# wkh923/m3pc

Hardware: AMD Instinct MI355X
Metric: MPC plan-steps/sec (N=1024, H=16, hopper-medium-v2); independent plan steps, 3 in flight (higher is better)
Workload: dtype bf16; 1 GPU; hopper-medium-v2 shapes (S=11,A=3) rtg_guiding N=1024 H=16 T=32 bf16 candidate pass + fp32 policy pass + fp32 re-score (arg-max and multinomial draw certified under the calibrated bound delta, 8.4 candidates re-scored on average); 3 independent plan steps in flight (policy pass / candidate pass / re-score of neighbouring steps on different streams); window resident in HBM; candidates_per_gpu=1024, global_candidates=1024, horizon=16, traj_length=32, steps_in_flight=3, settle_steps=24, parallelism=1 GPU

## Files before the change

include/m3pc_hip_debug.h:

```cpp
#ifndef M3PC_HIP_DEBUG_H
#define M3PC_HIP_DEBUG_H

#ifdef __cplusplus
extern "C" {
#endif

int m3pc_debug_gemm(int dtype, const void* A, const void* Wt, const float* bias, const float* res, void* C, int M, int N,
                    int K, int gelu, int f32out, int variant, void* stream);
typedef struct m3pc_debug_gemm_args {
    int dtype;
    const void* A;
    int lda;
    int amap[3];
    const void* W;
    int ldw;
    int M, N, K;
    const float* bias;
    const float* rowtab;
    int rt_mod, rt_ld;
    int gelu;
    const float* res;
    int ldr;
    void* C;
    int f32out;
    int ldc;
    int cmap[3];
    float* ws;
    long long ws_bytes;
    int a_padded;
    const float* ln_g;
    const float* ln_b;
    float* ln_out;
    const float* a_ln_g;
    const float* a_ln_b;
    int variant;
    void* stream;
    int* picked;
} m3pc_debug_gemm_args;
int m3pc_debug_gemm_ex(const m3pc_debug_gemm_args* a);
int m3pc_debug_gemm_plan(const m3pc_debug_gemm_args* a);
int m3pc_debug_gemm_group(const m3pc_debug_gemm_args* a, int n);
int m3pc_debug_clock(long long* out2);
int m3pc_debug_clock_big(long long* out4);
int m3pc_debug_topk(const float* v, int n, int k, int* idx_out, void* stream);
int m3pc_debug_calibrate_stats(const float* scores_low, const float* f32, int n, float factor, float* stats, float* delta_out,
                               void* stream);
long long m3pc_debug_block_stream_bytes(void);
int m3pc_debug_block_fused(const void* O, int M, const float* res, const float* rowtab, int rt_mod, const void* Wo, const void* W1,
                           const void* W2, void* stream_buf, int pack, const float* bo, const float* b1, const float* b2,
                           const float* ln2_g, const float* ln2_b, const float* lnA_g, const float* lnA_b, const float* lnB_g0,
                           const float* lnB_b0, const float* lnB_g1, const float* lnB_b1, int out_mod, int out_grp, float* Xout,
                           void* Hout, int variant, void* stream, long long* stamps);
int m3pc_debug_block_fused_qkv(const void* O, int M, const float* res, const void* Wo, const void* W1, const void* W2, const void* Wqkv,
                               void* stream_buf, const float* bo, const float* b1, const float* b2, const float* ln2_g,
                               const float* ln2_b, const float* lnA_g, const float* lnA_b, const float* bqkv, float* Xout, void* QKV,
                               void* stream, long long* stamps, int x_bf16);
int m3pc_debug_block_fused_heads(const void* O, int M, const float* rowtab, int rt_mod, const void* Wo, const void* W1, const void* W2,
                                 const void* Wh, void* stream_buf, const float* bo, const float* b1, const float* b2, const float* ln2_g,
                                 const float* ln2_b, const float* lnA_g, const float* lnA_b, const float* lnB_g0, const float* lnB_b0,
                                 const float* lnB_g1, const float* lnB_b1, int out_mod, int out_grp, const float* hb1, const float* hw2,
                                 const float* hb2, const float* hmean, const float* hstd, float* out0, float* out1, void* stream,
                                 long long* stamps);
long long m3pc_debug_kv_stream_bytes(void);
int m3pc_debug_kv_fused(const void* Z, int n, int Le, int kept0, int off0, int kept1, int off1, const void* We0, const void* We1,
                        const void* Wkv, void* stream_buf, const float* rowtab0, const float* rowtab1, const float* ln_g,
                        const float* ln_b, const float* bkv, void* KV, void* stream, long long* stamps);
int m3pc_debug_attention_bf16(const void* QKV, const void* QKVs, void* O, int batch, int n_own, int n_sh, int kernel, void* stream,
                              long long* stamps);
int m3pc_debug_attention_dec_bf16(const void* Qtab, const void* QKVm, const void* KV, void* O, float* pre, int n, int nq, int Lm, int kernel,
                                  void* stream);
int m3pc_debug_attention_dec_le_bf16(const void* Qtab, const void* QKVm, const void* KV, void* O, float* pre, int n, int nq, int Lm, int Le,
                                     int kernel, void* stream);
int m3pc_debug_attention_mix_bf16(const void* Qown, const void* Qsh, const void* KV, const void* QKVm, void* O, int n, int Lq, int Lq2, int kernel,
                                  void* stream);
int m3pc_debug_attention(int dtype, const void* Q, long long q_bstride, int ldq, int Lq, int orow1, const void* Q2, int ldq2, int Lq2,
                         int orow2, const void* K1, const void* V1, long long kv1_bstride, int ldkv1, int L1, const void* K2,
                         const void* V2, int ldkv2, int L2, const void* Kp, const void* Vp, int ldp, int Lp, float* pre, void* O,
                         long long o_bstride, int ldo, int batch, int n_head, int hd, float scale, int kernel, int* picked,
                         void* stream);
int m3pc_debug_stamp_log(m3pc_handle* h, int cap, long long* out, int* n_logged);
int m3pc_debug_step_streams_created(m3pc_handle* h);
int m3pc_debug_xcc_probe(int* out, int n_blocks, void* stream);

#ifdef __cplusplus
}
#endif
#endif
```

m3pc_amd/capi.py:

```python
from __future__ import annotations

import ctypes as C
import os
from typing import Dict, Optional, Sequence

import torch

_HERE = os.path.dirname(os.path.abspath(__file__))
LIB_PATH = os.environ.get("M3PC_LIB") or os.path.join(_HERE, "libm3pc_hip.so")

STATES, ACTIONS, REWARDS, RETURNS = 0, 1, 2, 3
KEYS = ("states", "actions", "rewards", "returns")
MODE_RTG, MODE_CRITIC, MODE_NOISE = 0, 1, 2
PREC_FP32, PREC_BF16, PREC_BF16X3 = 0, 1, 2
PRECISIONS = {"fp32": PREC_FP32, "bf16": PREC_BF16, "bf16x3": PREC_BF16X3}
LOW_PRECISION = (PREC_BF16, PREC_BF16X3)
PROF_LAYER_TAIL = 16
ABI_VERSION = 7
GOAL_PIID, GOAL_ID = 0, 1
SLOTS = 4


def precision_code(name: str) -> int:
    if name not in PRECISIONS:
# ... 249 lines not shown
        x = x.contiguous()
        out = torch.empty(x.shape, dtype=torch.float32, device=x.device)
        rows = x.numel() // x.shape[-1]
        check(self.lib.m3pc_tokenize(self._h, key, _ptr(x), int(x.dtype == torch.float64), _ptr(out), rows,
                                     _stream(self.device)))
        return out

    def detokenize(self, key: int, y: torch.Tensor) -> torch.Tensor:
        y = y.contiguous()
        out = torch.empty_like(y)
        check(self.lib.m3pc_detokenize(self._h, key, _ptr(y), _ptr(out), y.numel() // y.shape[-1],
                                       _stream(self.device)))
        return out

    def forward(self, tokens: Sequence[Optional[torch.Tensor]], masks: Sequence, want=KEYS, precision=PREC_FP32):
        B = next(t.shape[0] for t in tokens if t is not None)
        toks = [None if t is None else t.to(torch.float32).contiguous() for t in tokens]
        tp = (C.c_void_p * 4)(*[None if t is None else t.data_ptr() for t in toks])
        mb = [bytes(bytearray(int(v != 0) for v in m)) for m in masks]
        mbuf = [C.create_string_buffer(b, len(b)) for b in mb]
        mp = (C.c_void_p * 4)(*[C.addressof(b) for b in mbuf])
        dev = self.device
        feat = (self.S, self.A, 1, 1)
        out = {}
        for k, name in enumerate(KEYS):
            if name in want and k != ACTIONS:
                out[name] = torch.empty((B, self.T, feat[k]), dtype=torch.float32, device=dev)
        mu = sd = None
        if "actions" in want:
            mu = torch.empty((B, self.T, self.A), dtype=torch.float32, device=dev)
            sd = torch.empty_like(mu)
            out["actions"] = (mu, sd)
        check(self.lib.m3pc_forward(self._h, B, tp, mp, _ptr(out.get("states")), _ptr(out.get("rewards")),
                                    _ptr(out.get("returns")), _ptr(mu), _ptr(sd), precision, _stream(dev)))
        return out

    @staticmethod
    def _mask_ptrs(masks):
        mb = [bytes(bytearray(int(v != 0) for v in m)) for m in masks]
        mbuf = [C.create_string_buffer(b, len(b)) for b in mb]
        return (C.c_void_p * 4)(*[C.addressof(b) for b in mbuf]), mbuf

    def goal_step(self, states, actions, rewards, rtg, masks_pi, masks_fid, idx: int):
        E = states.shape[0]
        f32 = dict(dtype=torch.float32, device=self.device)
        ins = [self._f32(t) for t in (states, actions, rewards)]
        inferred = torch.empty((E, self.T, self.S), **f32)
        window = torch.empty((E, self.T, self.S), **f32)
        mu = torch.empty((E, self.T, self.A), **f32)
        sd = torch.empty_like(mu)
        rt = (C.c_double * E)(*[float(v) for v in rtg])
        pi, keep1 = self._mask_ptrs(masks_pi)
        fid, keep2 = self._mask_ptrs(masks_fid)
        check(self.lib.m3pc_goal_step(self._h, E, _ptr(ins[0]), _ptr(ins[1]), _ptr(ins[2]), rt, pi, fid, int(idx), _ptr(inferred),
                                      _ptr(window), _ptr(mu), _ptr(sd), _stream(self.device)))
        return mu, sd, inferred, window

    def goal_step_batch(self, states, actions, idx: int, goal_mode: int = GOAL_PIID, precision: int = PREC_BF16,
                        want_window: bool = False, out=None):
        E = states.shape[0]
        f32 = dict(dtype=torch.float32, device=self.device)
        s, a = self._f32(states), self._f32(actions)
        assert s.shape == (E, self.T, self.S) and a.shape == (E, self.T, self.A)
        mu, sd = out if out is not None else (torch.empty((E, self.A), **f32), torch.empty((E, self.A), **f32))
        window = torch.empty((E, self.T, self.S), **f32) if want_window else None
        check(self.lib.m3pc_goal_step_batch(self._h, E, _ptr(s), _ptr(a), int(idx), int(goal_mode), int(precision), _ptr(window),
                                            _ptr(mu), _ptr(sd), _stream(self.device)))
        return (mu, sd, window) if want_window else (mu, sd)

    @staticmethod
    def _f32(t):
        return t if (t.dtype == torch.float32 and t.is_contiguous()) else t.to(torch.float32).contiguous()

    def _args(self, mode, precision, horizon, n_total, n_begin, n_count, lmbda, discount, rtg, slot=0, returns=None):
        a = PlanArgs(mode, precision, horizon, n_total, n_begin, n_count, lmbda, discount, rtg, slot, 0, None, 0, 0)
        if returns is not None:
            assert returns.is_cuda and returns.is_contiguous() and returns.numel() == self.T
            assert returns.dtype in (torch.float32, torch.float64)
            a.returns_f64 = int(returns.dtype == torch.float64)
            a.returns = returns.data_ptr()
        return a

    def policy_pass(self, mode: int, states, actions, rewards, horizon: int, rtg: float, slot: int = 0, returns=None,
                    loc=None, std=None, pruned: bool = False):
        args = self._args(mode, PREC_FP32, horizon, 1, 0, 1, 0.0, 0.0, rtg, slot, returns)
        if pruned and loc is None and std is None:
            args.flags = PLAN_PRUNED_POLICY
        check(self.lib.m3pc_policy_pass(self._h, C.byref(args), _ptr(self._f32(states)), _ptr(self._f32(actions)),
                                        _ptr(self._f32(rewards)), _ptr(loc), _ptr(std), _stream(self.device)))

    def candidate_pass(self, mode: int, states, actions, rewards, eps, horizon: int, lmbda: float, discount: float,
                       n_total: int, n_begin: int = 0, n_count: Optional[int] = None, precision: int = PREC_FP32, slot: int = 0,
                       want_debug: bool = False, out=None, defer_join: bool = False, window: int = 0):
        n_count = n_total - n_begin if n_count is None else n_count
        dev = self.device
        f32 = dict(dtype=torch.float32, device=dev)
        out = out or {}
        loc = out.get("loc")
        std = out.get("std")
        if loc is None:
            loc = torch.empty((self.T, self.A), **f32)
            std = torch.empty((self.T, self.A), **f32)
        acts = out.get("sample_actions")
        if acts is None:
            acts = torch.empty((n_count, horizon, self.A), **f32)
        er = out.get("expect_return")
        if er is None:
            er = torch.empty((n_count,), **f32)
        pr = torch.empty((n_count, horizon), **f32) if want_debug else None
        pb = torch.empty((n_count, horizon), **f32) if want_debug else None
        args = self._args(mode, precision, horizon, n_total, n_begin, n_count, lmbda, discount, 0.0, slot)
        args.flags = PLAN_DEFER_JOIN if defer_join else 0
        args.window = int(window)
        ins = [self._f32(t) for t in (states, actions, rewards, eps)]
        check(self.lib.m3pc_candidate_pass(self._h, C.byref(args), _ptr(ins[0]), _ptr(ins[1]), _ptr(ins[2]), _ptr(ins[3]),
                                           _ptr(loc), _ptr(std), _ptr(acts), _ptr(er), _ptr(pr), _ptr(pb), _stream(dev)))
        res = dict(loc=loc, std=std, sample_actions=acts, expect_return=er)
        if want_debug:
            res["pred_rewards"], res["pred_boot"] = pr, pb
        return res

    def policy_pass_batch(self, mode: int, states, actions, rewards, horizon: int, rtg, slot: int = 0, loc=None, std=None):
        E = states.shape[0]
        args = self._args(mode, PREC_FP32, horizon, 1, 0, 1, 0.0, 0.0, 0.0, slot)
        rt = (C.c_double * E)(*[float(v) for v in rtg])
        check(self.lib.m3pc_policy_pass_batch(self._h, C.byref(args), E, _ptr(self._f32(states)), _ptr(self._f32(actions)),
                                              _ptr(self._f32(rewards)), rt, _ptr(loc), _ptr(std), _stream(self.device)))

    def candidate_join(self, slot: int):
        check(self.lib.m3pc_candidate_join(self._h, int(slot), _stream(self.device)))

    def plan_step(self, mode: int, states, actions, rewards, eps, horizon: int, rtg: float, lmbda: float,
                  discount: float, n_total: int, n_begin: int = 0, n_count: Optional[int] = None,
                  precision: int = PREC_FP32, want_debug: bool = False, slot: int = 0, returns=None):
        n_count = n_total - n_begin if n_count is None else n_count
        dev = self.device
        f32 = dict(dtype=torch.float32, device=dev)
        loc = torch.empty((self.T, self.A), **f32)
        std = torch.empty((self.T, self.A), **f32)
        acts = torch.empty((n_count, horizon, self.A), **f32)
        er = torch.empty((n_count,), **f32)
        pr = torch.empty((n_count, horizon), **f32) if want_debug else None
        pb = torch.empty((n_count, horizon), **f32) if want_debug else None
        args = self._args(mode, precision, horizon, n_total, n_begin, n_count, lmbda, discount, rtg, slot, returns)
        ins = [self._f32(t) for t in (states, actions, rewards, eps)]
        check(self.lib.m3pc_plan_step(self._h, C.byref(args), _ptr(ins[0]), _ptr(ins[1]), _ptr(ins[2]), _ptr(ins[3]),
                                      _ptr(loc), _ptr(std), _ptr(acts), _ptr(er), _ptr(pr), _ptr(pb), _stream(dev)))
        res = dict(loc=loc, std=std, sample_actions=acts, expect_return=er)
        if want_debug:
            res["pred_rewards"], res["pred_boot"] = pr, pb
        return res

    def plan_step_certified(self, mode: int, states, actions, rewards, eps, expo, horizon: int, rtg: float, lmbda: float,
                            discount: float, n_total: int, temperature: float, delta: float = 0.0, grow_delta: bool = False,
                            kmin: int = 8, kmax: int = 128, rfirst: int = 2, rmax: int = 32, precision: int = PREC_BF16,
                            slot: int = 0, returns=None, pruned: bool = False):
        dev = self.device
        f32 = dict(dtype=torch.float32, device=dev)
        loc = torch.empty((self.T, self.A), **f32)
        std = torch.empty((self.T, self.A), **f32)
        acts = torch.empty((n_total, horizon, self.A), **f32)
        low = torch.empty((n_total,), **f32)
        merged = torch.empty((n_total,), **f32)
        lst = torch.empty((int(rmax) + 1024,), dtype=torch.int32, device=dev)
        sel = self.select_buffers(n_total)
        args = self._args(mode, precision, horizon, n_total, 0, n_total, lmbda, discount, rtg, slot, returns)
        args.flags = PLAN_PRUNED_POLICY if pruned else 0
        cert = CertArgs(float(temperature), float(delta), int(bool(grow_delta)), int(kmin), int(kmax), int(rfirst), int(rmax))
# ... 316 lines not shown
```

m3pc_amd/csrc/elementwise.hip:

```cpp
#include "kernels.h"

namespace m3pc {

__device__ __forceinline__ int map_row(const RowMap& m, int r) {
    if (m.rpg == 0) return r;
    return (r / m.rpg) * m.gstride + (r % m.rpg) + m.off;
}

__device__ __forceinline__ float wave_sum(float v) {
#pragma unroll
    for (int o = 32; o > 0; o >>= 1) v += __shfl_xor(v, o);
    return v;
}
__device__ __forceinline__ float wave_max(float v) {
#pragma unroll
    for (int o = 32; o > 0; o >>= 1) v = fmaxf(v, __shfl_xor(v, o));
    return v;
}

__global__ __launch_bounds__(256) void embed_kernel(EmbedP p) {
    const long long row = blockIdx.x;
    const int b = (int)(row / p.L), j = (int)(row % p.L);
    const int2 kt = p.tokmap[j];
    const int key = kt.x, t = kt.y;
    const int D = p.feat[key];
    const float* x = p.tok[key] + (long long)b * p.bstride[key] + (p.widx ? (long long)p.widx[b] * p.wstride[key] : 0) + (long long)t * D;
    __shared__ float xs[32];
    if (threadIdx.x < D) {
        float v = x[threadIdx.x];
        if (p.normalize[key]) v = (v - p.mean[key][threadIdx.x]) / p.stdv[key][threadIdx.x];
        xs[threadIdx.x] = v;
    }
    __syncthreads();
    const float* WT = p.WT[key];
    const float* E = p.E[key] + (long long)t * p.d;
    float* out = p.X + row * p.d;
    float vals[4];
    float s = 0.f;
#pragma unroll
    for (int i = 0; i < 4; ++i) {
        const int c = threadIdx.x + i * blockDim.x;
        vals[i] = 0.f;
        if (c < p.d) {
            float acc = 0.f;
            for (int f = 0; f < D; ++f) acc = fmaf(xs[f], WT[f * p.d + c], acc);
            acc += E[c];
            out[c] = acc;
            vals[i] = acc;
            s += acc;
        }
    }
    if (!p.ln_g) return;
    __shared__ float red[8];
    const int lane = threadIdx.x & 63, wid = threadIdx.x >> 6, nwv = blockDim.x >> 6;
    s = wave_sum(s);
    if (lane == 0) red[wid] = s;
    __syncthreads();
    float tot = 0.f;
    for (int w = 0; w < nwv; ++w) tot += red[w];
    const float mean = tot / (float)p.d;
    float q = 0.f;
#pragma unroll
    for (int i = 0; i < 4; ++i)
        if (threadIdx.x + i * blockDim.x < p.d) {
            const float c = vals[i] - mean;
            q += c * c;
        }
    q = wave_sum(q);
    __syncthreads();
    if (lane == 0) red[wid] = q;
    __syncthreads();
    tot = 0.f;
    for (int w = 0; w < nwv; ++w) tot += red[w];
    const float rstd = rsqrtf(tot / (float)p.d + 1e-5f);
#pragma unroll
    for (int i = 0; i < 4; ++i) {
        const int c = threadIdx.x + i * blockDim.x;
        if (c < p.d) {
            const float y = (vals[i] - mean) * rstd * p.ln_g[c] + p.ln_b[c];
            if (p.Hf) p.Hf[row * p.d + c] = y;
            if (p.Hb) p.Hb[row * p.d + c] = (bf16_t)y;
        }
    }
}
template <int NV>
__global__ __launch_bounds__(256) void embed_rows_kernel(EmbedP p, int CB, int nchunk) {
    const int lane = threadIdx.x & 63;
    const int w = blockIdx.x * 4 + (threadIdx.x >> 6);
    if (w >= p.L * nchunk) return;
    const int j = w / nchunk, ch = w % nchunk;
    const int2 kt = p.tokmap[j];
    const int key = kt.x, t = kt.y;
    const int D = p.feat[key], d = p.d;
    const float* WT = p.WT[key];
    const float* E = p.E[key] + (long long)t * d;
    const bool indep = j < p.n_indep;
    const int b0 = ch * CB, b1 = b0 + CB < p.batch ? b0 + CB : p.batch;
    if (indep && p.x_first_only && b0 > 0 && p.Hb && !p.Hf && j < p.n_sh) return;
    const int n_own = p.L - p.n_sh;
    float4 ev[NV], gv[NV], bv[NV];
#pragma unroll
    for (int i = 0; i < NV; ++i) {
        const int c = (i * 64 + lane) * 4;
        ev[i] = *(const float4*)(E + c);
        if (p.ln_g) {
            gv[i] = *(const float4*)(p.ln_g + c);
            bv[i] = *(const float4*)(p.ln_b + c);
        }
    }
    float4 x[NV], y[NV];
    for (int b = b0; b < b1; ++b) {
        if (b == b0 || !indep) {
            const float* xin = p.tok[key] + (long long)b * p.bstride[key] + (p.widx ? (long long)p.widx[b] * p.wstride[key] : 0) + (long long)t * D;
#pragma unroll
            for (int i = 0; i < NV; ++i) x[i] = make_float4(0.f, 0.f, 0.f, 0.f);
            for (int f = 0; f < D; ++f) {
                float xf = xin[f];
                if (p.normalize[key]) xf = (xf - p.mean[key][f]) / p.stdv[key][f];
#pragma unroll
                for (int i = 0; i < NV; ++i) {
                    const float4 wv = *(const float4*)(WT + (long long)f * d + (i * 64 + lane) * 4);
                    x[i].x = fmaf(xf, wv.x, x[i].x);
                    x[i].y = fmaf(xf, wv.y, x[i].y);
                    x[i].z = fmaf(xf, wv.z, x[i].z);
                    x[i].w = fmaf(xf, wv.w, x[i].w);
                }
            }
            float s = 0.f;
#pragma unroll
            for (int i = 0; i < NV; ++i) {
                x[i].x += ev[i].x;
                x[i].y += ev[i].y;
                x[i].z += ev[i].z;
                x[i].w += ev[i].w;
                s += (x[i].x + x[i].y) + (x[i].z + x[i].w);
            }
            if (p.ln_g) {
                const float mean = wave_sum(s) / (float)d;
                float q = 0.f;
#pragma unroll
                for (int i = 0; i < NV; ++i) {
                    const float c0 = x[i].x - mean, c1 = x[i].y - mean, c2 = x[i].z - mean, c3 = x[i].w - mean;
                    q += (c0 * c0 + c1 * c1) + (c2 * c2 + c3 * c3);
                }
                const float rstd = rsqrtf(wave_sum(q) / (float)d + 1e-5f);
#pragma unroll
                for (int i = 0; i < NV; ++i) {
                    y[i].x = (x[i].x - mean) * rstd * gv[i].x + bv[i].x;
                    y[i].y = (x[i].y - mean) * rstd * gv[i].y + bv[i].y;
                    y[i].z = (x[i].z - mean) * rstd * gv[i].z + bv[i].z;
                    y[i].w = (x[i].w - mean) * rstd * gv[i].w + bv[i].w;
                }
            }
        }
        const long long row = (long long)b * p.L + j;
        if (!(indep && p.x_first_only && b > 0)) {
            if (p.Xb) {
#pragma unroll
                for (int i = 0; i < NV; ++i) {
                    typedef bf16_t bf16x4_t __attribute__((ext_vector_type(4)));
                    bf16x4_t o;
                    o[0] = (bf16_t)x[i].x;
                    o[1] = (bf16_t)x[i].y;
                    o[2] = (bf16_t)x[i].z;
                    o[3] = (bf16_t)x[i].w;
                    stream_store(o, (bf16x4_t*)(p.Xb + row * d + (i * 64 + lane) * 4));
                }
            } else {
#pragma unroll
                for (int i = 0; i < NV; ++i) *(float4*)(p.X + row * d + (i * 64 + lane) * 4) = x[i];
            }
        }
        if (!p.ln_g) continue;
        if (p.Hf) {
#pragma unroll
            for (int i = 0; i < NV; ++i) *(float4*)(p.Hf + row * d + (i * 64 + lane) * 4) = y[i];
        }
        if (p.Hb) {
            bf16_t* dst;
            if (p.n_sh == 0)
                dst = p.Hb + row * d;
            else if (j >= p.n_sh)
                dst = p.Hb + ((long long)b * n_own + (j - p.n_sh)) * d;
            else if (b == 0)
                dst = p.Hb_sh + (long long)j * d;
            else
                continue;
#pragma unroll
            for (int i = 0; i < NV; ++i) {
                typedef bf16_t bf16x4_t __attribute__((ext_vector_type(4)));
                bf16x4_t o;
                o[0] = (bf16_t)y[i].x;
                o[1] = (bf16_t)y[i].y;
                o[2] = (bf16_t)y[i].z;
                o[3] = (bf16_t)y[i].w;
                stream_store(o, (bf16x4_t*)(dst + (i * 64 + lane) * 4));
            }
        }
    }
}

void launch_embed(const EmbedP& p, hipStream_t st) {
    const long long rows = (long long)p.batch * p.L;
    if (rows <= 0) return;
    if (p.d % 256 == 0 && p.d <= 1024) {
        int CB = p.batch / 64;
        CB = CB < 1 ? 1 : (CB > 16 ? 16 : CB);
        if (p.n_indep == 0 && CB > 4) CB = 4;
        const int nchunk = (p.batch + CB - 1) / CB;
        const int waves = p.L * nchunk;
        const dim3 grid((waves + 3) / 4), block(256);
        switch (p.d / 256) {
            case 1: hipLaunchKernelGGL(embed_rows_kernel<1>, grid, block, 0, st, p, CB, nchunk); break;
            case 2: hipLaunchKernelGGL(embed_rows_kernel<2>, grid, block, 0, st, p, CB, nchunk); break;
            case 3: hipLaunchKernelGGL(embed_rows_kernel<3>, grid, block, 0, st, p, CB, nchunk); break;
            default: hipLaunchKernelGGL(embed_rows_kernel<4>, grid, block, 0, st, p, CB, nchunk); break;
        }
        return;
    }
    hipLaunchKernelGGL(embed_kernel, dim3((unsigned)rows), dim3(p.d < 256 ? p.d : 256), 0, st, p);
}

__global__ __launch_bounds__(256) void gather_rows_kernel(GatherP p) {
    const long long row = blockIdx.x;
    const int b = (int)(row / p.rows_per_batch), i = (int)(row % p.rows_per_batch);
    const int s = p.rowsrc[i];
    const float* src = s >= 0 ? p.Xe + (long long)b * p.xe_bstride + (long long)s * p.d : p.table + (long long)(-s - 1) * p.d;
    for (int c = threadIdx.x * 4; c < p.d; c += blockDim.x * 4) {
        const float4 v = *(const float4*)(src + c);
        if (p.out) *(float4*)(p.out + row * p.d + c) = v;
        if (p.outb) {
            bf16_t* ob = p.outb + row * p.d + c;
            ob[0] = (bf16_t)v.x;
            ob[1] = (bf16_t)v.y;
            ob[2] = (bf16_t)v.z;
            ob[3] = (bf16_t)v.w;
        }
    }
}
void launch_gather_rows(const GatherP& p, hipStream_t st) {
    const long long rows = (long long)p.batch * p.rows_per_batch;
    if (rows <= 0) return;
    hipLaunchKernelGGL(gather_rows_kernel, dim3((unsigned)rows), dim3(p.d / 4 < 256 ? p.d / 4 : 256), 0, st, p);
}

__global__ __launch_bounds__(256) void layernorm_kernel(LnP p) {
    const int lane = threadIdx.x & 63;
    const int r = blockIdx.x * 4 + (threadIdx.x >> 6);
    if (r >= p.rows) return;
    const float* x = p.X + (long long)map_row(p.xmap, r) * p.ldx;
    const int n = p.d >> 6;
    float v[16];
    float s = 0.f;
#pragma unroll
    for (int i = 0; i < 16; ++i)
        if (i < n) {
            v[i] = x[i * 64 + lane];
            s += v[i];
        }
    const float inv_d = 1.0f / (float)p.d;
    float mean = wave_sum(s) * inv_d;
    float q = 0.f;
#pragma unroll
    for (int i = 0; i < 16; ++i)
        if (i < n) {
            const float c = v[i] - mean;
            q += c * c;
        }
    float rstd = rsqrtf(wave_sum(q) * inv_d + 1e-5f);
#pragma unroll
    for (int i = 0; i < 16; ++i)
        if (i < n) v[i] = (v[i] - mean) * rstd * p.g1[i * 64 + lane] + p.b1[i * 64 + lane];
    if (p.g2) {
        s = 0.f;
#pragma unroll
        for (int i = 0; i < 16; ++i)
            if (i < n) s += v[i];
        mean = wave_sum(s) * inv_d;
        q = 0.f;
#pragma unroll
        for (int i = 0; i < 16; ++i)
            if (i < n) {
                const float c = v[i] - mean;
                q += c * c;
            }
        rstd = rsqrtf(wave_sum(q) * inv_d + 1e-5f);
#pragma unroll
        for (int i = 0; i < 16; ++i)
            if (i < n) v[i] = (v[i] - mean) * rstd * p.g2[i * 64 + lane] + p.b2[i * 64 + lane];
    }
#pragma unroll
    for (int i = 0; i < 16; ++i)
        if (i < n) {
            if (p.Yf) p.Yf[(long long)r * p.d + i * 64 + lane] = v[i];
            if (p.Yb) p.Yb[(long long)r * p.d + i * 64 + lane] = (bf16_t)v[i];
        }
}
typedef float f32x4v __attribute__((ext_vector_type(4)));
typedef __bf16 bf16x4v __attribute__((ext_vector_type(4)));
__global__ __launch_bounds__(256) void layernorm_vec_kernel(LnP p) {
// ... 310 lines not shown
#pragma unroll
    for (int f = 0; f < AMAX; ++f) {
        s1[f] = 0.f;
        s2[f] = 0.f;
        const int ff = f < p.A ? f : p.A - 1;
#pragma unroll
        for (int i = 0; i < 4; ++i)
            if (i < n) {
                const f32x4v wm = *(const f32x4v*)(p.Wmu + (long long)ff * p.d + i * 256 + lane * 4);
                const f32x4v wl = *(const f32x4v*)(p.Wls + (long long)ff * p.d + i * 256 + lane * 4);
#pragma unroll
                for (int e = 0; e < 4; ++e) {
                    s1[f] = fmaf(v[i][e], wm[e], s1[f]);
                    s2[f] = fmaf(v[i][e], wl[e], s2[f]);
                }
            }
    }
#pragma unroll
    for (int f = 0; f < AMAX; ++f) {
        s1[f] = wave_sum(s1[f]);
        s2[f] = wave_sum(s2[f]);
    }
#pragma unroll
    for (int f = 0; f < AMAX; ++f)
        if (f < p.A && lane == f) {
            p.mu[(long long)r * p.A + f] = s1[f] + p.bmu[f];
            float ls = tanhf(s2[f] + p.bls[f]);
            ls = -5.0f + 0.5f * (2.0f - (-5.0f)) * (ls + 1.0f);
            p.sd[(long long)r * p.A + f] = expf(ls);
        }
}
__global__ __launch_bounds__(256) void actor_head_small_kernel(ActorP p) {
    const int lane = threadIdx.x & 63;
    const int r = blockIdx.x * 4 + (threadIdx.x >> 6);
    if (r >= p.rows) return;
    const float* x = p.X + (long long)map_row(p.xmap, r) * p.ldx;
    const int n = p.d >> 6;
    float v[16];
#pragma unroll
    for (int i = 0; i < 16; ++i)
        if (i < n) v[i] = x[i * 64 + lane];
    for (int f = 0; f < p.A; ++f) {
        float s1 = 0.f, s2 = 0.f;
#pragma unroll
        for (int i = 0; i < 16; ++i)
            if (i < n) {
                s1 = fmaf(v[i], p.Wmu[(long long)f * p.d + i * 64 + lane], s1);
                s2 = fmaf(v[i], p.Wls[(long long)f * p.d + i * 64 + lane], s2);
            }
        s1 = wave_sum(s1);
        s2 = wave_sum(s2);
        if (lane == 0) {
            p.mu[(long long)r * p.A + f] = s1 + p.bmu[f];
            float ls = tanhf(s2 + p.bls[f]);
            ls = -5.0f + 0.5f * (2.0f - (-5.0f)) * (ls + 1.0f);
            p.sd[(long long)r * p.A + f] = expf(ls);
        }
    }
}
bool actor_head_fuses_ln(int d, int A) { return d % 256 == 0 && d <= 1024 && A <= 8; }
void launch_actor_head(const ActorP& p, hipStream_t st) {
    if (p.rows <= 0) return;
    const dim3 grid((p.rows + 3) / 4), block(256);
    if (actor_head_fuses_ln(p.d, p.A)) {
        if (p.A <= 4) hipLaunchKernelGGL((actor_head_kernel<4>), grid, block, 0, st, p);
        else hipLaunchKernelGGL((actor_head_kernel<8>), grid, block, 0, st, p);
    } else {
        hipLaunchKernelGGL(actor_head_small_kernel, grid, block, 0, st, p);
    }
}

__global__ __launch_bounds__(256) void sample_kernel(SampleP p) {
    const long long tot = (long long)p.n_count * p.T * p.A;
    if (blockIdx.x == 0) {
        for (int x = threadIdx.x; x < p.T * p.A; x += blockDim.x) {
            if (p.loc_out && p.loc) p.loc_out[x] = p.loc[x];
            if (p.sd_out && p.sd) p.sd_out[x] = p.sd[x];
        }
    }
    for (long long x = blockIdx.x * (long long)blockDim.x + threadIdx.x; x < tot; x += (long long)gridDim.x * blockDim.x) {
        const int a = (int)(x % p.A);
        const int t = (int)((x / p.A) % p.T);
        const long long n = x / ((long long)p.A * p.T);
        float v;
        if (t < p.idx) {
            v = p.hist_actions[(p.widx ? (long long)p.widx[n] * p.T * p.A : 0) + t * p.A + a];
        } else {
            const int ta = t * p.A + a;
            const long long src = p.index ? (long long)p.index[n] : p.n_begin + n;
            if (p.mode == 2) {
                v = p.eps[(src * p.h + (t - p.idx)) * p.A + a];
            } else if (p.mode == 0) {
                const float e = p.eps[(src * p.T + t) * p.A + a];
                v = tanhf(__fadd_rn(__fmul_rn(e, p.sd[ta]), p.loc[ta]));
            } else {
                const float e = p.eps[(src * p.h + (t - p.idx)) * p.A + a];
                v = __fadd_rn(tanhf(p.loc[ta]), __fmul_rn(e, 0.09f));
                v = fminf(fmaxf(v, -0.99999f), 0.99999f);
            }
            if (p.sample_actions) p.sample_actions[(n * p.h + (t - p.idx)) * p.A + a] = v;
        }
        p.cand[x] = v;
    }
}
void launch_sample(const SampleP& p, hipStream_t st) {
    const long long tot = (long long)p.n_count * p.T * p.A;
    if (tot <= 0) return;
    const int grid = (int)((tot + 255) / 256 < 2048 ? (tot + 255) / 256 : 2048);
    hipLaunchKernelGGL(sample_kernel, dim3(grid), dim3(256), 0, st, p);
}

#define CR_ROWS 16
__global__ __launch_bounds__(256) void critic_kernel(CriticP p) {
    __shared__ float sa[CR_ROWS][32];
    __shared__ float h1[CR_ROWS][256];
    __shared__ float red[CR_ROWS][4];
    const int tid = threadIdx.x;
    const int r0 = blockIdx.x * CR_ROWS;
    const int SA = p.S + p.A, Hd = p.hidden;
    const bool on = tid < Hd;
    for (int x = tid; x < CR_ROWS * SA; x += 256) {
        const int rr = x / SA, f = x % SA, r = r0 + rr;
        float v = 0.f;
        if (r < p.rows) v = f < p.S ? (p.states[(long long)r * p.S + f] - p.om[f]) / p.os[f] : p.actions[(long long)r * p.A + (f - p.S)];
        sa[rr][f] = v;
    }
    float qmin = 0.f;
    for (int net = 0; net < 2; ++net) {
        __syncthreads();
        {
            float acc[CR_ROWS];
#pragma unroll
            for (int rr = 0; rr < CR_ROWS; ++rr) acc[rr] = 0.f;
            if (on) {
                for (int f = 0; f < SA; ++f) {
                    const float w = p.W1T[net][f * Hd + tid];
#pragma unroll
                    for (int rr = 0; rr < CR_ROWS; ++rr) acc[rr] = fmaf(sa[rr][f], w, acc[rr]);
                }
                const float bb = p.b1[net][tid];
#pragma unroll
                for (int rr = 0; rr < CR_ROWS; ++rr) h1[rr][tid] = fmaxf(acc[rr] + bb, 0.f);
            }
        }
        __syncthreads();
        float acc[CR_ROWS];
#pragma unroll
        for (int rr = 0; rr < CR_ROWS; ++rr) acc[rr] = 0.f;
        float bb = 0.f, w3 = 0.f;
        if (on) {
            for (int k = 0; k < Hd; ++k) {
                const float w = p.W2T[net][k * Hd + tid];
#pragma unroll
                for (int rr = 0; rr < CR_ROWS; ++rr) acc[rr] = fmaf(h1[rr][k], w, acc[rr]);
            }
            bb = p.b2[net][tid];
            w3 = p.W3[net][tid];
        }
#pragma unroll
        for (int rr = 0; rr < CR_ROWS; ++rr) {
            float v = on ? fmaxf(acc[rr] + bb, 0.f) * w3 : 0.f;
            v = wave_sum(v);
            if ((tid & 63) == 0) red[rr][tid >> 6] = v;
        }
        __syncthreads();
        if (tid < CR_ROWS) {
            const float q = red[tid][0] + red[tid][1] + red[tid][2] + red[tid][3] + p.b3[net][0];
            qmin = net == 0 ? q : fminf(qmin, q);
            if (net == 1 && r0 + tid < p.rows) p.q[r0 + tid] = qmin;
        }
    }
}
template <int NT>
__global__ __launch_bounds__(256, 2) void critic_mfma_kernel(CriticP p) {
#if defined(__HIP_DEVICE_COMPILE__)
    typedef float f32x16v __attribute__((ext_vector_type(16)));
    const int lane = threadIdx.x & 63, wave = threadIdx.x >> 6;
    const int l31 = lane & 31, lh = lane >> 5;
    const int r = (blockIdx.x * 4 + wave) * 32 + l31;
    if ((blockIdx.x * 4 + wave) * 32 >= p.rows) return;
    const long long rl = r < p.rows ? r : p.rows - 1;
    const int SA = p.S + p.A;
    float x[16];
#pragma unroll
// ... 244 lines not shown
```

m3pc_amd/csrc/kernels.h:

```cpp
#pragma once
#include <hip/hip_runtime.h>
#include <stdint.h>

#ifdef M3PC_LAB
#define M3PC_ENV(name) getenv(name)
#else
#define M3PC_ENV(name) ((const char*)nullptr)
#endif

namespace m3pc {

typedef __bf16 bf16_t;

enum DType { DT_F32 = 0, DT_BF16 = 1, DT_X3 = 2 };

static inline size_t dtype_size(int dt) { return dt == DT_F32 ? 4 : 2; }

#ifndef M3PC_STREAM_AUX
#define M3PC_STREAM_AUX 0
#endif
template <typename V>
__device__ __forceinline__ V stream_load(const V* p) { return M3PC_STREAM_AUX ? __builtin_nontemporal_load(p) : *p; }
template <typename V>
__device__ __forceinline__ void stream_store(V v, V* p) {
// ... 164 lines not shown
    const float* g2;
    const float* b2;
    float* Yf;
    bf16_t* Yb;
};
void launch_layernorm(const LnP& p, hipStream_t st);

struct AttnP {
    const void* Q;
    long long q_bstride;
    int ldq;
    const void* K1;
    const void* V1;
    long long kv1_bstride;
    int ldkv1;
    int L1;
    const void* K2;
    const void* V2;
    int ldkv2;
    int L2;
    void* O;
    long long o_bstride;
    int ldo;
    int batch, n_head, hd, Lq;
    float scale;
    const void* Q2;
    int ldq2, Lq2;
    int orow1, orow2;
    const float* pre_m;
    const float* pre_l;
    const float* pre_O;
    long long* stamps;
    int no_pipe;
};
void launch_attention_prestats(const AttnP& p, float* pre_m, float* pre_l, float* pre_O, hipStream_t st);
void launch_attention(const AttnP& p, int dtype, hipStream_t st);
#ifdef M3PC_LAB
extern thread_local int g_attn_picked;
#define M3PC_ATTN_PICK(id) (::m3pc::g_attn_picked = (id))
#else
#define M3PC_ATTN_PICK(id) ((void)0)
#endif
void launch_attention_bf16(const AttnP& p, hipStream_t st);
#ifdef M3PC_LAB
extern thread_local int g_gemm_picked[4];
extern thread_local int g_gemm_dry;
#define M3PC_GEMM_PICK(id, S, peel, flags)                                                          \
    (::m3pc::g_gemm_picked[0] = (id), ::m3pc::g_gemm_picked[1] = (S), ::m3pc::g_gemm_picked[2] = (peel), \
     ::m3pc::g_gemm_picked[3] = (flags))
#define M3PC_GEMM_PICK_FLAG(f) (::m3pc::g_gemm_picked[3] |= (f))
#define M3PC_GEMM_LAUNCH(...)                                     \
    do {                                                          \
        if (!::m3pc::g_gemm_dry) hipLaunchKernelGGL(__VA_ARGS__); \
    } while (0)
#else
#define M3PC_GEMM_PICK(id, S, peel, flags) ((void)0)
#define M3PC_GEMM_PICK_FLAG(f) ((void)0)
#define M3PC_GEMM_LAUNCH(...) hipLaunchKernelGGL(__VA_ARGS__)
#endif

struct EmbedP {
    const float* tok[4];
    long long bstride[4];
    const int* widx;
    long long wstride[4];
    int normalize[4];
    const float* mean[4];
    const float* stdv[4];
    const float* WT[4];
    const float* E[4];
    int feat[4];
    const int2* tokmap;
    int batch, L, d, T;
    float* X;
    bf16_t* Xb;
    const float* ln_g;
    const float* ln_b;
    float* Hf;
    bf16_t* Hb;
    int n_indep;
    int x_first_only;
    int n_sh;
    bf16_t* Hb_sh;
};
void launch_embed(const EmbedP& p, hipStream_t st);

struct GatherP {
    const float* Xe;
    long long xe_bstride;
    const float* table;
    const int* rowsrc;
    int rows_per_batch, batch, d;
    float* out;
    bf16_t* outb;
};
void launch_gather_rows(const GatherP& p, hipStream_t st);

struct HeadOutP {
    const float* X;
    const bf16_t* Xb;
    int ldx;
    int rows, d, D;
    const float* W;
    const float* b;
    const float* mean;
    const float* stdv;
    float* Y;
    RowMap ymap;
    int ldy;
};
void launch_head_out(const HeadOutP& p, hipStream_t st);
bool head_out_mfma_covers(int rows, int d, int D);

struct ActorP {
    const float* X;
    int ldx;
    RowMap xmap;
    int rows, d, A;
    const float* Wmu;
    const float* bmu;
    const float* Wls;
    const float* bls;
    float* mu;
    float* sd;
    const float* ln_g;
    const float* ln_b;
};
void launch_actor_head(const ActorP& p, hipStream_t st);
bool actor_head_fuses_ln(int d, int A);

struct SampleP {
    const float* hist_actions;
    const float* loc;
    const float* sd;
    const float* eps;
    int mode, T, A, idx, h, n_begin, n_count;
    const int* widx;
    const int* index;
    float* cand;
    float* sample_actions;
    float* loc_out;
    float* sd_out;
};
void launch_sample(const SampleP& p, hipStream_t st);

struct CriticP {
    const float* states;
    const float* actions;
    int rows, S, A, hidden;
    const float* om;
    const float* os;
    const float* W1T[2];
    const float* b1[2];
    const float* W2T[2];
    const float* b2[2];
    const float* W3[2];
    const float* b3[2];
    const float* W1F[2];
    const float* W2F[2];
    float* q;
};
void launch_critic(const CriticP& p, hipStream_t st);
bool critic_mfma_covers(int S, int A, int hidden);
size_t critic_w1f_floats(int hidden);
size_t critic_w2f_floats(int hidden);
void critic_pack(const float* W1, const float* W2, int SA, int hidden, float* w1f, float* w2f);

struct ScoreP {
// ... 82 lines not shown
```

m3pc_amd/csrc/m3pc.hip:

```cpp
#include <atomic>
#include <chrono>

#include "m3pc_internal.h"

namespace m3pc {
thread_local char g_err[512] = "";
int fail(int code, const char* fmt, ...) {
    va_list ap;
    va_start(ap, fmt);
    vsnprintf(g_err, sizeof(g_err), fmt, ap);
    va_end(ap);
    return code;
}
}

namespace {

int find_tensor(const m3pc_named_tensor* list, int n, const std::string& name) {
    for (int i = 0; i < n; ++i)
        if (list[i].name && name == list[i].name) return i;
    return -1;
}


}


static int fill_rtok(m3pc_handle* h, const double* rtg, int n_windows, hipStream_t st);

#pragma GCC visibility push(default)
extern "C" {

const char* m3pc_last_error(void) { return g_err; }
int m3pc_abi_version(void) { return M3PC_ABI_VERSION; }

int m3pc_create(const m3pc_dims* dims, int device, m3pc_handle** out) {
    if (!dims || !out) return fail(M3PC_EINVAL, "null argument");
    const m3pc_dims& D = *dims;
    if (D.n_embd % 64 || D.n_embd > 1024 || D.n_head <= 0 || D.n_embd % D.n_head)
        return fail(M3PC_EINVAL, "n_embd must be a multiple of 64 (<=1024) and divisible by n_head");
    const int hd = D.n_embd / D.n_head;
    if (hd != 32 && hd != 64 && hd != 128) return fail(M3PC_EINVAL, "head_dim %d unsupported (32, 64, 128)", hd);
    if (D.state_dim < 1 || D.state_dim > 32 || D.action_dim < 1 || D.action_dim > 32)
        return fail(M3PC_EINVAL, "state_dim/action_dim must be in [1,32]");
    if (D.traj_length < 1 || D.traj_length > 64) return fail(M3PC_EINVAL, "traj_length must be in [1,64]");
    if (D.n_dec_layer != 1) return fail(M3PC_EINVAL, "n_dec_layer must be 1 (every shipped m3pc config)");
    if (D.n_enc_layer < 1 || D.max_candidates < 1 || D.max_batch < 1) return fail(M3PC_EINVAL, "bad sizes");
    if (D.critic_hidden < 0 || D.critic_hidden > 256) return fail(M3PC_EINVAL, "critic_hidden must be <= 256");
    if (D.max_goal_batch < 0) return fail(M3PC_EINVAL, "max_goal_batch must be >= 0");
    HIPCHK(hipSetDevice(device));
    std::unique_ptr<m3pc_handle> h(new m3pc_handle());
    h->dm = D;
    h->device = device;
    h->d = D.n_embd;
    h->nh = D.n_head;
    h->hd = hd;
    h->T = D.traj_length;
    h->S = D.state_dim;
    h->A = D.action_dim;
    h->ff = 4 * D.n_embd;
    h->feat[0] = D.state_dim;
    h->feat[1] = D.action_dim;
    h->feat[2] = 1;
    h->feat[3] = 1;
    declare_weights(h.get());
    for (auto& kv : h->w) {
        CHK(dmalloc(&kv.second.f, (size_t)kv.second.numel));
        if (kv.second.gemm) {
            CHK(dmalloc(&kv.second.b, 2 * (size_t)kv.second.numel));
            h->gemm_w.push_back({kv.second.f, &kv.second});
        }
    }
    std::sort(h->gemm_w.begin(), h->gemm_w.end());
    const int d = h->d, T = h->T;
    for (int k = 0; k < 4; ++k) {
        CHK(dmalloc(&h->WT[k], (size_t)h->feat[k] * d));
        CHK(dmalloc(&h->Eenc[k], (size_t)T * d));
        CHK(dmalloc(&h->Edec[k], (size_t)T * d));
        CHK(dmalloc(&h->tok_mean[k], 32));
        CHK(dmalloc(&h->tok_std[k], 32));
    }
    CHK(dmalloc(&h->mask_tokens, (size_t)4 * d));
    {
        const long long r1 = (long long)D.max_candidates * 2 * T, r2 = (long long)D.max_batch * 4 * T;
        const long long r3 = (long long)D.max_goal_batch * 2 * T;
        long long R = r1 > r2 ? r1 : r2;
        if (r3 > R) R = r3;
        if (R < 4 * T) R = 4 * T;
        CHK(alloc_ws(h.get(), h->base, R, D.max_candidates > D.max_goal_batch ? D.max_candidates : D.max_goal_batch, 64LL << 20));
        if (D.max_goal_batch > 0) CHK(dmalloc(&h->goal_ws, (size_t)D.max_goal_batch * T * h->S));
    }
    {
        const int mr = D.max_rescore > 0 ? D.max_rescore : 64;
        long long R = (long long)mr * 2 * T;
        if (R < 4 * T) R = 4 * T;
        for (int par = 0; par < 2; ++par) {
            CHK(alloc_ws(h.get(), h->chain[par], R, mr, 32LL << 20));
            CHK(alloc_ws(h.get(), h->pchain[par], (long long)D.max_batch * 4 * T, 1, 32LL << 20));
        }
    }
    for (int s = 0; s < M3PC_SLOTS; ++s) {
        CHK(dmalloc(&h->slot[s].loc, (size_t)D.max_batch * T * h->A + 64));
        CHK(dmalloc(&h->slot[s].sd, (size_t)D.max_batch * T * h->A + 64));
        CHK(dmalloc(&h->slot[s].rtok, (size_t)D.max_batch * T));
    }
    CHK(dmalloc(&h->sel_scratch, 64));
    CHK(dmalloc(&h->d_topk, 1024));
    CHK(dmalloc(&h->er_top, 1024));
    CHK(dmalloc(&h->sa_buf, (size_t)(D.max_candidates > h->chain[0].max_cand ? D.max_candidates : h->chain[0].max_cand) * T * h->A));
    CHK(dmalloc(&h->sa_chain[0], (size_t)h->chain[0].max_cand * T * h->A));
    CHK(dmalloc(&h->sa_chain[1], (size_t)h->chain[0].max_cand * T * h->A));
    CHK(dmalloc(&h->refine_noise, (size_t)D.max_candidates * T * h->A));
    CHK(dmalloc(&h->refine_scores, (size_t)D.max_candidates));
    CHK(dmalloc(&h->refine_elites, (size_t)D.max_candidates));
    for (int s = 0; s < M3PC_SLOTS; ++s) {
        CHK(dmalloc(&h->cert_list[s], 64 + 1024));
        CHK(dmalloc(&h->cert_b[s], 64 + 1024));
        CHK(dmalloc(&h->cert_f[s], 64 + 1024));
        CHK(dmalloc(&h->cert_stats[s], 32));
        CHK(dmalloc(&h->cert_f32[s], (size_t)D.max_candidates));
        CHK(dmalloc(&h->cert_top1[s], 4));
    }
    HIPCHK(hipHostMalloc((void**)&h->cert_host, (size_t)M3PC_SLOTS * 8 * sizeof(float), hipHostMallocMapped | hipHostMallocCoherent));
    memset(h->cert_host, 0, (size_t)M3PC_SLOTS * 8 * sizeof(float));
    HIPCHK(hipHostGetDevicePointer((void**)&h->cert_host_dev, h->cert_host, 0));
    bind_ws(h.get(), &h->base);
    bind_slot(h.get(), 0);
    {
        static std::map<int, hipStream_t> shared_aux;
        static std::mutex shared_aux_mutex;
        std::lock_guard<std::mutex> lock(shared_aux_mutex);
        hipStream_t& sa = shared_aux[device];
#ifdef M3PC_LAB
        if (!sa)
            if (const char* e = M3PC_ENV("M3PC_AUX_CU_MASK")) {
                std::vector<uint32_t> words;
                for (const char* q = e; *q;) {
                    words.push_back((uint32_t)strtoul(q, nullptr, 16));
                    while (*q && *q != ',') ++q;
                    if (*q == ',') ++q;
                }
                HIPCHK(hipExtStreamCreateWithCUMask(&sa, (uint32_t)words.size(), words.data()));
            }
#endif
        if (!sa) HIPCHK(hipStreamCreateWithFlags(&sa, hipStreamNonBlocking));
        h->aux = sa;
    }
    HIPCHK(hipEventCreateWithFlags(&h->ev_fork, hipEventDisableTiming));
    HIPCHK(hipEventCreateWithFlags(&h->ev_join, hipEventDisableTiming));
    for (int s = 0; s < M3PC_SLOTS; ++s)
        for (int i = 0; i < 3; ++i) HIPCHK(hipEventCreateWithFlags(&h->slot_join[s][i], hipEventDisableTiming));
    for (int i = 0; i < 3; ++i) HIPCHK(hipEventCreateWithFlags(&h->aux_tail[i], hipEventDisableTiming));
    if (const char* e = M3PC_ENV("M3PC_TWO_STREAM")) h->two_stream = atoi(e) != 0;
    h->auxs.push_back(h->aux);
    h->ev_joins.push_back(h->ev_join);
    if (const char* e = M3PC_ENV("M3PC_STREAM_SPLIT")) {
        for (const char* q = e; *q;) {
            h->stream_split.push_back(atoi(q));
            while (*q && *q != ',') ++q;
            if (*q == ',') ++q;
        }
        for (size_t i = 1; i < h->stream_split.size() && i < 3; ++i) {
            hipStream_t s2;
            hipEvent_t e2;
            HIPCHK(hipStreamCreateWithFlags(&s2, hipStreamNonBlocking));
            HIPCHK(hipEventCreateWithFlags(&e2, hipEventDisableTiming));
            h->auxs.push_back(s2);
            h->ev_joins.push_back(e2);
        }
    }
    if (D.critic_hidden > 0) {
        const int Hd = D.critic_hidden, SA = h->S + h->A;
        for (int i = 0; i < 2; ++i) {
            CHK(dmalloc(&h->cW1T[i], (size_t)SA * Hd));
            CHK(dmalloc(&h->cb1[i], Hd));
            CHK(dmalloc(&h->cW2T[i], (size_t)Hd * Hd));
            CHK(dmalloc(&h->cb2[i], Hd));
            CHK(dmalloc(&h->cW3[i], Hd));
            CHK(dmalloc(&h->cb3[i], 4));
            if (critic_mfma_covers(h->S, h->A, Hd)) {
                CHK(dmalloc(&h->cW1F[i], critic_w1f_floats(Hd)));
                CHK(dmalloc(&h->cW2F[i], critic_w2f_floats(Hd)));
            }
        }
        CHK(dmalloc(&h->c_om, 32));
        CHK(dmalloc(&h->c_os, 32));
    }
    *out = h.release();
    return 0;
}

int m3pc_destroy(m3pc_handle* h) {
    if (!h) return 0;
    hipSetDevice(h->device);
    hipDeviceSynchronize();
    for (auto& kv : h->w) {
        hipFree(kv.second.f);
        if (kv.second.b) hipFree(kv.second.b);
    }
    for (int k = 0; k < 4; ++k) {
        hipFree(h->WT[k]);
        hipFree(h->Eenc[k]);
        hipFree(h->Edec[k]);
        hipFree(h->tok_mean[k]);
        hipFree(h->tok_std[k]);
    }
    hipFree(h->mask_tokens);
    free_ws(h->base);
    for (int par = 0; par < 2; ++par) {
        free_ws(h->chain[par]);
        free_ws(h->pchain[par]);
    }
    for (int s = 0; s < M3PC_SLOTS; ++s) {
        hipFree(h->slot[s].loc);
        hipFree(h->slot[s].sd);
        hipFree(h->slot[s].rtok);
    }
    void* bufs[] = {h->sel_scratch, h->d_topk, h->er_top, h->sa_buf, h->sa_chain[0], h->sa_chain[1], h->c_om, h->c_os, h->goal_ws,
                    h->refine_noise, h->refine_scores, h->refine_elites};
    for (int s = 0; s < M3PC_SLOTS; ++s) {
        void* cb[] = {h->cert_list[s], h->cert_b[s], h->cert_f[s], h->cert_stats[s], h->cert_f32[s], h->cert_top1[s]};
        for (void* b : cb)
            if (b) hipFree(b);
        for (int i = 0; i < 4; ++i)
            if (h->step_ev[s][i]) hipEventDestroy(h->step_ev[s][i]);
    }
    if (h->ev_excl) hipEventDestroy(h->ev_excl);
    if (h->step_chain_own)
        for (int i = 0; i < 2; ++i)
            if (h->step_chain[i]) hipStreamDestroy(h->step_chain[i]);
    if (h->cert_host) hipHostFree(h->cert_host);
    for (size_t i = 1; i < h->auxs.size(); ++i) {
        hipStreamDestroy(h->auxs[i]);
        hipEventDestroy(h->ev_joins[i]);
    }
    for (int s = 0; s < M3PC_SLOTS; ++s)
        for (int i = 0; i < 3; ++i)
            if (h->slot_join[s][i]) hipEventDestroy(h->slot_join[s][i]);
    for (int i = 0; i < 3; ++i)
        if (h->aux_tail[i]) hipEventDestroy(h->aux_tail[i]);
    if (h->aux) hipStreamSynchronize(h->aux);
    if (h->ev_fork) hipEventDestroy(h->ev_fork);
    if (h->ev_join) hipEventDestroy(h->ev_join);
    for (void* b : bufs)
        if (b) hipFree(b);
    for (int i = 0; i < 2; ++i) {
        void* cb[] = {h->cW1T[i], h->cb1[i], h->cW2T[i], h->cb2[i], h->cW3[i], h->cb3[i], h->cW1F[i], h->cW2F[i]};
        for (void* b : cb)
            if (b) hipFree(b);
    }
    for (auto& kv : h->plans) {
        Plan* pl = kv.second.get();
        hipFree(pl->d_tokmap);
        hipFree(pl->d_dec_rowsrc);
        hipFree(pl->d_masked_rowsrc);
        for (int k = 0; k < 4; ++k)
            if (pl->edec_own[k]) hipFree(pl->edec_own[k]);
        for (int q = 0; q < N_QUERY; ++q) {
            if (pl->query[q].d_q_rowsrc_tab) hipFree(pl->query[q].d_q_rowsrc_tab);
            if (pl->query[q].d_q_rowsrc_mix) hipFree(pl->query[q].d_q_rowsrc_mix);
            for (int pr = 0; pr < 2; ++pr) free_tables(pl->query[q].tab[pr]);
        }
    }
    for (auto& e : h->ev) {
        hipEventDestroy(e.a);
        hipEventDestroy(e.b);
    }
    for (int k = 0; k < 4; ++k)
        if (h->kvstream[k]) hipFree(h->kvstream[k]);
    for (auto& kv : h->wstream)
        if (kv.second) hipFree(kv.second);
    delete h;
    return 0;
}

int m3pc_load_weights(m3pc_handle* h, const m3pc_named_tensor* tensors, int n, void* stream) {
    if (!h || !tensors) return fail(M3PC_EINVAL, "null argument");
    hipStream_t st = (hipStream_t)stream;
    HIPCHK(hipSetDevice(h->device));
    CHK(ws_sync(h, st));
    const bool first = !h->weights_loaded;
    std::vector<std::string> dirty;
    for (auto& kv : h->w) {
        const int i = find_tensor(tensors, n, kv.first);
        if (i < 0) {
            if (first) return fail(M3PC_EINVAL, "state_dict is missing '%s'", kv.first.c_str());
            continue;
        }
        if (tensors[i].numel != kv.second.numel)
            return fail(M3PC_EINVAL, "'%s' has %lld elements, expected %lld", kv.first.c_str(), tensors[i].numel, kv.second.numel);
        HIPCHK(hipMemcpyAsync(kv.second.f, tensors[i].data, (size_t)kv.second.numel * sizeof(float),
                              tensors[i].on_device ? hipMemcpyDeviceToDevice : hipMemcpyHostToDevice, st));
        if (kv.second.gemm) launch_f32_split_bf16(kv.second.f, kv.second.b, kv.second.b + kv.second.numel, kv.second.numel, st);
        kv.second.loaded = true;
        dirty.push_back(kv.first);
    }
    auto is_dirty = [&](const std::string& name) {
        for (const std::string& d : dirty)
            if (d == name) return true;
        return false;
    };
    long long* ls = h->load_stats;
    ls[0] = (long long)dirty.size();
    ls[1] = ls[2] = ls[3] = 0;
    if (block_fused_supported(h->d, h->ff)) {
        auto pack = [&](const std::string& pfx, const std::string& nxt) -> int {
            const bool own = is_dirty(pfx + ".self_attn.out_proj.weight") || is_dirty(pfx + ".linear1.weight") || is_dirty(pfx + ".linear2.weight");
            const bool qkv = !nxt.empty() && is_dirty(nxt + ".self_attn.in_proj_weight");
            if (!own && !qkv) return 0;
            bf16_t*& ws = h->wstream[pfx];
            if (!ws) CHK(dmalloc((char**)&ws, block_stream_bytes()));
            if (own)
                launch_pack_block_stream(W(h, pfx + ".self_attn.out_proj.weight").b, W(h, pfx + ".linear1.weight").b,
                                         W(h, pfx + ".linear2.weight").b, ws, st);
            if (qkv) launch_pack_block_qkv(W(h, nxt + ".self_attn.in_proj_weight").b, ws, st);
            ++ls[1];
            return 0;
        };
        for (int i = 0; i < h->dm.n_enc_layer; ++i)
            CHK(pack("encoder.layers." + std::to_string(i), i + 1 < h->dm.n_enc_layer ? "encoder.layers." + std::to_string(i + 1) : ""));
        for (int i = 0; i < h->dm.n_dec_layer; ++i) CHK(pack("decoder.layers." + std::to_string(i), ""));
        if (h->dm.n_dec_layer >= 1 && h->wstream.count("decoder.layers.0")) {
            const std::string w0 = std::string("output_head_dict.") + KEYN[M3PC_REWARDS] + ".1.weight";
            const std::string w1 = std::string("output_head_dict.") + KEYN[M3PC_RETURNS] + ".1.weight";
            if (is_dirty(w0) || is_dirty(w1)) {
                launch_pack_block_heads(W(h, w0).b, W(h, w1).b, h->wstream["decoder.layers.0"], st);
                ++ls[1];
            }
        }
        if (h->dm.n_dec_layer >= 1)
            for (int k = 0; k < 4; ++k) {
                const std::string we = std::string("decoder_embed_dict.") + KEYN[k] + ".weight";
                if (!(is_dirty(we) || is_dirty("decoder.layers.0.self_attn.in_proj_weight"))) continue;
                if (!h->kvstream[k]) CHK(dmalloc((char**)&h->kvstream[k], kv_stream_bytes()));
                launch_pack_kv_stream(W(h, we).b, W(h, "decoder.layers.0.self_attn.in_proj_weight").b + (size_t)h->d * h->d,
                                      h->kvstream[k], st);
                ++ls[2];
            }
    }
    const int d = h->d, T = h->T;
    const bool pos_dirty = is_dirty("pos_embed");
    for (int k = 0; k < 4; ++k) {
        const std::string kn = KEYN[k];
        if (is_dirty("encoder_embed_dict." + kn + ".weight"))
            launch_transpose_f32(W(h, "encoder_embed_dict." + kn + ".weight").f, h->WT[k], d, h->feat[k], st);
        for (int pass = 0; pass < 2; ++pass) {
            const std::string side = pass == 0 ? "encoder" : "decoder";
            if (pos_dirty || is_dirty(side + "_embed_dict." + kn + ".bias") || is_dirty(side + "_per_dim_encoding." + kn))
                launch_embed_table(W(h, side + "_embed_dict." + kn + ".bias").f, W(h, side + "_per_dim_encoding." + kn).f,
                                   W(h, "pos_embed").f, pass == 0 ? h->Eenc[k] : h->Edec[k], T, d, st);
        }
        if (is_dirty("mask_token_dict." + kn))
            HIPCHK(hipMemcpyAsync(h->mask_tokens + (size_t)k * d, W(h, "mask_token_dict." + kn).f, d * sizeof(float),
                                  hipMemcpyDeviceToDevice, st));
    }
    bool dec_dirty = pos_dirty;
    for (const std::string& nme : dirty)
        if (nme.rfind("decoder", 0) == 0 || nme.rfind("mask_token_dict", 0) == 0) dec_dirty = true;
    if (dec_dirty) {
        invalidate_tables(h);
        ls[3] = 1;
    }
    for (int sl = 0; sl < M3PC_SLOTS; ++sl) {
        h->slot[sl].policy_valid = false;
        h->slot[sl].n_windows = 0;
    }
    HIPCHK(hipStreamSynchronize(st));
    h->weights_loaded = true;
    return check_launch("load_weights");
}

int m3pc_load_stats(m3pc_handle* h, long long* out4) {
    if (!h || !out4) return fail(M3PC_EINVAL, "null argument");
    for (int i = 0; i < 4; ++i) out4[i] = h->load_stats[i];
    return 0;
}

int m3pc_set_tokenizer(m3pc_handle* h, int key, const float* mean, const float* std_, int dim, int normalize) {
    if (!h || key < 0 || key > 3 || !mean || !std_) return fail(M3PC_EINVAL, "bad argument");
    if (dim != h->feat[key]) return fail(M3PC_EINVAL, "tokenizer '%s' has dim %d, expected %d", KEYN[key], dim, h->feat[key]);
    HIPCHK(hipSetDevice(h->device));
    HIPCHK(hipMemcpy(h->tok_mean[key], mean, dim * sizeof(float), hipMemcpyHostToDevice));
    HIPCHK(hipMemcpy(h->tok_std[key], std_, dim * sizeof(float), hipMemcpyHostToDevice));
    h->h_mean[key].assign(mean, mean + dim);
    h->h_std[key].assign(std_, std_ + dim);
    h->tok_norm[key] = normalize ? 1 : 0;
    h->tok_set[key] = true;
    return 0;
}

int m3pc_set_critic(m3pc_handle* h, const m3pc_named_tensor* tensors, int n, const float* obs_mean, const float* obs_std,
                    void* stream) {
    if (!h || !tensors || !obs_mean || !obs_std) return fail(M3PC_EINVAL, "null argument");
    if (h->dm.critic_hidden <= 0) return fail(M3PC_EINVAL, "handle was created without a critic");
    hipStream_t st = (hipStream_t)stream;
    HIPCHK(hipSetDevice(h->device));
    HIPCHK(hipStreamSynchronize(st));
    const int Hd = h->dm.critic_hidden, SA = h->S + h->A;
    auto fetch = [&](const std::string& name, long long numel, std::vector<float>& out) -> int {
        const int i = find_tensor(tensors, n, name);
        if (i < 0) return fail(M3PC_EINVAL, "critic state_dict is missing '%s'", name.c_str());
        if (tensors[i].numel != numel) return fail(M3PC_EINVAL, "'%s' has %lld elements, expected %lld", name.c_str(), tensors[i].numel, numel);
        out.resize((size_t)numel);
        HIPCHK(hipMemcpy(out.data(), tensors[i].data, (size_t)numel * sizeof(float),
                         tensors[i].on_device ? hipMemcpyDeviceToHost : hipMemcpyHostToHost));
        return 0;
    };
    for (int qn = 0; qn < 2; ++qn) {
        const std::string q = qn == 0 ? "q1" : "q2";
        std::vector<float> w1, b1, w2, b2, w3, b3;
        CHK(fetch(q + ".net.0.weight", (long long)Hd * SA, w1));
        CHK(fetch(q + ".net.0.bias", Hd, b1));
        CHK(fetch(q + ".net.2.weight", (long long)Hd * Hd, w2));
        CHK(fetch(q + ".net.2.bias", Hd, b2));
        CHK(fetch(q + ".net.4.weight", Hd, w3));
        CHK(fetch(q + ".net.4.bias", 1, b3));
        std::vector<float> w1t((size_t)SA * Hd), w2t((size_t)Hd * Hd);
        for (int c = 0; c < Hd; ++c)
            for (int f = 0; f < SA; ++f) w1t[(size_t)f * Hd + c] = w1[(size_t)c * SA + f];
        for (int c = 0; c < Hd; ++c)
            for (int k = 0; k < Hd; ++k) w2t[(size_t)k * Hd + c] = w2[(size_t)c * Hd + k];
        HIPCHK(hipMemcpy(h->cW1T[qn], w1t.data(), w1t.size() * sizeof(float), hipMemcpyHostToDevice));
        HIPCHK(hipMemcpy(h->cb1[qn], b1.data(), b1.size() * sizeof(float), hipMemcpyHostToDevice));
        HIPCHK(hipMemcpy(h->cW2T[qn], w2t.data(), w2t.size() * sizeof(float), hipMemcpyHostToDevice));
        HIPCHK(hipMemcpy(h->cb2[qn], b2.data(), b2.size() * sizeof(float), hipMemcpyHostToDevice));
        HIPCHK(hipMemcpy(h->cW3[qn], w3.data(), w3.size() * sizeof(float), hipMemcpyHostToDevice));
        HIPCHK(hipMemcpy(h->cb3[qn], b3.data(), sizeof(float), hipMemcpyHostToDevice));
        if (h->cW1F[qn]) {
            std::vector<float> w1f(critic_w1f_floats(Hd)), w2f(critic_w2f_floats(Hd));
            critic_pack(w1.data(), w2.data(), SA, Hd, w1f.data(), w2f.data());
            HIPCHK(hipMemcpy(h->cW1F[qn], w1f.data(), w1f.size() * sizeof(float), hipMemcpyHostToDevice));
            HIPCHK(hipMemcpy(h->cW2F[qn], w2f.data(), w2f.size() * sizeof(float), hipMemcpyHostToDevice));
        }
    }
    HIPCHK(hipMemcpy(h->c_om, obs_mean, h->S * sizeof(float), hipMemcpyHostToDevice));
    HIPCHK(hipMemcpy(h->c_os, obs_std, h->S * sizeof(float), hipMemcpyHostToDevice));
    h->critic_set = true;
    return 0;
}

int m3pc_tokenize(m3pc_handle* h, int key, const void* in, int in_f64, float* out, long long rows, void* stream) {
    if (!h || key < 0 || key > 3 || !in || !out) return fail(M3PC_EINVAL, "bad argument");
    if (!h->tok_set[key]) return fail(M3PC_ESTATE, "tokenizer '%s' not set", KEYN[key]);
    HIPCHK(hipSetDevice(h->device));
    launch_tokenize(in, in_f64, out, rows, h->feat[key], h->tok_mean[key], h->tok_std[key], h->tok_norm[key], (hipStream_t)stream);
    return check_launch("tokenize");
}

int m3pc_detokenize(m3pc_handle* h, int key, const float* in, float* out, long long rows, void* stream) {
    if (!h || key < 0 || key > 3 || !in || !out) return fail(M3PC_EINVAL, "bad argument");
    if (!h->tok_set[key]) return fail(M3PC_ESTATE, "tokenizer '%s' not set", KEYN[key]);
    HIPCHK(hipSetDevice(h->device));
    launch_detokenize(in, out, rows, h->feat[key], h->tok_mean[key], h->tok_std[key], h->tok_norm[key], (hipStream_t)stream);
    return check_launch("detokenize");
}

int m3pc_forward(m3pc_handle* h, int batch, const float* const tokens[4], const unsigned char* const masks[4],
                 float* out_states, float* out_rewards, float* out_returns, float* out_mu, float* out_std, int precision,
                 void* stream) {
    if (!h || !tokens || !masks) return fail(M3PC_EINVAL, "null argument");
    if (!h->weights_loaded) return fail(M3PC_ESTATE, "weights not loaded");
    if (batch < 1 || batch > h->dm.max_batch) return fail(M3PC_EINVAL, "batch %d outside [1, max_batch=%d]", batch, h->dm.max_batch);
    if (!precision_ok(precision)) return fail(M3PC_EINVAL, "bad precision %d", precision);
    if ((out_mu == nullptr) != (out_std == nullptr)) return fail(M3PC_EINVAL, "out_mu and out_std go together");
    HIPCHK(hipSetDevice(h->device));
    Plan* pl = nullptr;
    CHK(get_plan(h, masks, &pl));
    TokIn in;
    memset(&in, 0, sizeof(in));
    for (int k = 0; k < 4; ++k) {
        if (pl->kept[k] && !tokens[k]) return fail(M3PC_EINVAL, "tokens[%s] is null but its mask keeps tokens", KEYN[k]);
        in.ptr[k] = tokens[k];
        in.bstride[k] = (long long)h->T * h->feat[k];
    }
    h->allow_splitk = true;
    CHK(ws_sync(h, (hipStream_t)stream));
    X3Scope x3(h, precision == M3PC_PREC_BF16X3);
    return forward_impl(h, pl, in, batch, out_states, out_rewards, out_returns, out_mu, out_std, pass_dt(precision),
                        (hipStream_t)stream);
}

int m3pc_goal_step(m3pc_handle* h, int batch, const float* states, const float* actions, const float* rewards, const double* rtg,
                   const unsigned char* const masks_pi[4], const unsigned char* const masks_fid[4], int idx, float* inferred,
                   float* window_states, float* out_mu, float* out_std, void* stream) {
    if (!h || !states || !actions || !rewards || !rtg || !masks_pi || !masks_fid || !inferred || !window_states || !out_mu || !out_std)
        return fail(M3PC_EINVAL, "null argument");
    if (!h->weights_loaded) return fail(M3PC_ESTATE, "weights not loaded");
    for (int k = 0; k < 4; ++k)
        if (!h->tok_set[k]) return fail(M3PC_ESTATE, "tokenizer '%s' not set", KEYN[k]);
    if (batch < 1 || batch > h->dm.max_batch) return fail(M3PC_EINVAL, "batch %d outside [1, max_batch=%d]", batch, h->dm.max_batch);
    const int T = h->T;
    if (idx < 0 || idx >= T) return fail(M3PC_EINVAL, "idx %d outside [0, T=%d)", idx, T);
    hipStream_t st = (hipStream_t)stream;
    HIPCHK(hipSetDevice(h->device));
    Plan *pi = nullptr, *fid = nullptr;
    CHK(get_plan(h, masks_pi, &pi));
    CHK(get_plan(h, masks_fid, &fid));
    bind_slot(h, 0);
    h->slot[0].policy_valid = false;
    h->slot[0].n_windows = 0;
    CHK(fill_rtok(h, rtg, batch, st));
    TokIn in;
    memset(&in, 0, sizeof(in));
    const float* src[4] = {states, actions, rewards, h->rtok};
    for (int k = 0; k < 4; ++k) {
        in.ptr[k] = src[k];
        in.bstride[k] = (long long)T * h->feat[k];
        in.normalize[k] = k == M3PC_RETURNS ? 0 : h->tok_norm[k];
    }
    h->allow_splitk = true;
    WsScope ws(h, true, true);
    CHK(forward_impl(h, pi, in, batch, inferred, nullptr, nullptr, nullptr, nullptr, DT_F32, st));
    launch_goal_overlay(inferred, states, window_states, (long long)batch * T, T, h->S, idx, h->tok_mean[M3PC_STATES],
                        h->tok_std[M3PC_STATES], h->tok_norm[M3PC_STATES], st);
    in.ptr[M3PC_STATES] = window_states;
    CHK(forward_impl(h, fid, in, batch, nullptr, nullptr, nullptr, out_mu, out_std, DT_F32, st));
    return check_launch("goal_step");
}

static int goal_prepare(m3pc_handle* h, int kind, int qi, int idx, int dt, hipStream_t st, Plan** pl_out, Plan::Query** q_out) {
    const int T = h->T;
    Plan* pl = nullptr;
    CHK(get_mask_plan(h, kind, idx, &pl));
    std::vector<int> toks;
    if (qi == 2) {
        for (int t = 0; t < T; ++t)
            if (t <= idx || (t >= idx + 2 && t < T - 1)) toks.push_back(M3PC_STATES * T + t);
    } else {
        toks.push_back(M3PC_ACTIONS * T + idx);
    }
    CHK(build_query_list(h, pl, qi, T - idx, toks, 1, qi == 2 ? M3PC_STATES : M3PC_ACTIONS, 0));
    CHK(build_tables(h, pl, qi, dt, st));
    CHK(ensure_edec(h, pl, st));
    if (pl_out) *pl_out = pl;
    if (q_out) *q_out = &pl->query[qi];
    return 0;
}

static int goal_forward(m3pc_handle* h, int kind, int qi, int idx, const float* states, const float* actions, int n, int dt,
                        hipStream_t st, int tail, float** xrows) {
    const int T = h->T;
    Plan* pl = nullptr;
    Plan::Query* qp = nullptr;
    CHK(goal_prepare(h, kind, qi, idx, dt, st, &pl, &qp));
    Plan::Query& q = *qp;
    if ((long long)n * pl->Le > h->R || (long long)n * q.nq > h->R) return fail(M3PC_ENOMEM, "batch %d exceeds workspace", n);
    TokIn in;
    memset(&in, 0, sizeof(in));
    in.ptr[M3PC_STATES] = states;
    in.bstride[M3PC_STATES] = (long long)T * h->S;
    in.normalize[M3PC_STATES] = h->tok_norm[M3PC_STATES];
    in.ptr[M3PC_ACTIONS] = actions;
    in.bstride[M3PC_ACTIONS] = (long long)T * h->A;
    in.normalize[M3PC_ACTIONS] = h->tok_norm[M3PC_ACTIONS];
    CHK(run_encoder(h, pl, in, n, dt, st, dt == DT_BF16, 0));
    return pruned_decoder(h, pl, q, q.tab[dt], n, dt, st, tail, xrows);
}

int m3pc_goal_step_batch(m3pc_handle* h, int batch, const float* states, const float* actions, int idx, int goal_mode,
                         int precision, float* window_states, float* out_mu, float* out_std, void* stream) {
    if (!h || !states || !actions || !out_mu || !out_std) return fail(M3PC_EINVAL, "null argument");
    if (!h->weights_loaded) return fail(M3PC_ESTATE, "weights not loaded");
    for (int k = 0; k < 2; ++k)
        if (!h->tok_set[k]) return fail(M3PC_ESTATE, "tokenizer '%s' not set", KEYN[k]);
    if (batch < 1 || batch > h->dm.max_goal_batch) return fail(M3PC_EINVAL, "batch %d outside [1, max_goal_batch=%d]", batch, h->dm.max_goal_batch);
    if (!precision_ok(precision)) return fail(M3PC_EINVAL, "bad precision %d", precision);
    if (goal_mode != M3PC_GOAL_PIID && goal_mode != M3PC_GOAL_ID) return fail(M3PC_EINVAL, "bad goal_mode %d", goal_mode);
    const int T = h->T, d = h->d;
    if (idx < 0 || idx >= T) return fail(M3PC_EINVAL, "idx %d outside [0, T=%d)", idx, T);
    hipStream_t st = (hipStream_t)stream;
    HIPCHK(hipSetDevice(h->device));
    const int dt = pass_dt(precision);
    X3Scope x3(h, precision == M3PC_PREC_BF16X3);
    bind_ws(h, &h->base);
    CHK(ws_sync(h, st));
    h->allow_splitk = false;
    h->pass_scale = 1.0;
    int nq_a = 0;
    for (int t = 0; t < T; ++t) nq_a += (t <= idx || (t >= idx + 2 && t < T - 1)) ? 1 : 0;
    float* const ws_all = window_states ? window_states : h->goal_ws;
    auto run_part = [&](int c0, int cnt, hipStream_t s) -> int {
        set_view(h, c0, cnt);
        const float* st_p = states + (size_t)c0 * T * h->S;
// ... 7 lines not shown
        } else if (window_states) {
            HIPCHK(hipMemcpyAsync(window_states + (size_t)c0 * T * h->S, st_p, (size_t)cnt * T * h->S * sizeof(float), hipMemcpyDeviceToDevice, s));
        }
        float* xr = nullptr;
        CHK(goal_forward(h, goal_mode == M3PC_GOAL_PIID ? 3 : 2, 3, idx, second, ac_p, cnt, dt, s, TAIL_X, &xr));
        const bool fuse_ln = actor_head_fuses_ln(d, h->A);
        if (!fuse_ln) {
            LnP ln;
            memset(&ln, 0, sizeof(ln));
            ln.X = xr;
            ln.ldx = d;
            ln.rows = cnt;
            ln.d = d;
            ln.g1 = W(h, "decoder.norm.weight").f;
            ln.b1 = W(h, "decoder.norm.bias").f;
            ln.Yf = h->G;
            launch_layernorm(ln, s);
        }
        ActorP ac;
        memset(&ac, 0, sizeof(ac));
        ac.X = fuse_ln ? xr : h->G;
        if (fuse_ln) {
            ac.ln_g = W(h, "decoder.norm.weight").f;
            ac.ln_b = W(h, "decoder.norm.bias").f;
        }
        ac.ldx = d;
        ac.rows = cnt;
        ac.d = d;
        ac.A = h->A;
        ac.Wmu = W(h, "output_head_dict.actions.mu.weight").f;
        ac.bmu = W(h, "output_head_dict.actions.mu.bias").f;
        ac.Wls = W(h, "output_head_dict.actions.log_std.weight").f;
        ac.bls = W(h, "output_head_dict.actions.log_std.bias").f;
        ac.mu = out_mu + (size_t)c0 * h->A;
        ac.sd = out_std + (size_t)c0 * h->A;
        launch_actor_head(ac, s);
        return 0;
    };
    int rc = 0;
    if (h->two_stream && dt == DT_BF16 && batch >= 2048 && !h->prof_serial) {
        const int n0 = ((batch / 2 + 63) / 64) * 64;
        if (goal_mode == M3PC_GOAL_PIID) CHK(goal_prepare(h, 2, 2, idx, dt, st, nullptr, nullptr));
        CHK(goal_prepare(h, goal_mode == M3PC_GOAL_PIID ? 3 : 2, 3, idx, dt, st, nullptr, nullptr));
        HIPCHK(hipEventRecord(h->ev_fork, st));
        HIPCHK(hipStreamWaitEvent(h->aux, h->ev_fork, 0));
        h->pass_scale = (double)batch / (double)n0;
        rc = run_part(0, n0, st);
        h->pass_scale = (double)batch / (double)(batch - n0);
        if (rc == 0) rc = run_part(n0, batch - n0, h->aux);
        HIPCHK(hipEventRecord(h->ev_join, h->aux));
        HIPCHK(hipStreamWaitEvent(st, h->ev_join, 0));
    } else {
        rc = run_part(0, batch, st);
    }
    h->pass_scale = 1.0;
    set_view(h, 0, h->base.max_cand);
    if (rc) return rc;
    return check_launch("goal_step_batch");
}

static int plan_check(m3pc_handle* h, const m3pc_plan_args* a, bool need_critic) {
    if (!h->weights_loaded) return fail(M3PC_ESTATE, "weights not loaded");
    for (int k = 0; k < 4; ++k)
        if (!h->tok_set[k]) return fail(M3PC_ESTATE, "tokenizer '%s' not set", KEYN[k]);
    const int T = h->T;
    if (a->horizon < 1 || a->horizon > T) return fail(M3PC_EINVAL, "horizon %d outside [1, T=%d]", a->horizon, T);
    if (a->mode < 0 || a->mode > 2) return fail(M3PC_EINVAL, "bad mode %d", a->mode);
    if (!precision_ok(a->precision)) return fail(M3PC_EINVAL, "bad precision %d", a->precision);
    if (a->slot < 0 || a->slot >= M3PC_SLOTS) return fail(M3PC_EINVAL, "slot %d outside [0, %d)", a->slot, M3PC_SLOTS);
    if (a->flags & ~(M3PC_PLAN_DEFER_JOIN | M3PC_PLAN_PRUNED_POLICY))
        return fail(M3PC_EINVAL, "unknown m3pc_plan_args::flags 0x%x (is the caller's structure the ABI v%d one?)", a->flags, M3PC_ABI_VERSION);
    if (need_critic && a->mode != M3PC_MODE_RTG && !h->critic_set) return fail(M3PC_ESTATE, "critic weights not set");
    HIPCHK(hipSetDevice(h->device));
    bind_slot(h, a->slot);
    return 0;
}

int m3pc_policy_pass(m3pc_handle* h, const m3pc_plan_args* a, const float* states, const float* actions, const float* rewards,
                     float* loc, float* std_, void* stream) {
    if (!h || !a || !states || !actions || !rewards) return fail(M3PC_EINVAL, "null argument");
    CHK(plan_check(h, a, false));
    hipStream_t st = (hipStream_t)stream;
    const int T = h->T, hh = a->horizon, idx = T - hh;
    if (a->returns) {
        launch_tokenize(a->returns, a->returns_f64, h->rtok, T, 1, h->tok_mean[M3PC_RETURNS], h->tok_std[M3PC_RETURNS],
                        h->tok_norm[M3PC_RETURNS], st);
    } else {
        double rt = a->rtg;
        if (h->tok_norm[M3PC_RETURNS]) rt = (rt - (double)h->h_mean[M3PC_RETURNS][0]) / (double)h->h_std[M3PC_RETURNS][0];
        launch_fill(h->rtok, (float)rt, T, st);
    }
    Plan* pl = nullptr;
    CHK(get_mask_plan(h, 0, idx, &pl));
    TokIn in;
    memset(&in, 0, sizeof(in));
    in.ptr[M3PC_STATES] = states;
    in.normalize[M3PC_STATES] = h->tok_norm[M3PC_STATES];
    in.ptr[M3PC_ACTIONS] = actions;
    in.normalize[M3PC_ACTIONS] = h->tok_norm[M3PC_ACTIONS];
    in.ptr[M3PC_REWARDS] = rewards;
    in.normalize[M3PC_REWARDS] = h->tok_norm[M3PC_REWARDS];
    in.ptr[M3PC_RETURNS] = h->rtok;
    h->allow_splitk = true;
    int rc;
    if ((a->flags & M3PC_PLAN_PRUNED_POLICY) && !loc && !std_ && idx > 0) {
        WsScope ws(h, true, true, a->slot);
        std::vector<int> toks;
        for (int t = idx; t < T; ++t) toks.push_back(M3PC_ACTIONS * T + t);
        rc = build_query_list(h, pl, 4, hh, toks, 1, M3PC_ACTIONS, 0);
        if (!rc) rc = build_tables(h, pl, 4, DT_F32, st);
        if (!rc && !pl->query[4].all_masked) rc = fail(M3PC_EINVAL, "policy pass: an action token at t >= idx is not masked");
        if (!rc) rc = run_encoder(h, pl, in, 1, DT_F32, st, false, 0);
        float* xr = nullptr;
        if (!rc) rc = pruned_decoder(h, pl, pl->query[4], pl->query[4].tab[DT_F32], 1, DT_F32, st, TAIL_X, &xr);
        if (!rc) {
            const int d = h->d;
            const bool fuse_ln = actor_head_fuses_ln(d, h->A);
            if (!fuse_ln) {
                LnP ln;
                memset(&ln, 0, sizeof(ln));
                ln.X = xr;
                ln.ldx = d;
                ln.rows = hh;
                ln.d = d;
                ln.g1 = W(h, "decoder.norm.weight").f;
                ln.b1 = W(h, "decoder.norm.bias").f;
                ln.Yf = h->G;
                launch_layernorm(ln, st);
            }
            ActorP ac;
            memset(&ac, 0, sizeof(ac));
            ac.X = fuse_ln ? xr : h->G;
            if (fuse_ln) {
                ac.ln_g = W(h, "decoder.norm.weight").f;
                ac.ln_b = W(h, "decoder.norm.bias").f;
            }
            ac.ldx = d;
            ac.rows = hh;
            ac.d = d;
            ac.A = h->A;
            ac.Wmu = W(h, "output_head_dict.actions.mu.weight").f;
            ac.bmu = W(h, "output_head_dict.actions.mu.bias").f;
            ac.Wls = W(h, "output_head_dict.actions.log_std.weight").f;
            ac.bls = W(h, "output_head_dict.actions.log_std.bias").f;
            ac.mu = h->loc + (size_t)idx * h->A;
            ac.sd = h->sd + (size_t)idx * h->A;
            launch_actor_head(ac, st);
            if (hipMemsetAsync(h->loc, 0, (size_t)idx * h->A * sizeof(float), st) != hipSuccess ||
                hipMemsetAsync(h->sd, 0, (size_t)idx * h->A * sizeof(float), st) != hipSuccess)
                rc = fail(M3PC_EHIP, "hipMemsetAsync failed in the pruned policy pass");
        }
    } else {
        WsScope ws(h, true, true, a->slot);
        rc = forward_impl(h, pl, in, 1, nullptr, nullptr, nullptr, h->loc, h->sd, DT_F32, st);
    }
    h->allow_splitk = false;
    if (rc) return rc;
    h->slot[a->slot].policy_valid = true;
    h->slot[a->slot].n_windows = 1;
    if (loc) HIPCHK(hipMemcpyAsync(loc, h->loc, (size_t)T * h->A * sizeof(float), hipMemcpyDeviceToDevice, st));
    if (std_) HIPCHK(hipMemcpyAsync(std_, h->sd, (size_t)T * h->A * sizeof(float), hipMemcpyDeviceToDevice, st));
    return check_launch("policy_pass");
}

int m3pc_candidate_pass(m3pc_handle* h, const m3pc_plan_args* a, const float* states, const float* actions, const float* rewards,
                        const float* eps, float* loc, float* std_, float* sample_actions, float* expect_return,
                        float* pred_rewards, float* pred_boot, void* stream) {
    if (!h || !a || !states || !actions || !rewards || !eps || !sample_actions || !expect_return)
        return fail(M3PC_EINVAL, "null argument");
    CHK(plan_check(h, a, true));
    if (a->window < 0 || a->window >= h->slot[a->slot].n_windows)
        return fail(M3PC_ESTATE, "m3pc_candidate_pass: slot %d holds %d policy pass(es), window %d asked for (m3pc_policy_pass[_batch] first)",
                    a->slot, h->slot[a->slot].n_windows, a->window);
    const int T = h->T;
    if (a->n_count < 1 || a->n_begin < 0 || a->n_begin + a->n_count > a->n_total)
        return fail(M3PC_EINVAL, "candidate range [%d,+%d) outside n_total=%d", a->n_begin, a->n_count, a->n_total);
    if (a->n_count > h->dm.max_candidates) return fail(M3PC_ENOMEM, "n_count %d > max_candidates %d", a->n_count, h->dm.max_candidates);
    hipStream_t st = (hipStream_t)stream;
    const int hh = a->horizon, idx = T - hh;
    bind_ws(h, &h->base);
    h->allow_splitk = false;

    auto sample = [&](int c0, int cnt, hipStream_t s) {
        SampleP sp;
        memset(&sp, 0, sizeof(sp));
        sp.hist_actions = actions;
        sp.loc = h->loc + (size_t)a->window * T * h->A;
        sp.sd = h->sd + (size_t)a->window * T * h->A;
        sp.eps = eps;
        sp.mode = a->mode == M3PC_MODE_NOISE ? 1 : 0;
        sp.T = T;
        sp.A = h->A;
        sp.idx = idx;
        sp.h = hh;
        sp.n_begin = a->n_begin + c0;
        sp.n_count = cnt;
        sp.cand = h->base.cand + (size_t)c0 * T * h->A;
        sp.sample_actions = sample_actions + (size_t)c0 * hh * h->A;
        if (c0 == 0) {
            sp.loc_out = loc;
            sp.sd_out = std_;
        }
        launch_sample(sp, s);
    };

    const int dt = pass_dt(a->precision);
    X3Scope x3(h, a->precision == M3PC_PREC_BF16X3);
    const int n = a->n_count;
    h->slot_join_n[a->slot] = 0;
    if (h->two_stream && dt == DT_BF16 && n >= 512 && (long long)n * (2 * T - hh + 1) > 256 * 128) {
        std::vector<int> parts;
        if (!h->stream_split.empty()) {
            int left = n;
            for (int v : h->stream_split)
                if (v > 0 && v < left && parts.size() + 1 < h->auxs.size() + 1) {
                    parts.push_back(v);
                    left -= v;
                }
            parts.push_back(left);
        } else {
            int n0 = ((n / 2 + 127) / 128) * 128;
            parts = {n0, n - n0};
        }
        const bool defer = (a->flags & M3PC_PLAN_DEFER_JOIN) != 0 && !h->prof_serial && parts.size() <= 4;
        if (!(defer && parts == h->defer_parts)) CHK(ws_sync(h, st));
        HIPCHK(hipEventRecord(h->ev_fork, st));
        int rc = 0;
        const int n_stage = h->dm.n_enc_layer + 1;
        PieceState lnst[4];
        for (int stg = 0; stg < (h->prof_serial ? 1 : n_stage) && rc == 0; ++stg) {
            int c0 = 0;
            for (size_t i = 0; i < parts.size() && rc == 0; ++i) {
                hipStream_t s = i == 0 || h->prof_serial ? st : h->auxs[i - 1];
                if (stg == 0) {
                    if (s != st) HIPCHK(hipStreamWaitEvent(s, h->ev_fork, 0));
                    sample(c0, parts[i], s);
                }
                set_view(h, c0, parts[i]);
                rc = candidate_pass(h, a, states, rewards, parts[i], sample_actions + (size_t)c0 * hh * h->A, expect_return + c0,
                                    pred_rewards ? pred_rewards + (size_t)c0 * hh : nullptr,
                                    pred_boot ? pred_boot + (size_t)c0 * hh : nullptr, dt, s, nullptr,
                                    h->prof_serial ? 0 : stg, h->prof_serial ? 1 << 30 : stg + 1, &lnst[i]);
                if (s != st && stg == n_stage - 1 && rc == 0) {
                    if (defer) {
                        HIPCHK(hipEventRecord(h->slot_join[a->slot][i - 1], s));
                        HIPCHK(hipEventRecord(h->aux_tail[i - 1], s));
                        h->aux_unjoined[i - 1] = true;
                        h->slot_join_n[a->slot] = (int)i;
                    } else {
                        HIPCHK(hipEventRecord(h->ev_joins[i - 1], s));
                        HIPCHK(hipStreamWaitEvent(st, h->ev_joins[i - 1], 0));
                    }
                }
                c0 += parts[i];
            }
        }
        if (defer && rc == 0) h->defer_parts = parts;
        set_view(h, 0, h->dm.max_candidates);
        return rc;
    }
    CHK(ws_sync(h, st));
    sample(0, n, st);
    return candidate_pass(h, a, states, rewards, n, sample_actions, expect_return, pred_rewards, pred_boot, dt, st);
}

int m3pc_candidate_join(m3pc_handle* h, int slot, void* stream) {
    if (!h) return fail(M3PC_EINVAL, "null handle");
    if (slot < 0 || slot >= M3PC_SLOTS) return fail(M3PC_EINVAL, "slot %d outside [0, %d)", slot, M3PC_SLOTS);
    for (int i = 0; i < h->slot_join_n[slot]; ++i) HIPCHK(hipStreamWaitEvent((hipStream_t)stream, h->slot_join[slot][i], 0));
    h->slot_join_n[slot] = 0;
    return 0;
}

int m3pc_plan_step(m3pc_handle* h, const m3pc_plan_args* a, const float* states, const float* actions, const float* rewards,
                   const float* eps, float* loc, float* std_, float* sample_actions, float* expect_return,
                   float* pred_rewards, float* pred_boot, void* stream) {
    if (!h || !a || !states || !actions || !rewards || !eps || !sample_actions || !expect_return)
        return fail(M3PC_EINVAL, "null argument");
    if (a->mode >= 0 && a->mode <= 2 && a->mode != M3PC_MODE_RTG && !h->critic_set) return fail(M3PC_ESTATE, "critic weights not set");
    if (a->n_count < 1 || a->n_begin < 0 || a->n_begin + a->n_count > a->n_total)
        return fail(M3PC_EINVAL, "candidate range [%d,+%d) outside n_total=%d", a->n_begin, a->n_count, a->n_total);
    if (a->n_count > h->dm.max_candidates) return fail(M3PC_ENOMEM, "n_count %d > max_candidates %d", a->n_count, h->dm.max_candidates);
    CHK(m3pc_policy_pass(h, a, states, actions, rewards, nullptr, nullptr, stream));
    return m3pc_candidate_pass(h, a, states, actions, rewards, eps, loc, std_, sample_actions, expect_return, pred_rewards,
                               pred_boot, stream);
}

static int fill_rtok(m3pc_handle* h, const double* rtg, int n_windows, hipStream_t st) {
    for (int w = 0; w < n_windows; ++w) {
        double rt = rtg[w];
        if (h->tok_norm[M3PC_RETURNS]) rt = (rt - (double)h->h_mean[M3PC_RETURNS][0]) / (double)h->h_std[M3PC_RETURNS][0];
        launch_fill(h->rtok + (size_t)w * h->T, (float)rt, h->T, st);
    }
    return 0;
}

int m3pc_score_actions(m3pc_handle* h, const m3pc_plan_args* a, int n_windows, const float* states, const float* actions,
                       const float* rewards, const float* cand, const int* window_index, float* expect_return,
                       float* pred_rewards, float* pred_boot, void* stream) {
    if (!h || !a || !states || !actions || !rewards || !cand || !expect_return) return fail(M3PC_EINVAL, "null argument");
    if (!h->weights_loaded) return fail(M3PC_ESTATE, "weights not loaded");
    for (int k = 0; k < 4; ++k)
        if (!h->tok_set[k]) return fail(M3PC_ESTATE, "tokenizer '%s' not set", KEYN[k]);
    const int T = h->T, n = a->n_count;
    if (a->horizon < 1 || a->horizon > T) return fail(M3PC_EINVAL, "horizon %d outside [1, T=%d]", a->horizon, T);
    if (a->mode != M3PC_MODE_RTG && a->mode != M3PC_MODE_CRITIC) return fail(M3PC_EINVAL, "mode must be RTG or CRITIC scoring");
    if (!precision_ok(a->precision)) return fail(M3PC_EINVAL, "bad precision %d", a->precision);
    if (n < 1 || (n > h->dm.max_candidates && !(a->precision == M3PC_PREC_FP32 && n <= h->chain[0].max_cand)))
        return fail(M3PC_ENOMEM, "n_count %d outside [1, max_candidates=%d]", n, h->dm.max_candidates);
    if (n_windows < 1 || (n_windows > 1 && !window_index)) return fail(M3PC_EINVAL, "n_windows > 1 needs window_index");
    if (a->mode == M3PC_MODE_CRITIC && !h->critic_set) return fail(M3PC_ESTATE, "critic weights not set");
    hipStream_t st = (hipStream_t)stream;
    HIPCHK(hipSetDevice(h->device));
    const int dt = pass_dt(a->precision);
    const bool fp32 = a->precision == M3PC_PREC_FP32;
    X3Scope x3(h, a->precision == M3PC_PREC_BF16X3);
    WsScope ws(h, fp32 && n <= h->chain[0].max_cand, false, a->slot);
    if (h->cur == &h->base) CHK(ws_sync(h, st));
    SampleP sp;
    memset(&sp, 0, sizeof(sp));
    sp.hist_actions = actions;
    sp.eps = cand;
    sp.mode = 2;
    sp.T = T;
    sp.A = h->A;
    sp.idx = T - a->horizon;
    sp.h = a->horizon;
    sp.n_count = n;
    sp.widx = window_index;
    sp.cand = h->cand;
    launch_sample(sp, st);
    h->allow_splitk = fp32;
    const int rc = candidate_pass(h, a, states, rewards, n, cand, expect_return, pred_rewards, pred_boot, dt, st, window_index);
    h->allow_splitk = false;
    return rc;
}

int m3pc_policy_pass_batch(m3pc_handle* h, const m3pc_plan_args* a, int n_windows, const float* states, const float* actions,
                           const float* rewards, const double* rtg, float* loc, float* std_, void* stream) {
    if (!h || !a || !states || !actions || !rewards || !rtg) return fail(M3PC_EINVAL, "null argument");
    if (!h->weights_loaded) return fail(M3PC_ESTATE, "weights not loaded");
    for (int k = 0; k < 4; ++k)
        if (!h->tok_set[k]) return fail(M3PC_ESTATE, "tokenizer '%s' not set", KEYN[k]);
    const int T = h->T, E = n_windows;
    if (E < 1 || E > h->dm.max_batch) return fail(M3PC_ENOMEM, "n_windows %d outside [1, max_batch=%d]", E, h->dm.max_batch);
    if (a->horizon < 1 || a->horizon > T) return fail(M3PC_EINVAL, "horizon %d outside [1, T=%d]", a->horizon, T);
    if (a->mode < 0 || a->mode > 2) return fail(M3PC_EINVAL, "bad mode %d", a->mode);
    if (a->slot < 0 || a->slot >= M3PC_SLOTS) return fail(M3PC_EINVAL, "slot %d outside [0, %d)", a->slot, M3PC_SLOTS);
    hipStream_t st = (hipStream_t)stream;
    HIPCHK(hipSetDevice(h->device));
    const int idx = T - a->horizon, A = h->A;
    bind_slot(h, a->slot);
    CHK(fill_rtok(h, rtg, E, st));
    Plan* pl = nullptr;
    CHK(get_mask_plan(h, 0, idx, &pl));
    TokIn in;
    memset(&in, 0, sizeof(in));
    in.ptr[M3PC_STATES] = states;
    in.bstride[M3PC_STATES] = (long long)T * h->S;
    in.normalize[M3PC_STATES] = h->tok_norm[M3PC_STATES];
    in.ptr[M3PC_ACTIONS] = actions;
    in.bstride[M3PC_ACTIONS] = (long long)T * A;
    in.normalize[M3PC_ACTIONS] = h->tok_norm[M3PC_ACTIONS];
    in.ptr[M3PC_REWARDS] = rewards;
    in.bstride[M3PC_REWARDS] = T;
    in.normalize[M3PC_REWARDS] = h->tok_norm[M3PC_REWARDS];
    in.ptr[M3PC_RETURNS] = h->rtok;
    in.bstride[M3PC_RETURNS] = T;
    h->allow_splitk = true;
    {
        WsScope ws(h, true, true, a->slot);
        const int rc = forward_impl(h, pl, in, E, nullptr, nullptr, nullptr, h->loc, h->sd, DT_F32, st);
        h->allow_splitk = false;
        if (rc) return rc;
    }
    h->slot[a->slot].policy_valid = E == 1;
    h->slot[a->slot].n_windows = E;
    if (loc) HIPCHK(hipMemcpyAsync(loc, h->loc, (size_t)E * T * A * sizeof(float), hipMemcpyDeviceToDevice, st));
    if (std_) HIPCHK(hipMemcpyAsync(std_, h->sd, (size_t)E * T * A * sizeof(float), hipMemcpyDeviceToDevice, st));
    return check_launch("policy_pass_batch");
}

int m3pc_plan_step_batch(m3pc_handle* h, const m3pc_plan_args* a, int n_windows, const float* states, const float* actions,
                         const float* rewards, const double* rtg, const float* eps, const int* window_index, float* loc,
                         float* std_, float* sample_actions, float* expect_return, void* stream) {
    if (!h || !a || !states || !actions || !rewards || !rtg || !eps || !window_index || !sample_actions || !expect_return)
        return fail(M3PC_EINVAL, "null argument");
    const int T = h->T, E = n_windows, N = a->n_total;
    if (!precision_ok(a->precision)) return fail(M3PC_EINVAL, "bad precision %d", a->precision);
    if (E >= 1 && (N < 1 || (long long)E * N > h->dm.max_candidates))
        return fail(M3PC_ENOMEM, "n_windows * n_total = %lld > max_candidates %d", (long long)E * N, h->dm.max_candidates);
    if (a->mode >= 0 && a->mode <= 2 && a->mode != M3PC_MODE_RTG && !h->critic_set) return fail(M3PC_ESTATE, "critic weights not set");
    CHK(m3pc_policy_pass_batch(h, a, n_windows, states, actions, rewards, rtg, nullptr, nullptr, stream));
    hipStream_t st = (hipStream_t)stream;
    const int hh = a->horizon, idx = T - hh, A = h->A;
    h->slot[a->slot].policy_valid = false;
    CHK(ws_sync(h, st));
    for (int w = 0; w < E; ++w) {
        SampleP sp;
        memset(&sp, 0, sizeof(sp));
        sp.hist_actions = actions + (size_t)w * T * A;
        sp.loc = h->loc + (size_t)w * T * A;
        sp.sd = h->sd + (size_t)w * T * A;
        const size_t per = a->mode == M3PC_MODE_NOISE ? (size_t)hh * A : (size_t)T * A;
        sp.eps = eps + (size_t)w * N * per;
        sp.mode = a->mode == M3PC_MODE_NOISE ? 1 : 0;
        sp.T = T;
        sp.A = A;
        sp.idx = idx;
        sp.h = hh;
        sp.n_count = N;
        sp.cand = h->cand + (size_t)w * N * T * A;
        sp.sample_actions = sample_actions + (size_t)w * N * hh * A;
        sp.loc_out = loc ? loc + (size_t)w * T * A : nullptr;
        sp.sd_out = std_ ? std_ + (size_t)w * T * A : nullptr;
        launch_sample(sp, st);
    }
    const int dt = pass_dt(a->precision);
    X3Scope x3(h, a->precision == M3PC_PREC_BF16X3);
    return candidate_pass(h, a, states, rewards, E * N, sample_actions, expect_return, nullptr, nullptr, dt, st, window_index);
}

int m3pc_rescore(m3pc_handle* h, const m3pc_plan_args* a, const float* states, const float* actions, const float* rewards,
                 const float* eps, const int* index, int n, float* sample_actions, float* expect_return, void* stream) {
    if (!h || !a || !states || !actions || !rewards || !eps || !index || !expect_return) return fail(M3PC_EINVAL, "null argument");
    if (!h->weights_loaded) return fail(M3PC_ESTATE, "weights not loaded");
    if (a->slot < 0 || a->slot >= M3PC_SLOTS) return fail(M3PC_EINVAL, "slot %d outside [0, %d)", a->slot, M3PC_SLOTS);
    if (!h->slot[a->slot].policy_valid) return fail(M3PC_ESTATE, "m3pc_rescore needs a preceding m3pc_plan_step / m3pc_policy_pass on slot %d", a->slot);
    const int T = h->T;
    if (a->horizon < 1 || a->horizon > T || a->mode < 0 || a->mode > 2) return fail(M3PC_EINVAL, "bad horizon/mode");
    const bool in_chain = n <= h->chain[0].max_cand;
    if (n < 1 || (!in_chain && n > h->dm.max_candidates))
        return fail(M3PC_ENOMEM, "n %d outside [1, max(max_rescore=%d, max_candidates=%d)]", n, h->chain[0].max_cand, h->dm.max_candidates);
    if (a->mode != M3PC_MODE_RTG && !h->critic_set) return fail(M3PC_ESTATE, "critic weights not set");
    hipStream_t st = (hipStream_t)stream;
    HIPCHK(hipSetDevice(h->device));
    bind_slot(h, a->slot);
    WsScope ws(h, in_chain, false, a->slot);
    if (!in_chain) CHK(ws_sync(h, st));
    float* sa = sample_actions ? sample_actions : (in_chain ? h->sa_chain[a->slot & 1] : h->sa_buf);
    SampleP sp;
    memset(&sp, 0, sizeof(sp));
    sp.hist_actions = actions;
    sp.loc = h->loc;
    sp.sd = h->sd;
    sp.eps = eps;
    sp.mode = a->mode == M3PC_MODE_NOISE ? 1 : 0;
    sp.T = T;
    sp.A = h->A;
    sp.idx = T - a->horizon;
    sp.h = a->horizon;
    sp.n_count = n;
    sp.index = index;
    sp.cand = h->cand;
    sp.sample_actions = sa;
    launch_sample(sp, st);
    h->allow_splitk = true;
    const int rc = candidate_pass(h, a, states, rewards, n, sa, expect_return, nullptr, nullptr, DT_F32, st);
    h->allow_splitk = false;
    return rc;
// ... 605 lines not shown
int m3pc_refine_plan(m3pc_handle* h, const m3pc_plan_args* a, const m3pc_refine_args* r, const float* states, const float* actions,
                     const float* rewards, const float* init_mean, const float* noise, float* mean, float* std_, float* candidates,
                     float* scores, int* elites, float* sample_action, float* eval_action, void* stream) {
    if (!h || !a || !r || !states || !actions || !rewards || !mean || !std_ || !candidates) return fail(M3PC_EINVAL, "null argument");
    CHK(cert_check_args(a, "m3pc_refine_plan"));
    if (a->mode != M3PC_MODE_RTG && a->mode != M3PC_MODE_CRITIC) return fail(M3PC_EINVAL, "m3pc_refine_plan: mode must be RTG or CRITIC scoring");
    if (a->horizon < 1) return fail(M3PC_EINVAL, "m3pc_refine_plan: horizon %d < 1", a->horizon);
    if (a->flags & ~M3PC_PLAN_PRUNED_POLICY)
        return fail(M3PC_EINVAL, "m3pc_refine_plan: m3pc_plan_args::flags 0x%x holds more than M3PC_PLAN_PRUNED_POLICY", a->flags);
    if (r->iterations < 1 || r->iterations > M3PC_REFINE_MAX_ITER)
        return fail(M3PC_EINVAL, "m3pc_refine_plan: iterations %d outside [1, %d]", r->iterations, M3PC_REFINE_MAX_ITER);
    if (r->top_k < 1 || r->top_k > a->n_total) return fail(M3PC_EINVAL, "m3pc_refine_plan: top_k %d outside [1, n_total=%d]", r->top_k, a->n_total);
    CHK(refine_check_refit(r->weighting, r->temperature, r->min_std, "m3pc_refine_plan"));
    if (!finite_nonneg(r->init_std)) return fail(M3PC_EINVAL, "m3pc_refine_plan: init_std must be finite and >= 0");
    if (cert_any_begun(h)) return fail(M3PC_ESTATE, "m3pc_refine_plan with a pipelined step begun (m3pc_plan_step_certified_end first)");
    if (a->mode == M3PC_MODE_CRITIC && !h->critic_set) return fail(M3PC_ESTATE, "critic weights not set");
    const int N = a->n_total, k = r->top_k, T = h->T, hh = a->horizon;
    if (N > h->dm.max_candidates) return fail(M3PC_ENOMEM, "n_total %d > max_candidates %d", N, h->dm.max_candidates);
    if (hh > T) return fail(M3PC_EINVAL, "horizon %d outside [1, T=%d]", hh, T);
    hipStream_t st = (hipStream_t)stream;
    const int C = hh * h->A;
    const long long total = (long long)N * C;

    m3pc_plan_args pa = *a;
    pa.window = 0;
    CHK(m3pc_policy_pass(h, &pa, states, actions, rewards, nullptr, nullptr, stream));
    pa.flags = 0;

    const unsigned long long seed = ((unsigned long long)r->seed_hi << 32) | r->seed_lo, step = ((unsigned long long)r->step_hi << 32) | r->step_lo;
    auto noise_of = [&](int it) -> const float* {
        if (noise) return noise + (size_t)it * total;
        launch_variates(seed, step, 0, (long long)it * total, (long long)(it + 1) * total, h->refine_noise, st);
        return h->refine_noise;
    };
    ResampleP sp;
    memset(&sp, 0, sizeof(sp));
    sp.out = candidates;
    sp.total = (int)total;
    sp.C = C;
    sp.A = h->A;
    sp.mean = init_mean;
    sp.loc = h->loc + (size_t)(T - hh) * h->A;
    sp.std_const = r->init_std;
    sp.noise = noise_of(0);
    sp.mean_out = mean;
    sp.std_out = std_;
    launch_resample(sp, st);
    CHK(check_launch("refine_plan"));
    sp.mean_out = sp.std_out = nullptr;
    for (int it = 0; it < r->iterations; ++it) {
        float* er = scores ? scores + (size_t)it * N : h->refine_scores;
        int* top = elites ? elites + (size_t)it * k : h->refine_elites;
        CHK(m3pc_score_actions(h, &pa, 1, states, actions, rewards, candidates, nullptr, er, nullptr, nullptr, stream));
        launch_topk(er, N, k, top, st);
        RefitP rp;
        memset(&rp, 0, sizeof(rp));
        rp.cand = candidates;
        rp.elite = top;
        rp.scores = er;
        rp.n = N;
        rp.k = k;
        rp.C = C;
        rp.weighting = r->weighting;
        rp.tau = r->temperature;
        rp.min_std = r->min_std;
        rp.mean = mean + (size_t)(it + 1) * C;
        rp.std = std_ + (size_t)(it + 1) * C;
        launch_refit(rp, st);
        sp.mean = rp.mean;
        sp.std = rp.std;
        sp.noise = noise_of(it + 1);
        if (it == r->iterations - 1) {
            sp.sample_action = sample_action;
            sp.eval_action = eval_action;
        }
        launch_resample(sp, st);
        CHK(check_launch("refine_plan"));
    }
    return 0;
}

#ifdef M3PC_LAB
int m3pc_debug_step_streams_created(m3pc_handle* h) { return h ? h->step_streams_created : -1; }
int m3pc_debug_gemm(int dtype, const void* A, const void* Wt, const float* bias, const float* res, void* C, int M, int N,
                    int K, int gelu, int f32out, int variant, void* stream) {
    static const int ldpad = M3PC_ENV("M3PC_DEBUG_LDPAD") ? atoi(M3PC_ENV("M3PC_DEBUG_LDPAD")) : 0;
    GemmP p = gemm_basic(A, K + ldpad, Wt, K + ldpad, M, N, K, bias);
    p.a_padded = 0;
    p.gelu = gelu;
    p.res = res;
    p.ldr = N;
    p.variant = variant;
    if (dtype == DT_BF16 && !f32out)
        p.Cb = (bf16_t*)C;
    else
        p.Cf = (float*)C;
    p.ldc = N;
    if (dtype != DT_BF16 && variant != 1) {
        static float* ws = nullptr;
        if (!ws) HIPCHK(hipMalloc((void**)&ws, 64 << 20));
        p.ws = ws;
        p.ws_bytes = 64 << 20;
    }
    if (dtype == DT_X3) {
        static bf16_t* wsplit = nullptr;
        static size_t cap = 0;
        const size_t n = (size_t)N * (K + ldpad);
        if (n > cap) {
            if (wsplit) HIPCHK(hipFree(wsplit));
            wsplit = nullptr;
            cap = 0;
            HIPCHK(hipMalloc((void**)&wsplit, 2 * n * sizeof(bf16_t)));
            cap = n;
        }
        launch_f32_split_bf16((const float*)Wt, wsplit, wsplit + n, (long long)n, (hipStream_t)stream);
        p.W = wsplit;
        p.w_lo_off = (long long)n;
        if (launch_gemm_x3(p, (hipStream_t)stream) < 0) return fail(M3PC_EINVAL, "debug_gemm: shape not covered by the x3 kernel");
        return check_launch("debug_gemm");
    }
    launch_gemm(p, dtype, (hipStream_t)stream);
    return check_launch("debug_gemm");
}

static int debug_gemm_fill(const m3pc_debug_gemm_args* a, GemmP& p) {
    if (!a) return fail(M3PC_EINVAL, "debug_gemm_ex: null argument");
    const int dt = a->dtype;
    if (dt != DT_F32 && dt != DT_BF16 && dt != DT_X3) return fail(M3PC_EINVAL, "debug_gemm_ex: dtype %d", dt);
    if (!a->A || !a->W || !a->C) return fail(M3PC_EINVAL, "debug_gemm_ex: null operand");
    if (a->M < 1 || a->M > (1 << 20) || a->N < 32 || a->N > (1 << 16) || a->K < 1 || a->K > (1 << 16)) return fail(M3PC_EINVAL, "debug_gemm_ex: M / N / K out of range");
    const int es = dt == DT_BF16 ? 2 : 4;
    if (a->N % 32) return fail(M3PC_EINVAL, "debug_gemm_ex: N %d is not a multiple of 32 (columns would be dropped)", a->N);
    if (((long long)a->K * es) % 128) return fail(M3PC_EINVAL, "debug_gemm_ex: K %d is not a whole number of 128-byte k-tiles (k terms would be dropped)", a->K);
    if (dt == DT_F32 && !a->f32out) return fail(M3PC_EINVAL, "debug_gemm_ex: fp32 operands have fp32 output only");
    const int f32out = dt == DT_F32 || a->f32out;
    const int os = f32out ? 4 : 2;
    const uintptr_t ptrs = (uintptr_t)a->A | (uintptr_t)a->W | (uintptr_t)a->C | (uintptr_t)a->bias | (uintptr_t)a->rowtab | (uintptr_t)a->res |
                           (uintptr_t)a->ws | (uintptr_t)a->ln_g | (uintptr_t)a->ln_b | (uintptr_t)a->ln_out | (uintptr_t)a->a_ln_g |
                           (uintptr_t)a->a_ln_b;
    if (ptrs & 15) return fail(M3PC_EINVAL, "debug_gemm_ex: pointers must be 16-byte aligned");
    if (a->lda < a->K || a->ldw < a->K || a->ldc < a->N || (a->res && a->ldr < a->N) || (a->rowtab && a->rt_ld < a->N))
        return fail(M3PC_EINVAL, "debug_gemm_ex: a leading dimension is below its row length");
    if (((long long)a->lda * es) % 16 || ((long long)a->ldw * (dt == DT_F32 ? 4 : 2)) % 16 || (dt == DT_X3 && a->ldw % 4) || ((long long)a->ldc * os) % 16 ||
        (a->res && a->ldr % 4) || (a->rowtab && a->rt_ld % 4))
        return fail(M3PC_EINVAL, "debug_gemm_ex: rows of a leading dimension leave 16-byte alignment");
    if (a->rowtab && a->rt_mod < 1) return fail(M3PC_EINVAL, "debug_gemm_ex: rowtab with rt_mod %d", a->rt_mod);
    for (const int* m : {a->amap, a->cmap})
        if (m[0] < 0 || m[2] < 0 || (m[0] >= 1 && m[1] < m[0])) return fail(M3PC_EINVAL, "debug_gemm_ex: row map {%d, %d, %d}", m[0], m[1], m[2]);
    if (a->ws && a->ws_bytes < 0) return fail(M3PC_EINVAL, "debug_gemm_ex: negative ws_bytes");
    if (a->ln_out && (!f32out || !a->ln_g || !a->ln_b)) return fail(M3PC_EINVAL, "debug_gemm_ex: ln_out needs fp32 C, ln_g and ln_b");
    if ((a->a_ln_g != nullptr) != (a->a_ln_b != nullptr)) return fail(M3PC_EINVAL, "debug_gemm_ex: a_ln_g and a_ln_b go together");
    const int v = a->variant;
    if (!(v == 0 || (dt == DT_BF16 && (v == 2 || v == 26 || v == 37 || v == 43 || v == 44)) || (dt == DT_F32 && v == 2)))
        return fail(M3PC_EINVAL, "debug_gemm_ex: variant %d of dtype %d is not one this hook drives", v, dt);
    if (v == 44 && a->a_padded && a->M % 256 && 256 - a->M % 256 > 127)
        return fail(M3PC_EINVAL, "debug_gemm_ex: variant 44 with a_padded would read %d rows behind A", 256 - a->M % 256);
    p = gemm_basic(a->A, a->lda, a->W, a->ldw, a->M, a->N, a->K, a->bias);
    p.amap = RowMap{a->amap[0], a->amap[1], a->amap[2]};
    p.cmap = RowMap{a->cmap[0], a->cmap[1], a->cmap[2]};
    p.rowtab = a->rowtab;
    if (a->rowtab) {
        p.rt_mod = a->rt_mod;
        p.rt_ld = a->rt_ld;
    }
    p.gelu = a->gelu ? 1 : 0;
    p.res = a->res;
// ... 542 lines not shown
```

m3pc_amd/csrc/m3pc_internal.h:

```cpp
#pragma once
#include <math.h>
#include <stdarg.h>
#include <stdio.h>
#include <stdlib.h>
#include <string.h>

#include <algorithm>
#include <map>
#include <mutex>
#include <memory>
#include <string>
#include <vector>

#include "../../include/m3pc_hip.h"
#ifdef M3PC_LAB
#include "../../include/m3pc_hip_debug.h"
#endif
#include "kernels.h"

using namespace m3pc;

namespace m3pc {
extern thread_local char g_err[512];
int fail(int code, const char* fmt, ...);
// ... 58 lines not shown
    } query[N_QUERY];
};

struct EventPair {
    hipEvent_t a, b;
    double flops;
    int dt;
    int kind;
};

}


struct m3pc_handle {
    m3pc_dims dm;
    int device = 0;
    int d = 0, nh = 0, hd = 0, T = 0, S = 0, A = 0, ff = 0, feat[4] = {0, 0, 0, 0};
    std::map<std::string, Tensor> w;
    bool weights_loaded = false;
    long long load_stats[4] = {0, 0, 0, 0};
    float* WT[4] = {nullptr, nullptr, nullptr, nullptr};
    float* Eenc[4] = {nullptr, nullptr, nullptr, nullptr};
    float* Edec[4] = {nullptr, nullptr, nullptr, nullptr};
    float* mask_tokens = nullptr;
    bool tok_set[4] = {false, false, false, false};
    int tok_norm[4] = {0, 0, 0, 0};
    float* tok_mean[4] = {nullptr, nullptr, nullptr, nullptr};
    float* tok_std[4] = {nullptr, nullptr, nullptr, nullptr};
    std::vector<float> h_mean[4], h_std[4];
    bool critic_set = false;
    float *cW1T[2] = {nullptr, nullptr}, *cb1[2] = {nullptr, nullptr}, *cW2T[2] = {nullptr, nullptr},
          *cb2[2] = {nullptr, nullptr}, *cW3[2] = {nullptr, nullptr}, *cb3[2] = {nullptr, nullptr};
    float *cW1F[2] = {nullptr, nullptr}, *cW2F[2] = {nullptr, nullptr};
    float *c_om = nullptr, *c_os = nullptr;
    long long R = 0;
    float *X = nullptr, *Y = nullptr, *EncOut = nullptr, *G = nullptr;
    void *Hn = nullptr, *QKV = nullptr, *O = nullptr, *F = nullptr, *Z = nullptr;
    float *cand = nullptr, *loc = nullptr, *sd = nullptr, *rtok = nullptr, *pred[2] = {nullptr, nullptr}, *qv = nullptr;
    float* sel_scratch = nullptr;
    float* goal_ws = nullptr;
    int* d_topk = nullptr;
    float* er_top = nullptr;
    float* sa_buf = nullptr;
    float* sa_chain[2] = {nullptr, nullptr};
    float* refine_noise = nullptr;
    float* refine_scores = nullptr;
    int* refine_elites = nullptr;
    float* splitk_ws = nullptr;
    long long splitk_ws_bytes = 0;
    int* cert_list[M3PC_SLOTS] = {};
    float *cert_b[M3PC_SLOTS] = {}, *cert_f[M3PC_SLOTS] = {}, *cert_stats[M3PC_SLOTS] = {}, *cert_f32[M3PC_SLOTS] = {};
    int* cert_top1[M3PC_SLOTS] = {};
    float* cert_host = nullptr;
    float* cert_host_dev = nullptr;
    int cert_seq[M3PC_SLOTS] = {};
    struct CertStep {
        bool begun = false;
        bool tail_pending = false;
        bool async = false;
        unsigned long long order = 0;
        m3pc_plan_args a;
        m3pc_cert_args c;
        const float *states = nullptr, *actions = nullptr, *rewards = nullptr, *eps = nullptr, *expo = nullptr;
        float *sample_actions = nullptr, *scores_low = nullptr, *merged = nullptr, *p = nullptr, *eval_action = nullptr,
              *sample_action = nullptr;
        int *list = nullptr, *argmax = nullptr, *sample_idx = nullptr;
        hipStream_t tail = nullptr;
        double delta = 0.0;
        int rounds = 0, n_done = 0, r_done = 0;
        float seq = 0.f;
    } cstep[M3PC_SLOTS];
    hipStream_t step_chain[2] = {nullptr, nullptr};
    bool step_chain_own = false;
    int step_streams_created = 0;
    hipEvent_t step_ev[M3PC_SLOTS][4] = {};
    hipEvent_t ev_excl = nullptr;
    bool excl_valid = false;
    int cand_last_slot = -1;
    unsigned long long step_order = 0;
    struct Slot {
        float *loc = nullptr, *sd = nullptr, *rtok = nullptr;
        bool policy_valid = false;
        int n_windows = 0;
    } slot[M3PC_SLOTS];
    int cur_slot = 0;
    struct Base {
        float *X = nullptr, *Y = nullptr, *EncOut = nullptr, *G = nullptr, *cand = nullptr, *pred[2] = {nullptr, nullptr},
              *qv = nullptr, *splitk_ws = nullptr;
        char *Hn = nullptr, *QKV = nullptr, *O = nullptr, *F = nullptr, *Z = nullptr;
        long long splitk_ws_bytes = 0;
        float* head_part = nullptr;
        int* head_ticket = nullptr;
        int head_rows = 0;
        long long R = 0;
        int max_cand = 0;
    } base, chain[2], pchain[2];
    Base* cur = nullptr;
    bool two_stream = true;
    bool allow_splitk = true;
    bool x3 = false;
    std::vector<std::pair<const float*, Tensor*>> gemm_w;
    double pass_scale = 1.0;
    hipStream_t aux = nullptr;
    hipEvent_t ev_fork = nullptr, ev_join = nullptr;
    const int* score_scatter_index = nullptr;
    float* score_scatter_out = nullptr;
    std::vector<hipStream_t> auxs;
    std::vector<hipEvent_t> ev_joins;
    std::vector<int> stream_split;
    hipEvent_t slot_join[M3PC_SLOTS][3] = {};
    int slot_join_n[M3PC_SLOTS] = {};
    hipEvent_t aux_tail[3] = {};
    bool aux_unjoined[3] = {false, false, false};
    std::vector<int> defer_parts;
    std::map<std::string, std::unique_ptr<Plan>> plans;
    Plan* mask_plan[4][65] = {};
    std::map<std::string, bf16_t*> wstream;
    bf16_t* kvstream[4] = {nullptr, nullptr, nullptr, nullptr};
    long long* stamp_log = nullptr;
    int stamp_cap = 0, stamp_i = 0;
    bool prof = false;
    bool prof_serial = false;
    std::vector<EventPair> ev;
    size_t ev_used = 0;
};

namespace m3pc {


template <typename T>
inline int dmalloc(T** p, size_t n) {
    hipError_t e = hipMalloc((void**)p, n * sizeof(T) > 0 ? n * sizeof(T) : 16);
    if (e != hipSuccess) return fail(M3PC_EHIP, "hipMalloc(%zu bytes) failed: %s", n * sizeof(T), hipGetErrorString(e));
    return 0;
}

inline int check_launch(const char* what) {
    hipError_t e = hipGetLastError();
    if (e != hipSuccess) return fail(M3PC_EHIP, "kernel launch failed in %s: %s", what, hipGetErrorString(e));
    return 0;
}

inline void set_view(m3pc_handle* h, int c0, int ) {
    const size_t rows = (size_t)c0 * 2 * h->T, d = (size_t)h->d;
    const m3pc_handle::Base& b = *h->cur;
    h->X = b.X + rows * d;
    h->Y = b.Y + rows * d;
    h->EncOut = b.EncOut + rows * d;
    h->G = b.G + rows * d;
    h->Hn = b.Hn + rows * d * 4;
    h->QKV = b.QKV + rows * 3 * d * 4;
    h->O = b.O + rows * d * 4;
    h->F = b.F + rows * 4 * d * 4;
    h->Z = b.Z + rows * d * 4;
    h->cand = b.cand + (size_t)c0 * h->T * h->A;
    h->pred[0] = b.pred[0] + (size_t)c0 * h->T * 32;
    h->pred[1] = b.pred[1] + (size_t)c0 * h->T * 32;
    h->qv = b.qv + (size_t)c0 * h->T;
    const long long half = b.splitk_ws_bytes / 2;
    h->splitk_ws = c0 == 0 ? b.splitk_ws : b.splitk_ws + half / 4;
    h->splitk_ws_bytes = half;
}

inline void bind_ws(m3pc_handle* h, m3pc_handle::Base* b) {
    h->cur = b;
    h->R = b->R;
    set_view(h, 0, b->max_cand);
}
struct WsScope {
    m3pc_handle* h;
    WsScope(m3pc_handle* h_, bool chain, bool policy = false, int slot = 0) : h(h_) {
        if (chain) bind_ws(h, policy ? &h->pchain[slot & 1] : &h->chain[slot & 1]);
    }
    ~WsScope() { bind_ws(h, &h->base); }
};
struct X3Scope {
    m3pc_handle* h;
    bool prev;
    X3Scope(m3pc_handle* h_, bool on) : h(h_), prev(h_->x3) { h->x3 = on; }
    ~X3Scope() { h->x3 = prev; }
};
// ... 131 lines not shown
        }
        e = &h->ev[h->ev_used++];
        e->flops = flops;
        e->dt = dt;
        e->kind = kind;
        hipEventRecord(e->a, st);
    }
    ~GemmTimer() {
        if (e) hipEventRecord(e->b, st);
    }
};

inline Tensor* x3_weight(m3pc_handle* h, const void* w) {
    const float* f = (const float*)w;
    auto it = std::upper_bound(h->gemm_w.begin(), h->gemm_w.end(), f,
                               [](const float* a, const std::pair<const float*, Tensor*>& e) { return a < e.first; });
    if (it == h->gemm_w.begin()) return nullptr;
    --it;
    return f < it->first + it->second->numel ? it->second : nullptr;
}

inline int gemm(m3pc_handle* h, const GemmP& p_in, int dt, hipStream_t st) {
    GemmP p = p_in;
    p.ws = h->allow_splitk ? h->splitk_ws : nullptr;
    p.ws_bytes = h->splitk_ws_bytes;
    if (h->x3 && dt == DT_F32 && p.K >= 32) {
        if (Tensor* t = x3_weight(h, p.W)) {
            p.W = t->b + ((const float*)p.W - t->f);
            p.w_lo_off = t->numel;
            GemmTimer t3(h, st, 2.0 * p.M * (double)p.N * p.K, DT_X3);
            const int rc = launch_gemm_x3(p, st);
            if (rc >= 0) return rc;
            p = p_in;
            p.ws = h->allow_splitk ? h->splitk_ws : nullptr;
            p.ws_bytes = h->splitk_ws_bytes;
        }
    }
#ifdef M3PC_LAB
    static const int env_variant = M3PC_ENV("M3PC_GEMM_VARIANT") ? atoi(M3PC_ENV("M3PC_GEMM_VARIANT")) : 0;
    if (env_variant) p.variant = env_variant;
#endif
    GemmTimer t(h, st, 2.0 * p.M * (double)p.N * p.K, dt);
    return launch_gemm(p, dt, st);
}

inline bool can_fold_ln(m3pc_handle* h, const GemmP& p, int dt) {
    static const bool on = M3PC_ENV("M3PC_LN_FOLD") != nullptr && M3PC_ENV("M3PC_NO_F32_DIRECT") == nullptr &&
                           M3PC_ENV("M3PC_GEMM_VARIANT") == nullptr;
    return dt == DT_F32 && on && h->allow_splitk && h->splitk_ws && gemm_f32_direct_covers(p);
}

inline GemmP gemm_basic(const void* A, int lda, const void* Wp, int ldw, int M, int N, int K, const float* bias) {
    GemmP p;
    memset(&p, 0, sizeof(p));
    p.A = A;
    p.lda = lda;
    p.W = Wp;
    p.ldw = ldw;
    p.M = M;
    p.N = N;
    p.K = K;
    p.bias = bias;
    p.rt_mod = 1;
    p.a_padded = 1;
    return p;
}
inline void gemm_out(GemmP& p, int dt_out, void* C, int ldc) {
    if (dt_out == DT_BF16)
        p.Cb = (bf16_t*)C;
    else
        p.Cf = (float*)C;
    p.ldc = ldc;
}

constexpr long long FUSED_MIN_ROWS = 96 * 128;
constexpr long long SPLIT_MIN_ROWS = 16 * 128;

struct TokIn {
    const float* ptr[4];
    long long bstride[4];
    int normalize[4];
    const int* widx = nullptr;
    long long wstride[4] = {0, 0, 0, 0};
};

struct PieceState {
    bool ln = true, qkv = false;
};

enum { TAIL_HEADS = 0, TAIL_X = 1 };

int get_plan(m3pc_handle* h, const unsigned char* const masks[4], Plan** out);
int get_mask_plan(m3pc_handle* h, int kind, int idx, Plan** out);
int ensure_edec(m3pc_handle* h, Plan* pl, hipStream_t st);
void free_tables(SharedTables& t);
void invalidate_tables(m3pc_handle* h);
int build_query_list(m3pc_handle* h, Plan* pl, int qi, int hh, const std::vector<int>& toks, int n_groups, int key0, int key1);
int build_query(m3pc_handle* h, Plan* pl, int qi, int hh);
int build_tables(m3pc_handle* h, Plan* pl, int qi, int dt, hipStream_t st);
int run_block(m3pc_handle* h, const std::string& pfx, float* X, int batch, int L, int dt, hipStream_t st, bool ln1_done = false,
              int n_sh = 0, const LnP* next_ln = nullptr, bool* next_ln_done = nullptr, bool x_dead = false,
              float* Xnext = nullptr, int res_nshared = 0, bool qkv_done = false, const std::string* next_qkv = nullptr,
              bool* next_qkv_done = nullptr, bool x_bf16 = false);
int run_encoder(m3pc_handle* h, Plan* pl, const TokIn& in, int batch, int dt, hipStream_t st, bool bf16_out_only = false,
                int n_indep = 0, int layer_from = 0, int layer_to = 1 << 30, PieceState* ln_state = nullptr);
void dec_embed(m3pc_handle* h, int k, const void* Zop, RowMap amap, float* Yout, RowMap cmap, int M, int mod, int dt,
               hipStream_t st, const float* table = nullptr);
int run_decoder_full(m3pc_handle* h, const void* Zop, int batch, int dt, hipStream_t st);
int run_head(m3pc_handle* h, int k, const float* Ysrc, RowMap xmap, int rows, float* out, int ldy, bool detok, int dt,
             hipStream_t st);
int run_head_tail(m3pc_handle* h, int k, const void* ln_rows, int rows, float* out, int ldy, bool detok, int dt, hipStream_t st);
int forward_impl(m3pc_handle* h, Plan* pl, const TokIn& in, int batch, float* out_states, float* out_rewards,
                 float* out_returns, float* out_mu, float* out_std, int dt, hipStream_t st);
int pruned_decoder(m3pc_handle* h, Plan* pl, Plan::Query& q, SharedTables& tb, int n, int dt, hipStream_t st, int tail,
                   float** xrows);
int candidate_pass(m3pc_handle* h, const m3pc_plan_args* a, const float* states, const float* rewards, int n,
                   const float* sample_actions, float* expect_return, float* pred_rewards, float* pred_boot, int dt,
                   hipStream_t st, const int* widx = nullptr, int stage_from = 0, int stage_to = 1 << 30, PieceState* ln_state = nullptr);

}
```

m3pc_amd/csrc/m3pc_passes.hip:

```cpp
#include "m3pc_internal.h"

namespace m3pc {


int run_block(m3pc_handle* h, const std::string& pfx, float* X, int batch, int L, int dt, hipStream_t st, bool ln1_done,
              int n_sh, const LnP* next_ln, bool* next_ln_done, bool x_dead,
              float* Xnext, int res_nshared, bool qkv_done, const std::string* next_qkv,
              bool* next_qkv_done, bool x_bf16) {
    const int d = h->d, ff = h->ff;
    const int rows = batch * L;
    const int es = (int)dtype_size(dt);
    (void)es;
    LnP ln;
    memset(&ln, 0, sizeof(ln));
    ln.X = X;
    ln.ldx = d;
    ln.rows = rows;
    ln.d = d;
    ln.g1 = W(h, pfx + ".norm1.weight").f;
    ln.b1 = W(h, pfx + ".norm1.bias").f;
    if (dt == DT_BF16)
        ln.Yb = (bf16_t*)h->Hn;
    else
        ln.Yf = (float*)h->Hn;
    GemmP pqkv = gemm_basic(h->Hn, d, Wop(h, pfx + ".self_attn.in_proj_weight", dt), d, rows, 3 * d, d,
                            W(h, pfx + ".self_attn.in_proj_bias").f);
    gemm_out(pqkv, dt, h->QKV, 3 * d);
    if (!ln1_done && n_sh == 0) {
        GemmP t = pqkv;
        t.A = X;
        t.a_ln_g = ln.g1;
        t.a_ln_b = ln.b1;
        if (can_fold_ln(h, t, dt)) {
            pqkv = t;
            ln1_done = true;
        }
    }
    if (!ln1_done && !qkv_done) launch_layernorm(ln, st);
    if (n_sh > 0) {
        const int n_own = L - n_sh;
        const size_t es2 = dtype_size(dt);
        char* hn_sh = (char*)h->Hn + (size_t)batch * n_own * d * es2;
        char* qkv_sh = (char*)h->QKV + (size_t)batch * n_own * 3 * d * es2;
        {
            GemmP p = gemm_basic(h->Hn, d, Wop(h, pfx + ".self_attn.in_proj_weight", dt), d, batch * n_own, 3 * d, d,
                                 W(h, pfx + ".self_attn.in_proj_bias").f);
            gemm_out(p, dt, h->QKV, 3 * d);
            gemm(h, p, dt, st);
        }
        {
            GemmP p = gemm_basic(hn_sh, d, Wop(h, pfx + ".self_attn.in_proj_weight", dt), d, n_sh, 3 * d, d,
                                 W(h, pfx + ".self_attn.in_proj_bias").f);
            gemm_out(p, dt, qkv_sh, 3 * d);
            gemm(h, p, dt, st);
        }
        AttnP a;
        memset(&a, 0, sizeof(a));
        const char* q = (const char*)h->QKV;
        a.Q = q;
        a.q_bstride = (long long)n_own * 3 * d;
        a.ldq = 3 * d;
        a.Lq = n_own;
        a.orow1 = n_sh;
        a.Q2 = qkv_sh;
        a.ldq2 = 3 * d;
        a.Lq2 = n_sh;
        a.orow2 = 0;
        a.K1 = q + (size_t)d * es2;
        a.V1 = q + (size_t)2 * d * es2;
        a.kv1_bstride = (long long)n_own * 3 * d;
        a.ldkv1 = 3 * d;
        a.L1 = n_own;
        a.K2 = qkv_sh + (size_t)d * es2;
        a.V2 = qkv_sh + (size_t)2 * d * es2;
        a.ldkv2 = 3 * d;
        a.L2 = n_sh;
        a.O = h->O;
        a.o_bstride = (long long)L * d;
        a.ldo = d;
        a.batch = batch;
        a.n_head = h->nh;
        a.hd = h->hd;
        a.scale = 1.0f / sqrtf((float)h->hd);
        launch_attention(a, dt, st);
    } else {
    if (!qkv_done) gemm(h, pqkv, dt, st);
    {
        AttnP a;
        memset(&a, 0, sizeof(a));
        const char* q = (const char*)h->QKV;
        a.Q = q;
        a.q_bstride = (long long)L * 3 * d;
        a.ldq = 3 * d;
        a.K1 = q + (size_t)d * dtype_size(dt);
        a.V1 = q + (size_t)2 * d * dtype_size(dt);
        a.kv1_bstride = (long long)L * 3 * d;
        a.ldkv1 = 3 * d;
        a.L1 = L;
        a.O = h->O;
        a.o_bstride = (long long)L * d;
        a.ldo = d;
        a.batch = batch;
        a.n_head = h->nh;
        a.hd = h->hd;
        a.Lq = L;
        a.scale = 1.0f / sqrtf((float)h->hd);
        launch_attention(a, dt, st);
    }
    }
    static const bool no_fused = M3PC_ENV("M3PC_NO_BLOCK_FUSED") != nullptr;
    static const bool no_split = M3PC_ENV("M3PC_NO_BLOCK_SPLIT") != nullptr;
    const double step_rows = (double)rows * h->pass_scale;
    if (x_bf16 && (ln1_done == false && !qkv_done)) return fail(M3PC_EINVAL, "%s: norm1 of a bf16 residual stream has no kernel", pfx.c_str());
    if (dt == DT_BF16 && !no_fused && !no_split && step_rows < (double)FUSED_MIN_ROWS && step_rows >= (double)SPLIT_MIN_ROWS && !x_bf16 &&
        h->wstream.count(pfx) && !Xnext && !res_nshared && (long long)rows * block_split_n() * d <= h->R * 4LL * d) {
        BlockP b;
        memset(&b, 0, sizeof(b));
        b.O = (const bf16_t*)h->O;
        b.ldo = d;
        b.M = rows;
        b.res = X;
        b.ldr = d;
        b.wstream = h->wstream[pfx];
        b.bo = W(h, pfx + ".self_attn.out_proj.bias").f;
        b.b1 = W(h, pfx + ".linear1.bias").f;
        b.b2 = W(h, pfx + ".linear2.bias").f;
        b.ln2_g = W(h, pfx + ".norm2.weight").f;
        b.ln2_b = W(h, pfx + ".norm2.bias").f;
        b.split = 1;
        b.Xout = (float*)h->F;
        b.ldx = d;
        const bool fuse_ln = next_ln && next_ln->Yb && !next_ln->Yf && !next_ln->g2 && next_ln->X == X && next_ln->xmap.rpg == 0 &&
                             next_ln->rows == rows;
// ... 45 lines not shown
        static const bool no_qkv_fused = M3PC_ENV("M3PC_NO_QKV_FUSED") != nullptr;
        const bool fuse_qkv = fuse_ln && next_qkv && !no_qkv_fused && next_ln->Yb == (bf16_t*)h->Hn &&
                              (size_t)rows * 3 * d * 2 < 0x7fffffffull;
        if (fuse_qkv) {
            b.lnA_g = next_ln->g1;
            b.lnA_b = next_ln->b1;
            b.QKVout = (bf16_t*)h->QKV;
            b.ldq = 3 * d;
            b.qkv_bytes = (unsigned)((size_t)rows * 3 * d * 2);
            b.bqkv = W(h, *next_qkv + ".self_attn.in_proj_bias").f;
        } else if (fuse_ln) {
            b.lnA_g = next_ln->g1;
            b.lnA_b = next_ln->b1;
            b.Hout = next_ln->Yb;
            b.ldh = d;
        }
        if (next_qkv_done) *next_qkv_done = fuse_qkv;
        if (!(fuse_ln && x_dead)) {
            b.Xout = Xnext ? Xnext : X;
            b.ldx = d;
        }
        if (h->stamp_log) {
            b.stamps = h->stamp_log + 64 * (h->stamp_i++ % h->stamp_cap);
            b.stamp_block = 37;
        }
        GemmTimer t(h, st, 2.0 * rows * ((double)d * d + 2.0 * d * ff + (fuse_qkv ? 3.0 * d * d : 0.0)), dt, 1);
        if (x_bf16 && !(fuse_ln && (fuse_qkv || x_dead)))
            return fail(M3PC_EINVAL, "%s: a bf16 residual stream needs the consumer of the block output inside the tail", pfx.c_str());
        if (launch_block_fused(b, st)) {
            if (next_ln_done) *next_ln_done = fuse_ln;
            return check_launch(pfx.c_str());
        }
        if (next_qkv_done) *next_qkv_done = false;
    }
    if (Xnext || res_nshared || x_bf16) return fail(M3PC_EINVAL, "%s: the fused layer tail did not take a pass set up for it", pfx.c_str());
    {
        GemmP p = gemm_basic(h->O, d, Wop(h, pfx + ".self_attn.out_proj.weight", dt), d, rows, d, d,
                             W(h, pfx + ".self_attn.out_proj.bias").f);
        p.res = X;
        p.ldr = d;
        gemm_out(p, DT_F32, X, d);
        ln.g1 = W(h, pfx + ".norm2.weight").f;
        ln.b1 = W(h, pfx + ".norm2.bias").f;
        GemmP p1 = gemm_basic(h->Hn, d, Wop(h, pfx + ".linear1.weight", dt), d, rows, ff, d, W(h, pfx + ".linear1.bias").f);
        p1.gelu = 1;
        gemm_out(p1, dt, h->F, ff);
        GemmP t = p1;
        t.A = X;
        t.a_ln_g = ln.g1;
        t.a_ln_b = ln.b1;
        if (can_fold_ln(h, t, dt)) {
            gemm(h, p, dt, st);
            gemm(h, t, dt, st);
        } else {
            if (dt == DT_F32) {
                p.ln_g = ln.g1;
                p.ln_b = ln.b1;
                p.ln_out = ln.Yf;
            }
            if (!gemm(h, p, dt, st)) launch_layernorm(ln, st);
            gemm(h, p1, dt, st);
        }
    }
    {
        GemmP p = gemm_basic(h->F, ff, Wop(h, pfx + ".linear2.weight", dt), ff, rows, d, ff, W(h, pfx + ".linear2.bias").f);
        p.res = X;
        p.ldr = d;
        gemm_out(p, DT_F32, X, d);
        if (dt == DT_F32 && next_ln && next_ln->Yf && !next_ln->Yb && !next_ln->g2 && next_ln->X == X && next_ln->xmap.rpg == 0 &&
            next_ln->rows == rows) {
            p.ln_g = next_ln->g1;
            p.ln_b = next_ln->b1;
            p.ln_out = next_ln->Yf;
        }
        const int done = gemm(h, p, dt, st);
        if (next_ln_done) *next_ln_done = done != 0;
    }
    return check_launch(pfx.c_str());
}


int run_encoder(m3pc_handle* h, Plan* pl, const TokIn& in, int batch, int dt, hipStream_t st, bool bf16_out_only,
                int n_indep, int layer_from, int layer_to, PieceState* ln_state) {
    int n_sh = 0;
    static const bool no_prune1 = M3PC_ENV("M3PC_NO_PRUNE1") != nullptr;
    if (dt == DT_BF16 && batch >= 64 && h->d % 256 == 0 && h->d <= 1024 && n_indep >= 32 && !no_prune1)
        n_sh = (n_indep / 32) * 32;
    EmbedP e;
    memset(&e, 0, sizeof(e));
    e.n_indep = n_indep;
    e.n_sh = n_sh;
    e.Hb_sh = n_sh ? (bf16_t*)((char*)h->Hn + (size_t)batch * (pl->Le - n_sh) * h->d * 2) : nullptr;
    for (int k = 0; k < 4; ++k) {
        e.tok[k] = in.ptr[k];
        e.bstride[k] = in.bstride[k];
        e.wstride[k] = in.wstride[k];
        e.normalize[k] = in.normalize[k];
        e.mean[k] = h->tok_mean[k];
        e.stdv[k] = h->tok_std[k];
        e.WT[k] = h->WT[k];
        e.E[k] = h->Eenc[k];
        e.feat[k] = h->feat[k];
    }
    static const bool shared_res_on = M3PC_ENV("M3PC_SHARED_RES") != nullptr && M3PC_ENV("M3PC_NO_BLOCK_FUSED") == nullptr;
    const bool shared_res = n_sh > 0 && shared_res_on && (long long)batch * pl->Le >= 512 && h->wstream.count("encoder.layers.0") &&
                            bf16_out_only;
    static const bool no_xb16 = M3PC_ENV("M3PC_NO_BF16_RESIDUAL") != nullptr;
    static const bool no_fused_env = M3PC_ENV("M3PC_NO_BLOCK_FUSED") != nullptr || M3PC_ENV("M3PC_NO_QKV_FUSED") != nullptr;
    bool xb16 = dt == DT_BF16 && bf16_out_only && !shared_res && !no_xb16 && !no_fused_env && block_fused_supported(h->d, h->ff) &&
                (double)batch * pl->Le * h->pass_scale >= (double)FUSED_MIN_ROWS && (size_t)batch * pl->Le * 3 * h->d * 2 < 0x7fffffffull &&
                (unsigned long long)batch * pl->Le * h->d * 2 < 0x80000000ull;
    for (int i = 0; i < h->dm.n_enc_layer && xb16; ++i) xb16 = h->wstream.count("encoder.layers." + std::to_string(i)) != 0;
    e.x_first_only = shared_res ? 1 : 0;
    if (xb16) e.Xb = (bf16_t*)h->X;
    e.widx = in.widx;
    e.tokmap = pl->d_tokmap;
    e.batch = batch;
    e.L = pl->Le;
    e.d = h->d;
    e.T = h->T;
    e.X = h->X;
    e.ln_g = W(h, "encoder.layers.0.norm1.weight").f;
    e.ln_b = W(h, "encoder.layers.0.norm1.bias").f;
    if (dt == DT_BF16)
        e.Hb = (bf16_t*)h->Hn;
    else
        e.Hf = (float*)h->Hn;
    if (layer_from <= 0) launch_embed(e, st);
    LnP ln;
    memset(&ln, 0, sizeof(ln));
    ln.X = h->X;
    ln.ldx = h->d;
    ln.rows = batch * pl->Le;
    ln.d = h->d;
    ln.g1 = W(h, "encoder.norm.weight").f;
    ln.b1 = W(h, "encoder.norm.bias").f;
    if (bf16_out_only)
        ln.Yb = (bf16_t*)h->Z;
    else
        ln.Yf = h->EncOut;
    bool ln_done = layer_from <= 0 || !ln_state ? true : ln_state->ln;
    bool qkv_done = layer_from <= 0 || !ln_state ? false : ln_state->qkv;
    const int nl = h->dm.n_enc_layer;
    float* Xs = shared_res && layer_from > 0 ? h->Y : h->X;
    for (int i = layer_from > 0 ? layer_from : 0; i < nl && i < layer_to; ++i) {
        float* Xn = shared_res && i == 0 ? h->Y : nullptr;
        LnP nxt = ln;
        nxt.X = ln.X = Xn ? Xn : Xs;
        if (i + 1 < nl) {
            nxt.g1 = W(h, "encoder.layers." + std::to_string(i + 1) + ".norm1.weight").f;
            nxt.b1 = W(h, "encoder.layers." + std::to_string(i + 1) + ".norm1.bias").f;
            nxt.Yb = dt == DT_BF16 ? (bf16_t*)h->Hn : nullptr;
            nxt.Yf = dt == DT_F32 ? (float*)h->Hn : nullptr;
        }
        const bool l1 = ln_done;
        ln_done = false;
        const std::string nq = "encoder.layers." + std::to_string(i + 1);
        const bool q1 = qkv_done;
        qkv_done = false;
        CHK(run_block(h, "encoder.layers." + std::to_string(i), Xs, batch, pl->Le, dt, st, l1, i == 0 ? n_sh : 0, &nxt, &ln_done,
                      i + 1 == nl && bf16_out_only, Xn, Xn ? n_indep : 0, q1, i + 1 < nl ? &nq : nullptr, &qkv_done, xb16));
        if (Xn) Xs = Xn;
    }
    if (ln_state) {
        ln_state->ln = ln_done;
        ln_state->qkv = qkv_done;
    }
    if (layer_to < nl) return check_launch("encoder");
    ln.X = Xs;
    if (!ln_done) launch_layernorm(ln, st);
    return check_launch("encoder");
}

void dec_embed(m3pc_handle* h, int k, const void* Zop, RowMap amap, float* Yout, RowMap cmap, int M, int mod, int dt,
               hipStream_t st, const float* table) {
    const int d = h->d;
    const std::string kn = KEYN[k];
    GemmP p = gemm_basic(Zop, d, Wop(h, "decoder_embed_dict." + kn + ".weight", dt), d, M, d, d, nullptr);
    p.amap = amap;
    p.cmap = cmap;
    p.rowtab = table ? table : h->Edec[k];
    p.rt_mod = mod;
    p.rt_ld = d;
    gemm_out(p, DT_F32, Yout, d);
    gemm(h, p, dt, st);
}

int run_decoder_full(m3pc_handle* h, const void* Zop, int batch, int dt, hipStream_t st) {
    const int T = h->T, d = h->d;
    bool grouped = false;
    static const bool no_group = M3PC_ENV("M3PC_NO_GEMM_GROUP") != nullptr || M3PC_ENV("M3PC_NO_F32_DIRECT") != nullptr ||
                                 M3PC_ENV("M3PC_GEMM_VARIANT") != nullptr;
    if (dt == DT_F32 && !no_group && h->allow_splitk) {
        GemmP ps[4];
        for (int k = 0; k < 4; ++k) {
            RowMap m{T, 4 * T, k * T};
            ps[k] = gemm_basic(Zop, d, Wop(h, std::string("decoder_embed_dict.") + KEYN[k] + ".weight", dt), d, batch * T, d, d, nullptr);
            ps[k].amap = m;
            ps[k].cmap = m;
            ps[k].rowtab = h->Edec[k];
            ps[k].rt_mod = T;
            ps[k].rt_ld = d;
            gemm_out(ps[k], DT_F32, h->Y, d);
        }
        GemmTimer t(h, st, 4 * 2.0 * batch * T * (double)d * d, dt);
        grouped = launch_gemm_f32_direct_group(ps, 4, st);
    }
    for (int k = 0; k < 4 && !grouped; ++k) {
        RowMap m{T, 4 * T, k * T};
        dec_embed(h, k, Zop, m, h->Y, m, batch * T, T, dt, st);
    }
    for (int i = 0; i < h->dm.n_dec_layer; ++i) CHK(run_block(h, "decoder.layers." + std::to_string(i), h->Y, batch, 4 * T, dt, st));
    return check_launch("decoder");
}

int run_head_tail(m3pc_handle* h, int k, const void* ln_rows, int rows, float* out, int ldy, bool detok, int dt, hipStream_t st);

int run_head(m3pc_handle* h, int k, const float* Ysrc, RowMap xmap, int rows, float* out, int ldy, bool detok, int dt,
             hipStream_t st) {
    const int d = h->d;
    const std::string kn = KEYN[k];
    LnP ln;
    memset(&ln, 0, sizeof(ln));
    ln.X = Ysrc;
    ln.ldx = d;
    ln.xmap = xmap;
    ln.rows = rows;
    ln.d = d;
    ln.g1 = W(h, "decoder.norm.weight").f;
    ln.b1 = W(h, "decoder.norm.bias").f;
    ln.g2 = W(h, "output_head_dict." + kn + ".0.weight").f;
    ln.b2 = W(h, "output_head_dict." + kn + ".0.bias").f;
    if (dt == DT_BF16)
        ln.Yb = (bf16_t*)h->Hn;
    else
        ln.Yf = (float*)h->Hn;
    launch_layernorm(ln, st);
    return run_head_tail(h, k, h->Hn, rows, out, ldy, detok, dt, st);
}

int run_head_tail(m3pc_handle* h, int k, const void* ln_rows, int rows, float* out, int ldy, bool detok, int dt, hipStream_t st) {
    const int d = h->d;
    const std::string kn = KEYN[k];
    GemmP p = gemm_basic(ln_rows, d, Wop(h, "output_head_dict." + kn + ".1.weight", dt), d, rows, d, d,
// ... 402 lines not shown
            p.ldr = d;
        }
        gemm_out(p, DT_F32, Y1, d);
        ln.X = Y1;
        ln.rows = n * nq;
        ln.g1 = W(h, pfx + ".norm2.weight").f;
        ln.b1 = W(h, pfx + ".norm2.bias").f;
        GemmP p1 = gemm_basic(h->Hn, d, Wop(h, pfx + ".linear1.weight", dt), d, n * nq, h->ff, d, W(h, pfx + ".linear1.bias").f);
        p1.gelu = 1;
        gemm_out(p1, dt, h->F, h->ff);
        GemmP t = p1;
        t.A = Y1;
        t.a_ln_g = ln.g1;
        t.a_ln_b = ln.b1;
        if (can_fold_ln(h, t, dt)) {
            gemm(h, p, dt, st);
            gemm(h, t, dt, st);
        } else {
            if (dt == DT_F32) {
                p.ln_g = ln.g1;
                p.ln_b = ln.b1;
                p.ln_out = ln.Yf;
            }
            if (!gemm(h, p, dt, st)) launch_layernorm(ln, st);
            gemm(h, p1, dt, st);
        }
    }
    {
        GemmP p = gemm_basic(h->F, h->ff, Wop(h, pfx + ".linear2.weight", dt), h->ff, n * nq, d, h->ff, W(h, pfx + ".linear2.bias").f);
        p.res = Y1;
        p.ldr = d;
        gemm_out(p, DT_F32, Y1, d);
        gemm(h, p, dt, st);
    }
    bool heads_done = false;
    {
        static const bool no_head_f32 = M3PC_ENV("M3PC_NO_HEAD_F32_FUSED") != nullptr || M3PC_ENV("M3PC_NO_F32_DIRECT") != nullptr;
        bool scalar = tail == TAIL_HEADS && dt == DT_F32 && h->allow_splitk && !no_head_f32 && h->cur && h->cur->head_part &&
                      n * hh <= h->cur->head_rows && q.n_groups >= 1 && q.n_groups <= 2;
        for (int s = 0; s < q.n_groups && scalar; ++s) scalar = h->feat[q.qkeys[s]] == 1 && q.qkeys[s] != M3PC_ACTIONS;
        if (scalar) {
            HeadFusedP hp;
            memset(&hp, 0, sizeof(hp));
            hp.X = Y1;
            hp.ldx = d;
            hp.rows = n * hh;
            hp.d = d;
            hp.n_heads = q.n_groups;
            hp.grp = hh;
            hp.row_mod = nq;
            hp.gA = W(h, "decoder.norm.weight").f;
            hp.bA = W(h, "decoder.norm.bias").f;
            for (int s = 0; s < q.n_groups; ++s) {
                const std::string hn = std::string("output_head_dict.") + KEYN[q.qkeys[s]];
                hp.gB[s] = W(h, hn + ".0.weight").f;
                hp.bB[s] = W(h, hn + ".0.bias").f;
                hp.W1[s] = W(h, hn + ".1.weight").f;
                hp.b1[s] = W(h, hn + ".1.bias").f;
                hp.w2[s] = W(h, hn + ".3.weight").f;
                hp.b2[s] = W(h, hn + ".3.bias").f;
                if (h->tok_norm[q.qkeys[s]]) {
                    hp.mean[s] = h->tok_mean[q.qkeys[s]];
                    hp.stdv[s] = h->tok_std[q.qkeys[s]];
                }
                hp.out[s] = h->pred[s];
            }
            hp.part = h->cur->head_part;
            hp.ticket = h->cur->head_ticket;
            GemmTimer t(h, st, q.n_groups * 2.0 * n * hh * (double)d * d, dt);
            heads_done = launch_head_f32_fused(hp, st);
        }
    }
    for (int s = 0; s < q.n_groups && tail == TAIL_HEADS && !heads_done; ++s) {
        RowMap xm{hh, nq, s * hh};
        CHK(run_head(h, q.qkeys[s], Y1, xm, n * hh, h->pred[s], h->feat[q.qkeys[s]], true, dt, st));
    }
    }
    const int rc = check_launch("pruned_decoder");
    if (rc != 0 && h->cur && h->cur->head_ticket)
        (void)hipMemsetAsync(h->cur->head_ticket, 0, (size_t)2 * ((h->cur->head_rows + 31) / 32) * sizeof(int), st);
    return rc;
}

int candidate_pass(m3pc_handle* h, const m3pc_plan_args* a, const float* states, const float* rewards, int n,
                   const float* sample_actions, float* expect_return, float* pred_rewards, float* pred_boot, int dt,
                   hipStream_t st, const int* widx, int stage_from, int stage_to, PieceState* ln_state) {
    const int T = h->T, d = h->d, hh = a->horizon, idx = T - hh;
    const size_t es = dtype_size(dt);
    struct ScaleScope {
        m3pc_handle* h;
        ~ScaleScope() { h->pass_scale = 1.0; }
    } scale_scope{h};
    h->pass_scale = !widx && a->n_total > n ? (double)a->n_total / (double)n : 1.0;
    Plan* pl = nullptr;
    CHK(get_mask_plan(h, 1, idx, &pl));
    const int qi = a->mode == M3PC_MODE_RTG ? 0 : 1;
    CHK(build_query(h, pl, qi, hh));
    CHK(build_tables(h, pl, qi, dt, st));
    Plan::Query& q = pl->query[qi];
    SharedTables& tb = q.tab[dt];
    const int Le = pl->Le, nq = q.nq;
    if ((long long)n * Le > h->R || (long long)n * nq > h->R) return fail(M3PC_ENOMEM, "n_count %d exceeds workspace", n);

    TokIn in;
    memset(&in, 0, sizeof(in));
    in.ptr[M3PC_STATES] = states;
    in.normalize[M3PC_STATES] = h->tok_norm[M3PC_STATES];
    in.ptr[M3PC_ACTIONS] = h->cand;
    in.bstride[M3PC_ACTIONS] = (long long)T * h->A;
    in.normalize[M3PC_ACTIONS] = h->tok_norm[M3PC_ACTIONS];
    in.ptr[M3PC_REWARDS] = rewards;
    in.ptr[M3PC_RETURNS] = h->rtok;
    in.widx = widx;
    in.wstride[M3PC_STATES] = (long long)T * h->S;
    in.wstride[M3PC_REWARDS] = T;
    const int nl_enc = h->dm.n_enc_layer;
    if (stage_from < nl_enc) CHK(run_encoder(h, pl, in, n, dt, st, dt == DT_BF16, widx ? 0 : (idx + 1) + idx, stage_from, stage_to, ln_state));
    if (stage_to <= nl_enc) return check_launch("candidate_pass");

    CHK(pruned_decoder(h, pl, q, tb, n, dt, st, TAIL_HEADS, nullptr));
    const float* rw;
    const float* boot;
    float boot_scale;
    if (a->mode == M3PC_MODE_RTG) {
        rw = h->pred[0];
        boot = h->pred[1];
        boot_scale = 1000.0f;
    } else {
        if (!h->critic_set) return fail(M3PC_ESTATE, "critic weights not set");
        CriticP c;
        memset(&c, 0, sizeof(c));
        c.states = h->pred[0];
        c.actions = sample_actions;
        c.rows = n * hh;
        c.S = h->S;
        c.A = h->A;
        c.hidden = h->dm.critic_hidden;
        c.om = h->c_om;
        c.os = h->c_os;
        for (int i = 0; i < 2; ++i) {
            c.W1T[i] = h->cW1T[i];
            c.b1[i] = h->cb1[i];
            c.W2T[i] = h->cW2T[i];
            c.b2[i] = h->cb2[i];
            c.W3[i] = h->cW3[i];
            c.b3[i] = h->cb3[i];
            c.W1F[i] = h->cW1F[i];
            c.W2F[i] = h->cW2F[i];
        }
        c.q = h->qv;
        launch_critic(c, st);
        rw = h->pred[1];
        boot = h->qv;
        boot_scale = 1.0f;
    }
    ScoreP sc;
    memset(&sc, 0, sizeof(sc));
    sc.rewards = rw;
    sc.boot = boot;
    sc.n = n;
    sc.h = hh;
    sc.boot_scale = boot_scale;
    sc.gamma = (float)a->discount;
    sc.lmbda = a->lmbda;
    sc.expect_return = expect_return;
    sc.boot_out = pred_boot;
    sc.scatter_index = h->score_scatter_index;
    sc.scatter_out = h->score_scatter_out;
    launch_score(sc, st);
    if (pred_rewards) HIPCHK(hipMemcpyAsync(pred_rewards, rw, (size_t)n * hh * sizeof(float), hipMemcpyDeviceToDevice, st));
    return check_launch("candidate_pass");
}


}
```

m3pc_amd/planner.py:

```python
from __future__ import annotations

import types
from typing import Dict, Optional

import contextlib
import warnings

import numpy as np

import torch

from . import capi, dist as mdist
from .certificate import RACE_MAX, _TicketOps, resolve as _resolve_certificate
from .goal import GoalMixin
from .lockstep import LockstepMixin
from .tokenizers import ContinuousTokenizer, DataStatistics, SquashedNormal, TokenizerManager

KEYS = capi.KEYS
_MODES = {"rtg_guiding": capi.MODE_RTG, "critic_lambda_guiding": capi.MODE_CRITIC,
          "noise_adding_lambda": capi.MODE_NOISE}


_CHAIN_STREAMS = {}

# ... 275 lines not shown

    def _step_expo(self, step: int, buf=None):
        if self._variates != "library":
            return self._draw_expo() if buf is None else buf.exponential_(1, generator=self.generator)
        N = int(self.cfg.action_samples)
        out = buf if buf is not None else torch.empty((N,), dtype=torch.float32, device=self.device)
        self.handle.draw_variates(self._seed, step, N, 1, expo=out, want_eps=False)
        return out

    def _chain_streams(self):
        if self._chain is None:
            key = (str(self.device), self._chain_priority)
            if key not in _CHAIN_STREAMS:
                _CHAIN_STREAMS[key] = (torch.cuda.Stream(device=self.device, priority=self._chain_priority),
                                       torch.cuda.Stream(device=self.device, priority=self._chain_priority))
            self._chain, t = _CHAIN_STREAMS[key]
            self._tchain = t if self._tail_stream else self._chain
        return self._chain, self._tchain

    def _streams_of(self, sl):
        a, b = self._chain_streams()
        if self._alternate and self._tail_stream:
            c = (a, b)[sl.i & 1]
            return c, c
        return a, b

    def _acquire_slot(self):
        sl = self._slots[self._next_slot]
        self._next_slot = (self._next_slot + 1) % len(self._slots)
        if sl.owner is not None:
            self._finish(sl.owner)
        return sl

    def _drain(self):
        for tk in [sl.owner for sl in self._slots if sl.owner is not None and sl.owner.chain is not None]:
            self._finish(tk)

    def _mark_main(self):
        if self._ev_main is None:
            self._ev_main = torch.cuda.Event()
        self._ev_main.record(torch.cuda.current_stream(self.device))

    def _guide(self, mode: int, states, actions, rewards, rtg: float, h: int, lmbda: float, eps=None, returns=None):
        return self._issue(mode, states, actions, rewards, rtg, h, lmbda, eps=eps, returns=returns, pipelined=False).result()

    def _issue(self, mode: int, states, actions, rewards, rtg: float, h: int, lmbda: float, eps=None, returns=None,
               pipelined: bool = True, slot=None, inputs_ready: bool = False) -> "PlanTicket":
        cfg = self.cfg
        N, T, A = int(cfg.action_samples), self.T, self.A
        if self._auto_fp32 and not self.fp32_fallback:
            self._maybe_fall_back_to_fp32()
        if not pipelined:
            self._drain()
        if (self._native_step and not pipelined and slot is None and self.world == 1 and not self._force_collective
                and not self._bf16_offset and self.rescore in ("bound", "none")):
            return self._issue_native(mode, states, actions, rewards, rtg, h, lmbda, eps, returns)
        if (self._native_step and pipelined and self.world == 1 and not self._force_collective and not self._bf16_offset
                and self.rescore in ("bound", "none") and self._alternate and self._tail_stream and self._defer_join):
            return self._issue_native_async(mode, states, actions, rewards, rtg, h, lmbda, eps, returns, slot, inputs_ready)
        sl = (slot if slot is not None else self._acquire_slot()).ready(self)
        tk = PlanTicket(self, sl, mode, states, actions, rewards, float(rtg), int(h), float(lmbda), returns)
        sl.owner = tk
        tk.index, self._step_index = self._step_index, self._step_index + 1
        tk.grow_in, tk.kfirst_in, tk.rfirst_in = self._adapt(tk.index)
        main = torch.cuda.current_stream(self.device)
        chain, tchain = self._streams_of(sl) if pipelined else (None, None)
        tk.chain = chain
        tk.tchain = tchain
        hd = self.handle
        tk.outbuf = hd.select_buffers(N)
        if self.rescore != "none":
            tk.er = torch.empty((N,), dtype=torch.float32, device=self.device)
            tk.R = self._R
            tk.lst = torch.empty((tk.R + 1024,), dtype=torch.int32, device=self.device)
            tk.top = tk.lst[tk.R :]
        with (torch.cuda.stream(chain) if chain is not None else contextlib.nullcontext()):
            if chain is not None and not inputs_ready:
                sl.ev_in.record(main)
                chain.wait_event(sl.ev_in)
            if chain is not None:
                chain.wait_event(sl.ev_done)
                if self._ev_main is not None:
                    chain.wait_event(self._ev_main)
            hd.policy_pass(mode, states, actions, rewards, h, tk.rtg, slot=sl.i, returns=returns, pruned=self._policy_pruned)
            if eps is None:
                eps = self._step_eps(tk.index, mode, h, sl.eps_buf if chain is not None else None)
            tk.eps = eps = eps.reshape(N, -1, A)
            tk.expo = self._step_expo(tk.index, sl.expo_buf if chain is not None else None)
            if chain is not None:
                sl.ev_pol.record(chain)
        if chain is not None and self._alternate:
            for old in [o for o in self._pending if o.tchain is chain]:
                self._pending.remove(old)
                self._enqueue_tail(old)
        if chain is not None:
            main.wait_event(sl.ev_pol)
        begin, count = mdist.shard_range(N, self.rank, self.world)
        tk.deferred = bool(chain is not None and self.world == 1 and not self._force_collective and not self._bf16_offset
                           and self._defer_join)
        res = hd.candidate_pass(mode, states, actions, rewards, eps, h, tk.lmbda, float(cfg.discount), N, begin, count,
                                precision=self.precision, slot=sl.i, defer_join=tk.deferred)
        er, a0 = res["expect_return"], res["sample_actions"][:, 0]
        er, a0 = mdist.gather_candidates(er, a0, N, self.group, force=self._force_collective)
        if self._bf16_offset and self.precision in capi.LOW_PRECISION:
            er = er + self._bf16_offset
        tk.res, tk.er_b, tk.a0 = res, er, a0
        if chain is not None:
            sl.ev_cand.record(main)
            if not self._alternate:
                for old in self._pending:
                    self._enqueue_tail(old)
                self._pending = []
            self._pending.append(tk)
        else:
            self._enqueue_tail(tk)
            self._mark_main()
        return tk

    def _issue_native(self, mode: int, states, actions, rewards, rtg: float, h: int, lmbda: float, eps=None, returns=None,
                      slot=None) -> "PlanTicket":
        cfg, hd = self.cfg, self.handle
        N, A = int(cfg.action_samples), self.A
        sl = (slot if slot is not None else self._acquire_slot()).ready(self)
        tk = PlanTicket(self, sl, mode, states, actions, rewards, float(rtg), int(h), float(lmbda), returns)
        tk.index, self._step_index = self._step_index, self._step_index + 1
        tk.grow_in, tk.kfirst_in, tk.rfirst_in = self._adapt(tk.index)
        if eps is None:
            eps = self._step_eps(tk.index, mode, h)
        tk.eps = eps = eps.reshape(N, -1, A)
        tk.expo = self._step_expo(tk.index)
        disc, temp = float(cfg.discount), float(cfg.temperature)
        bound = self.rescore == "bound"
        R = self._R if bound else 0
        kmin = kmax = rfirst = 1
        delta = 0.0
        if bound:
            if self._delta_fixed is None and self._cal_left > 0:
                self._cal_left -= 1
                hd.policy_pass(mode, states, actions, rewards, h, tk.rtg, slot=sl.i, returns=returns, pruned=self._policy_pruned)
                low = hd.candidate_pass(mode, states, actions, rewards, eps, h, tk.lmbda, disc, N, precision=self.precision,
                                        slot=sl.i)["expect_return"]
                d = hd.calibrate_delta(mode, states, actions, rewards, eps, low, h, tk.lmbda, disc, N,
                                       factor=self.calibration_factor, slot=sl.i)
                self._delta0 = d if self._delta0 is None else max(self._delta0, d)
            kmax = max(min(self.rescore_max, N - 1 if N > 1 else 1, 1024 - self._R - 1), 1)
            kmin = max(min(tk.kfirst_in, N, kmax), 1)
            rfirst = max(min(tk.rfirst_in, R), 1) if R > 0 else 0
            delta = max(self._delta0, tk.grow_in)
        res, rec = hd.plan_step_certified(mode, states, actions, rewards, eps, tk.expo, h, tk.rtg, tk.lmbda, disc, N, temp,
                                          delta=delta, grow_delta=bound and self._delta_fixed is None, kmin=kmin, kmax=kmax,
                                          rfirst=rfirst, rmax=R, precision=self.precision, slot=sl.i, returns=returns,
                                          pruned=self._policy_pruned)
        self._mark_main()
        return self._native_result(tk, res, rec, delta, kmin, kmax)

    def _native_result(self, tk, res, rec, delta, kmin, kmax) -> "PlanTicket":
        N = int(self.cfg.action_samples)
        bound = self.rescore == "bound"
        R = self._R if bound else 0
        extra = {}
        top = None
        if bound:
            lst = res["list"]
            if rec.delta > float(np.float32(delta)):
                self.delta_grown += 1
            if rec.saturated and not self._warned_saturated:
                self._warned_saturated = True
                warnings.warn(f"m3pc_amd: the certificates asked for more candidates than the step lists (delta={rec.delta:.3g}, "
                              f"rescore_max={self.rescore_max}); the whole window set or every candidate was re-scored in fp32 (slow path)")
            top = torch.arange(N, dtype=torch.int32, device=self.device) if rec.everything else lst[R : R + rec.n_rescored]
            extra = dict(n_rescored=int(rec.n_rescored), n_in_window=int(rec.need_first), min_margin_outside=float(rec.margin),
                         delta=float(rec.delta), saturated=bool(rec.saturated), shift=float(rec.shift), deviation=float(rec.deviation),
                         n_race=int(rec.n_race), need_race=int(rec.need_race_first), certified=bool(rec.certified),
                         n_first=kmin, n_race_first=min(max(tk.rfirst_in, 1), R), race=lst[R - rec.n_race : R], rounds=int(rec.rounds))
            tk.delta = extra["delta"]
            self._hist[tk.index] = (float(rec.deviation), min(int(rec.need_first), kmax), min(int(rec.need_race_first), R),
                                    int(rec.n_rescored) + int(rec.n_race))
            for i in [i for i in self._hist if i < tk.index - 64]:
                if self._delta_fixed is None:
                    self._delta0 = max(self._delta0, 1.5 * self._hist[i][0])
                del self._hist[i]
        p, eval_action, argmax, sample_idx, sample_action = tk.sel = res["sel"]
        self.last = dict(expect_return=res["expect_return"] if bound else res["expect_return_low"],
                         expect_return_bf16=res["expect_return_low"] if bound else None, p=p, argmax=argmax, sample_idx=sample_idx,
                         loc=res["loc"], std=res["std"], sample_actions=res["sample_actions"], eps=tk.eps, topk=top,
                         eval_action=eval_action, sample_action=sample_action, horizon=tk.h, expo=tk.expo, **extra)
        tk.tail_enqueued = True
        tk.info = self.last
        tk.out = (sample_action, eval_action)
        return tk

    def _issue_native_async(self, mode: int, states, actions, rewards, rtg: float, h: int, lmbda: float, eps, returns, slot,
                            inputs_ready: bool) -> "PlanTicket":
        cfg, hd = self.cfg, self.handle
        N, A = int(cfg.action_samples), self.A
        sl = (slot if slot is not None else self._acquire_slot()).ready(self)
        bound = self.rescore == "bound"
        main = torch.cuda.current_stream(self.device)
        if bound and self._delta_fixed is None and self._cal_left > 0:
            self._drain()
            if inputs_ready:
                main.wait_event(sl.ev_h2d)
            tk = self._issue_native(mode, states, actions, rewards, rtg, h, lmbda, eps, returns, slot=sl)
            sl.ev_done.record(main)
            return tk
        chain, _ = self._streams_of(sl)
        if not self._step_streams_set:
            self._drain()
            hd.set_step_streams(*self._chain_streams())
            self._step_streams_set = True
        tk = PlanTicket(self, sl, mode, states, actions, rewards, float(rtg), int(h), float(lmbda), returns)
        sl.owner = tk
        tk.native = True
        tk.chain = tk.tchain = chain
        tk.index, self._step_index = self._step_index, self._step_index + 1
        tk.grow_in, tk.kfirst_in, tk.rfirst_in = self._adapt(tk.index)
        if inputs_ready and self._ev_main is not None:
            chain.wait_event(self._ev_main)
        if eps is None:
            eps = self._step_eps(tk.index, mode, h, sl.eps_buf)
        tk.eps = eps = eps.reshape(N, -1, A)
        tk.expo = self._step_expo(tk.index, sl.expo_buf)
# ... 404 lines not shown
```

Baseline: 873.4 plan-steps/s.

## Fuse sampling into embed, precompute shared first-layer QKV rows, join scoring across parts

Folds candidate action sampling into the embedding kernel so the separate sample launch and its round trip through memory go away. During the policy pass it precomputes the first encoder layer's embedding and QKV projection for the rows shared by all candidates, and reuses them in the candidate pass when the slot's states and actions match. Scoring is deferred so the two-stream parts write into per-slot joined buffers and are scored once, not per part. Each is on by default and can be turned off with an environment switch. The cost is extra per-slot buffers and cache-validity logic keyed on pointer identity, which could go stale if a buffer is reused with new contents.

New measurement: 868.2 plan-steps/s. No clear change (-0.6%).

```diff
diff --git a/include/m3pc_hip_debug.h b/include/m3pc_hip_debug.h
--- a/include/m3pc_hip_debug.h
+++ b/include/m3pc_hip_debug.h
@@ -80,6 +80,8 @@
                          void* stream);
 int m3pc_debug_stamp_log(m3pc_handle* h, int cap, long long* out, int* n_logged);
 int m3pc_debug_step_streams_created(m3pc_handle* h);
+int m3pc_debug_candidate_switches(void);
+int m3pc_debug_shared_rows(int d, int bf16, int batch, int n_indep);
 int m3pc_debug_xcc_probe(int* out, int n_blocks, void* stream);
 
 #ifdef __cplusplus
diff --git a/m3pc_amd/capi.py b/m3pc_amd/capi.py
--- a/m3pc_amd/capi.py
+++ b/m3pc_amd/capi.py
@@ -355,8 +355,8 @@
         return a
 
     def policy_pass(self, mode: int, states, actions, rewards, horizon: int, rtg: float, slot: int = 0, returns=None,
-                    loc=None, std=None, pruned: bool = False):
-        args = self._args(mode, PREC_FP32, horizon, 1, 0, 1, 0.0, 0.0, rtg, slot, returns)
+                    loc=None, std=None, pruned: bool = False, n_total: int = 1, precision: int = PREC_FP32):
+        args = self._args(mode, precision, horizon, max(int(n_total), 1), 0, 1, 0.0, 0.0, rtg, slot, returns)
         if pruned and loc is None and std is None:
             args.flags = PLAN_PRUNED_POLICY
         check(self.lib.m3pc_policy_pass(self._h, C.byref(args), _ptr(self._f32(states)), _ptr(self._f32(actions)),
diff --git a/m3pc_amd/csrc/elementwise.hip b/m3pc_amd/csrc/elementwise.hip
--- a/m3pc_amd/csrc/elementwise.hip
+++ b/m3pc_amd/csrc/elementwise.hip
@@ -1,3 +1,5 @@
+#include <string.h>
+
 #include "kernels.h"
 
 namespace m3pc {
@@ -16,6 +18,20 @@
 #pragma unroll
     for (int o = 32; o > 0; o >>= 1) v = fmaxf(v, __shfl_xor(v, o));
     return v;
+}
+
+__device__ __forceinline__ float sample_value(const SampleP& p, long long n, int t, int a) {
+    if (t < p.idx) return p.hist_actions[(p.widx ? (long long)p.widx[n] * p.T * p.A : 0) + t * p.A + a];
+    const int ta = t * p.A + a;
+    const long long src = p.index ? (long long)p.index[n] : p.n_begin + n;
+    if (p.mode == 2) return p.eps[(src * p.h + (t - p.idx)) * p.A + a];
+    if (p.mode == 0) {
+        const float e = p.eps[(src * p.T + t) * p.A + a];
+        return tanhf(__fadd_rn(__fmul_rn(e, p.sd[ta]), p.loc[ta]));
+    }
+    const float e = p.eps[(src * p.h + (t - p.idx)) * p.A + a];
+    const float v = __fadd_rn(tanhf(p.loc[ta]), __fmul_rn(e, 0.09f));
+    return fminf(fmaxf(v, -0.99999f), 0.99999f);
 }
 
 __global__ __launch_bounds__(256) void embed_kernel(EmbedP p) {
@@ -83,12 +99,18 @@
         }
     }
 }
-template <int NV>
-__global__ __launch_bounds__(256) void embed_rows_kernel(EmbedP p, int CB, int nchunk) {
+template <int NV, bool SMP>
+__global__ __launch_bounds__(256) void embed_rows_kernel(EmbedP p, int CB, int nchunk, SampleP sp) {
     const int lane = threadIdx.x & 63;
     const int w = blockIdx.x * 4 + (threadIdx.x >> 6);
-    if (w >= p.L * nchunk) return;
+    if (w >= (p.sh_only ? p.n_sh : p.L) * nchunk) return;
     const int j = w / nchunk, ch = w % nchunk;
+    if (SMP && w == 0) {
+        for (int x = lane; x < sp.T * sp.A; x += 64) {
+            if (sp.loc_out && sp.loc) sp.loc_out[x] = sp.loc[x];
+            if (sp.sd_out && sp.sd) sp.sd_out[x] = sp.sd[x];
+        }
+    }
     const int2 kt = p.tokmap[j];
     const int key = kt.x, t = kt.y;
     const int D = p.feat[key], d = p.d;
@@ -96,7 +118,8 @@
     const float* E = p.E[key] + (long long)t * d;
     const bool indep = j < p.n_indep;
     const int b0 = ch * CB, b1 = b0 + CB < p.batch ? b0 + CB : p.batch;
-    if (indep && p.x_first_only && b0 > 0 && p.Hb && !p.Hf && j < p.n_sh) return;
+    const bool draws = SMP && key == 1;
+    if (indep && p.x_first_only && b0 > 0 && p.Hb && !p.Hf && j < p.n_sh && !draws) return;
     const int n_own = p.L - p.n_sh;
     float4 ev[NV], gv[NV], bv[NV];
 #pragma unroll
@@ -110,12 +133,18 @@
     }
     float4 x[NV], y[NV];
     for (int b = b0; b < b1; ++b) {
+        float av = 0.f;
+        if (draws && lane < D) {
+            av = sample_value(sp, b, t, lane);
+            sp.cand[((long long)b * sp.T + t) * sp.A + lane] = av;
+            if (t >= sp.idx && sp.sample_actions) sp.sample_actions[((long long)b * sp.h + (t - sp.idx)) * sp.A + lane] = av;
+        }
         if (b == b0 || !indep) {
             const float* xin = p.tok[key] + (long long)b * p.bstride[key] + (p.widx ? (long long)p.widx[b] * p.wstride[key] : 0) + (long long)t * D;
 #pragma unroll
             for (int i = 0; i < NV; ++i) x[i] = make_float4(0.f, 0.f, 0.f, 0.f);
             for (int f = 0; f < D; ++f) {
-                float xf = xin[f];
+                float xf = draws ? __shfl(av, f) : xin[f];
                 if (p.normalize[key]) xf = (xf - p.mean[key][f]) / p.stdv[key][f];
 #pragma unroll
                 for (int i = 0; i < NV; ++i) {
@@ -154,7 +183,7 @@
             }
         }
         const long long row = (long long)b * p.L + j;
-        if (!(indep && p.x_first_only && b > 0)) {
+        if (!(indep && p.x_first_only && b > 0) && !p.sh_only) {
             if (p.Xb) {
 #pragma unroll
                 for (int i = 0; i < NV; ++i) {
@@ -182,7 +211,7 @@
                 dst = p.Hb + row * d;
             else if (j >= p.n_sh)
                 dst = p.Hb + ((long long)b * n_own + (j - p.n_sh)) * d;
-            else if (b == 0)
+            else if (b == 0 && !p.sh_skip)
                 dst = p.Hb_sh + (long long)j * d;
             else
                 continue;
@@ -200,22 +229,34 @@
     }
 }
 
-void launch_embed(const EmbedP& p, hipStream_t st) {
+bool embed_fuses_sample(int d) { return d % 256 == 0 && d <= 1024; }
+void launch_embed(const EmbedP& p, hipStream_t st, const SampleP* smp) {
     const long long rows = (long long)p.batch * p.L;
     if (rows <= 0) return;
+    if (smp && !(embed_fuses_sample(p.d) && !p.widx && !p.sh_only)) {
+        launch_sample(*smp, st);
+        smp = nullptr;
+    }
     if (p.d % 256 == 0 && p.d <= 1024) {
         int CB = p.batch / 64;
         CB = CB < 1 ? 1 : (CB > 16 ? 16 : CB);
         if (p.n_indep == 0 && CB > 4) CB = 4;
         const int nchunk = (p.batch + CB - 1) / CB;
-        const int waves = p.L * nchunk;
+        const int waves = (p.sh_only ? p.n_sh : p.L) * nchunk;
         const dim3 grid((waves + 3) / 4), block(256);
+        SampleP sp;
+        memset(&sp, 0, sizeof(sp));
+        if (smp) sp = *smp;
+#define M3PC_EMBED_ROWS(NV)                                                                                        \
+    if (smp) hipLaunchKernelGGL((embed_rows_kernel<NV, true>), grid, block, 0, st, p, CB, nchunk, sp);           \
+    else hipLaunchKernelGGL((embed_rows_kernel<NV, false>), grid, block, 0, st, p, CB, nchunk, sp)
         switch (p.d / 256) {
-            case 1: hipLaunchKernelGGL(embed_rows_kernel<1>, grid, block, 0, st, p, CB, nchunk); break;
-            case 2: hipLaunchKernelGGL(embed_rows_kernel<2>, grid, block, 0, st, p, CB, nchunk); break;
-            case 3: hipLaunchKernelGGL(embed_rows_kernel<3>, grid, block, 0, st, p, CB, nchunk); break;
-            default: hipLaunchKernelGGL(embed_rows_kernel<4>, grid, block, 0, st, p, CB, nchunk); break;
-        }
+            case 1: M3PC_EMBED_ROWS(1); break;
+            case 2: M3PC_EMBED_ROWS(2); break;
+            case 3: M3PC_EMBED_ROWS(3); break;
+            default: M3PC_EMBED_ROWS(4); break;
+        }
+#undef M3PC_EMBED_ROWS
         return;
     }
     hipLaunchKernelGGL(embed_kernel, dim3((unsigned)rows), dim3(p.d < 256 ? p.d : 256), 0, st, p);
@@ -692,24 +733,8 @@
         const int a = (int)(x % p.A);
         const int t = (int)((x / p.A) % p.T);
         const long long n = x / ((long long)p.A * p.T);
-        float v;
-        if (t < p.idx) {
-            v = p.hist_actions[(p.widx ? (long long)p.widx[n] * p.T * p.A : 0) + t * p.A + a];
-        } else {
-            const int ta = t * p.A + a;
-            const long long src = p.index ? (long long)p.index[n] : p.n_begin + n;
-            if (p.mode == 2) {
-                v = p.eps[(src * p.h + (t - p.idx)) * p.A + a];
-            } else if (p.mode == 0) {
-                const float e = p.eps[(src * p.T + t) * p.A + a];
-                v = tanhf(__fadd_rn(__fmul_rn(e, p.sd[ta]), p.loc[ta]));
-            } else {
-                const float e = p.eps[(src * p.h + (t - p.idx)) * p.A + a];
-                v = __fadd_rn(tanhf(p.loc[ta]), __fmul_rn(e, 0.09f));
-                v = fminf(fmaxf(v, -0.99999f), 0.99999f);
-            }
-            if (p.sample_actions) p.sample_actions[(n * p.h + (t - p.idx)) * p.A + a] = v;
-        }
+        const float v = sample_value(p, n, t, a);
+        if (t >= p.idx && p.sample_actions) p.sample_actions[(n * p.h + (t - p.idx)) * p.A + a] = v;
         p.cand[x] = v;
     }
 }
diff --git a/m3pc_amd/csrc/kernels.h b/m3pc_amd/csrc/kernels.h
--- a/m3pc_amd/csrc/kernels.h
+++ b/m3pc_amd/csrc/kernels.h
@@ -270,8 +270,12 @@
     int x_first_only;
     int n_sh;
     bf16_t* Hb_sh;
-};
-void launch_embed(const EmbedP& p, hipStream_t st);
+    int sh_only;
+    int sh_skip;
+};
+struct SampleP;
+void launch_embed(const EmbedP& p, hipStream_t st, const SampleP* smp = nullptr);
+bool embed_fuses_sample(int d);
 
 struct GatherP {
     const float* Xe;
diff --git a/m3pc_amd/csrc/m3pc.hip b/m3pc_amd/csrc/m3pc.hip
--- a/m3pc_amd/csrc/m3pc.hip
+++ b/m3pc_amd/csrc/m3pc.hip
@@ -33,6 +33,11 @@
 
 const char* m3pc_last_error(void) { return g_err; }
 int m3pc_abi_version(void) { return M3PC_ABI_VERSION; }
+
+static int candidate_switches() {
+    return (M3PC_ENV("M3PC_NO_SAMPLE_FUSED") == nullptr ? 1 : 0) | (M3PC_ENV("M3PC_NO_SHARED_PRE") == nullptr ? 2 : 0) |
+           (M3PC_ENV("M3PC_NO_SCORE_JOINED") == nullptr ? 4 : 0);
+}
 
 int m3pc_create(const m3pc_dims* dims, int device, m3pc_handle** out) {
     if (!dims || !out) return fail(M3PC_EINVAL, "null argument");
@@ -103,6 +108,8 @@
         CHK(dmalloc(&h->slot[s].loc, (size_t)D.max_batch * T * h->A + 64));
         CHK(dmalloc(&h->slot[s].sd, (size_t)D.max_batch * T * h->A + 64));
         CHK(dmalloc(&h->slot[s].rtok, (size_t)D.max_batch * T));
+        CHK(dmalloc(&h->slot[s].sh_hn, (size_t)2 * 2 * T * h->d));
+        CHK(dmalloc(&h->slot[s].sh_qkv, (size_t)2 * T * 3 * h->d));
     }
     CHK(dmalloc(&h->sel_scratch, 64));
     CHK(dmalloc(&h->d_topk, 1024));
@@ -152,6 +159,10 @@
         for (int i = 0; i < 3; ++i) HIPCHK(hipEventCreateWithFlags(&h->slot_join[s][i], hipEventDisableTiming));
     for (int i = 0; i < 3; ++i) HIPCHK(hipEventCreateWithFlags(&h->aux_tail[i], hipEventDisableTiming));
     if (const char* e = M3PC_ENV("M3PC_TWO_STREAM")) h->two_stream = atoi(e) != 0;
+    const int sw = candidate_switches();
+    h->fuse_sample = (sw & 1) != 0;
+    h->pre_shared = (sw & 2) != 0;
+    h->join_score = (sw & 4) != 0;
     h->auxs.push_back(h->aux);
     h->ev_joins.push_back(h->ev_join);
     if (const char* e = M3PC_ENV("M3PC_STREAM_SPLIT")) {
@@ -215,6 +226,10 @@
         hipFree(h->slot[s].loc);
         hipFree(h->slot[s].sd);
         hipFree(h->slot[s].rtok);
+        hipFree(h->slot[s].sh_hn);
+        hipFree(h->slot[s].sh_qkv);
+        for (float* b : {h->slot[s].jpred[0], h->slot[s].jpred[1], h->slot[s].jqv})
+            if (b) hipFree(b);
     }
     void* bufs[] = {h->sel_scratch, h->d_topk, h->er_top, h->sa_buf, h->sa_chain[0], h->sa_chain[1], h->c_om, h->c_os, h->goal_ws,
                     h->refine_noise, h->refine_scores, h->refine_elites};
@@ -364,6 +379,7 @@
     for (int sl = 0; sl < M3PC_SLOTS; ++sl) {
         h->slot[sl].policy_valid = false;
         h->slot[sl].n_windows = 0;
+        h->slot[sl].sh_idx = -1;
     }
     HIPCHK(hipStreamSynchronize(st));
     h->weights_loaded = true;
@@ -386,6 +402,7 @@
     h->h_std[key].assign(std_, std_ + dim);
     h->tok_norm[key] = normalize ? 1 : 0;
     h->tok_set[key] = true;
+    for (int sl = 0; sl < M3PC_SLOTS; ++sl) h->slot[sl].sh_idx = -1;
     return 0;
 }
 
@@ -499,6 +516,7 @@
     bind_slot(h, 0);
     h->slot[0].policy_valid = false;
     h->slot[0].n_windows = 0;
+    h->slot[0].sh_idx = -1;
     CHK(fill_rtok(h, rtg, batch, st));
     TokIn in;
     memset(&in, 0, sizeof(in));
@@ -672,6 +690,7 @@
     CHK(plan_check(h, a, false));
     hipStream_t st = (hipStream_t)stream;
     const int T = h->T, hh = a->horizon, idx = T - hh;
+    h->slot[a->slot].sh_idx = -1;
     if (a->returns) {
         launch_tokenize(a->returns, a->returns_f64, h->rtok, T, 1, h->tok_mean[M3PC_RETURNS], h->tok_std[M3PC_RETURNS],
                         h->tok_norm[M3PC_RETURNS], st);
@@ -748,6 +767,7 @@
     if (rc) return rc;
     h->slot[a->slot].policy_valid = true;
     h->slot[a->slot].n_windows = 1;
+    CHK(precompute_shared_rows(h, a, states, actions, st));
     if (loc) HIPCHK(hipMemcpyAsync(loc, h->loc, (size_t)T * h->A * sizeof(float), hipMemcpyDeviceToDevice, st));
     if (std_) HIPCHK(hipMemcpyAsync(std_, h->sd, (size_t)T * h->A * sizeof(float), hipMemcpyDeviceToDevice, st));
     return check_launch("policy_pass");
@@ -771,7 +791,7 @@
     bind_ws(h, &h->base);
     h->allow_splitk = false;
 
-    auto sample = [&](int c0, int cnt, hipStream_t s) {
+    auto sample_args = [&](int c0, int cnt) {
         SampleP sp;
         memset(&sp, 0, sizeof(sp));
         sp.hist_actions = actions;
@@ -791,13 +811,27 @@
             sp.loc_out = loc;
             sp.sd_out = std_;
         }
-        launch_sample(sp, s);
+        return sp;
     };
 
     const int dt = pass_dt(a->precision);
     X3Scope x3(h, a->precision == M3PC_PREC_BF16X3);
     const int n = a->n_count;
     h->slot_join_n[a->slot] = 0;
+    m3pc_handle::Slot& sl = h->slot[a->slot];
+    sl.score_pending = false;
+    const bool fuse_sample = h->fuse_sample && dt == DT_BF16 && embed_fuses_sample(h->d);
+    const bool sh_ok = h->pre_shared && dt == DT_BF16 && sl.sh_idx == idx && sl.sh_states == states && sl.sh_actions == actions &&
+                       a->window == 0 && sl.n_windows == 1;
+    auto extras = [&](int cnt, const SampleP* sp) {
+        PassExtras ex;
+        ex.sample = fuse_sample ? sp : nullptr;
+        if (sh_ok && first_layer_shared_rows(h->d, dt, cnt, candidate_n_indep(idx)) == sl.sh_n) {
+            ex.sh_qkv = sl.sh_qkv;
+            ex.sh_n = sl.sh_n;
+        }
+        return ex;
+    };
     if (h->two_stream && dt == DT_BF16 && n >= 512 && (long long)n * (2 * T - hh + 1) > 256 * 128) {
         std::vector<int> parts;
         if (!h->stream_split.empty()) {
@@ -816,21 +850,54 @@
         if (!(defer && parts == h->defer_parts)) CHK(ws_sync(h, st));
         HIPCHK(hipEventRecord(h->ev_fork, st));
         int rc = 0;
+        const bool join_score = h->join_score && !h->prof_serial && !pred_rewards && !pred_boot;
+        float *jpred[2] = {h->base.pred[0], h->base.pred[1]}, *jqv = h->base.qv;
+        if (join_score && defer) {
+            const int k0 = a->mode == M3PC_MODE_RTG ? M3PC_REWARDS : M3PC_STATES, k1 = a->mode == M3PC_MODE_RTG ? M3PC_RETURNS : M3PC_REWARDS;
+            const size_t need[2] = {(size_t)n * hh * h->feat[k0], (size_t)n * hh * h->feat[k1]};
+            for (int g = 0; g < 2; ++g)
+                if (sl.jpred_floats[g] < need[g]) {
+                    if (sl.jpred[g]) HIPCHK(hipFree(sl.jpred[g]));
+                    sl.jpred[g] = nullptr;
+                    sl.jpred_floats[g] = 0;
+                    CHK(dmalloc(&sl.jpred[g], need[g]));
+                    sl.jpred_floats[g] = need[g];
+                }
+            if (sl.jqv_floats < (size_t)n * hh) {
+                if (sl.jqv) HIPCHK(hipFree(sl.jqv));
+                sl.jqv = nullptr;
+                sl.jqv_floats = 0;
+                CHK(dmalloc(&sl.jqv, (size_t)n * hh));
+                sl.jqv_floats = (size_t)n * hh;
+            }
+            jpred[0] = sl.jpred[0];
+            jpred[1] = sl.jpred[1];
+            jqv = sl.jqv;
+        }
         const int n_stage = h->dm.n_enc_layer + 1;
         PieceState lnst[4];
         for (int stg = 0; stg < (h->prof_serial ? 1 : n_stage) && rc == 0; ++stg) {
             int c0 = 0;
             for (size_t i = 0; i < parts.size() && rc == 0; ++i) {
                 hipStream_t s = i == 0 || h->prof_serial ? st : h->auxs[i - 1];
+                const SampleP sp = sample_args(c0, parts[i]);
                 if (stg == 0) {
                     if (s != st) HIPCHK(hipStreamWaitEvent(s, h->ev_fork, 0));
-                    sample(c0, parts[i], s);
+                    if (!fuse_sample) launch_sample(sp, s);
                 }
                 set_view(h, c0, parts[i]);
+                PassExtras ex = extras(parts[i], &sp);
+                if (join_score) {
+                    ex.no_score = true;
+                    ex.pred[0] = jpred[0];
+                    ex.pred[1] = jpred[1];
+                    ex.qv = jqv;
+                    ex.c0 = c0;
+                }
                 rc = candidate_pass(h, a, states, rewards, parts[i], sample_actions + (size_t)c0 * hh * h->A, expect_return + c0,
                                     pred_rewards ? pred_rewards + (size_t)c0 * hh : nullptr,
                                     pred_boot ? pred_boot + (size_t)c0 * hh : nullptr, dt, s, nullptr,
-                                    h->prof_serial ? 0 : stg, h->prof_serial ? 1 << 30 : stg + 1, &lnst[i]);
+                                    h->prof_serial ? 0 : stg, h->prof_serial ? 1 << 30 : stg + 1, &lnst[i], &ex);
                 if (s != st && stg == n_stage - 1 && rc == 0) {
                     if (defer) {
                         HIPCHK(hipEventRecord(h->slot_join[a->slot][i - 1], s));
@@ -847,11 +914,25 @@
         }
         if (defer && rc == 0) h->defer_parts = parts;
         set_view(h, 0, h->dm.max_candidates);
+        if (join_score && rc == 0) {
+            if (defer) {
+                sl.score_pending = true;
+                sl.score_args = *a;
+                sl.score_args.returns = nullptr;
+                sl.score_actions = sample_actions;
+                sl.score_out = expect_return;
+            } else {
+                rc = score_candidates(h, a, n, jpred[0], jpred[1], jqv, sample_actions, expect_return, nullptr, nullptr, st);
+            }
+        }
         return rc;
     }
     CHK(ws_sync(h, st));
-    sample(0, n, st);
-    return candidate_pass(h, a, states, rewards, n, sample_actions, expect_return, pred_rewards, pred_boot, dt, st);
+    const SampleP sp = sample_args(0, n);
+    if (!fuse_sample) launch_sample(sp, st);
+    const PassExtras ex = extras(n, &sp);
+    return candidate_pass(h, a, states, rewards, n, sample_actions, expect_return, pred_rewards, pred_boot, dt, st, nullptr, 0, 1 << 30,
+                          nullptr, &ex);
 }
 
 int m3pc_candidate_join(m3pc_handle* h, int slot, void* stream) {
@@ -859,6 +940,13 @@
     if (slot < 0 || slot >= M3PC_SLOTS) return fail(M3PC_EINVAL, "slot %d outside [0, %d)", slot, M3PC_SLOTS);
     for (int i = 0; i < h->slot_join_n[slot]; ++i) HIPCHK(hipStreamWaitEvent((hipStream_t)stream, h->slot_join[slot][i], 0));
     h->slot_join_n[slot] = 0;
+    m3pc_handle::Slot& sl = h->slot[slot];
+    if (sl.score_pending) {
+        sl.score_pending = false;
+        HIPCHK(hipSetDevice(h->device));
+        CHK(score_candidates(h, &sl.score_args, sl.score_args.n_count, sl.jpred[0], sl.jpred[1], sl.jqv, sl.score_actions, sl.score_out,
+                             nullptr, nullptr, (hipStream_t)stream));
+    }
     return 0;
 }
 
@@ -966,6 +1054,7 @@
     }
     h->slot[a->slot].policy_valid = E == 1;
     h->slot[a->slot].n_windows = E;
+    h->slot[a->slot].sh_idx = -1;
     if (loc) HIPCHK(hipMemcpyAsync(loc, h->loc, (size_t)E * T * A * sizeof(float), hipMemcpyDeviceToDevice, st));
     if (std_) HIPCHK(hipMemcpyAsync(std_, h->sd, (size_t)E * T * A * sizeof(float), hipMemcpyDeviceToDevice, st));
     return check_launch("policy_pass_batch");
@@ -1737,6 +1826,8 @@
 
 #ifdef M3PC_LAB
 int m3pc_debug_step_streams_created(m3pc_handle* h) { return h ? h->step_streams_created : -1; }
+int m3pc_debug_candidate_switches(void) { return candidate_switches(); }
+int m3pc_debug_shared_rows(int d, int bf16, int batch, int n_indep) { return first_layer_shared_rows(d, bf16 ? DT_BF16 : DT_F32, batch, n_indep); }
 int m3pc_debug_gemm(int dtype, const void* A, const void* Wt, const float* bias, const float* res, void* C, int M, int N,
                     int K, int gelu, int f32out, int variant, void* stream) {
     static const int ldpad = M3PC_ENV("M3PC_DEBUG_LDPAD") ? atoi(M3PC_ENV("M3PC_DEBUG_LDPAD")) : 0;
diff --git a/m3pc_amd/csrc/m3pc_internal.h b/m3pc_amd/csrc/m3pc_internal.h
--- a/m3pc_amd/csrc/m3pc_internal.h
+++ b/m3pc_amd/csrc/m3pc_internal.h
@@ -164,6 +164,15 @@
         float *loc = nullptr, *sd = nullptr, *rtok = nullptr;
         bool policy_valid = false;
         int n_windows = 0;
+        m3pc::bf16_t *sh_hn = nullptr, *sh_qkv = nullptr;
+        int sh_idx = -1, sh_n = 0;
+        const float *sh_states = nullptr, *sh_actions = nullptr;
+        float *jpred[2] = {nullptr, nullptr}, *jqv = nullptr;
+        size_t jpred_floats[2] = {0, 0}, jqv_floats = 0;
+        bool score_pending = false;
+        m3pc_plan_args score_args;
+        const float* score_actions = nullptr;
+        float* score_out = nullptr;
     } slot[M3PC_SLOTS];
     int cur_slot = 0;
     struct Base {
@@ -179,6 +188,9 @@
     } base, chain[2], pchain[2];
     Base* cur = nullptr;
     bool two_stream = true;
+    bool fuse_sample = true;
+    bool pre_shared = true;
+    bool join_score = true;
     bool allow_splitk = true;
     bool x3 = false;
     std::vector<std::pair<const float*, Tensor*>> gemm_w;
@@ -476,6 +488,26 @@
     int normalize[4];
     const int* widx = nullptr;
     long long wstride[4] = {0, 0, 0, 0};
+    const SampleP* sample = nullptr;
+    const bf16_t* sh_qkv = nullptr;
+    int sh_n = 0;
+};
+
+inline int first_layer_shared_rows(int d, int dt, int batch, int n_indep) {
+    static const bool no_prune1 = M3PC_ENV("M3PC_NO_PRUNE1") != nullptr;
+    if (dt == DT_BF16 && batch >= 64 && d % 256 == 0 && d <= 1024 && n_indep >= 32 && !no_prune1) return (n_indep / 32) * 32;
+    return 0;
+}
+inline int candidate_n_indep(int idx) { return (idx + 1) + idx; }
+
+struct PassExtras {
+    const SampleP* sample = nullptr;
+    const bf16_t* sh_qkv = nullptr;
+    int sh_n = 0;
+    bool no_score = false;
+    float* pred[2] = {nullptr, nullptr};
+    float* qv = nullptr;
+    int c0 = 0;
 };
 
 struct PieceState {
@@ -495,7 +527,7 @@
 int run_block(m3pc_handle* h, const std::string& pfx, float* X, int batch, int L, int dt, hipStream_t st, bool ln1_done = false,
               int n_sh = 0, const LnP* next_ln = nullptr, bool* next_ln_done = nullptr, bool x_dead = false,
               float* Xnext = nullptr, int res_nshared = 0, bool qkv_done = false, const std::string* next_qkv = nullptr,
-              bool* next_qkv_done = nullptr, bool x_bf16 = false);
+              bool* next_qkv_done = nullptr, bool x_bf16 = false, const void* qkv_sh_pre = nullptr);
 int run_encoder(m3pc_handle* h, Plan* pl, const TokIn& in, int batch, int dt, hipStream_t st, bool bf16_out_only = false,
                 int n_indep = 0, int layer_from = 0, int layer_to = 1 << 30, PieceState* ln_state = nullptr);
 void dec_embed(m3pc_handle* h, int k, const void* Zop, RowMap amap, float* Yout, RowMap cmap, int M, int mod, int dt,
@@ -510,6 +542,10 @@
                    float** xrows);
 int candidate_pass(m3pc_handle* h, const m3pc_plan_args* a, const float* states, const float* rewards, int n,
                    const float* sample_actions, float* expect_return, float* pred_rewards, float* pred_boot, int dt,
-                   hipStream_t st, const int* widx = nullptr, int stage_from = 0, int stage_to = 1 << 30, PieceState* ln_state = nullptr);
-
-}
+                   hipStream_t st, const int* widx = nullptr, int stage_from = 0, int stage_to = 1 << 30, PieceState* ln_state = nullptr,
+                   const PassExtras* ex = nullptr);
+int score_candidates(m3pc_handle* h, const m3pc_plan_args* a, int n, const float* pred0, const float* pred1, float* qv,
+                     const float* sample_actions, float* expect_return, float* pred_rewards, float* pred_boot, hipStream_t st);
+int precompute_shared_rows(m3pc_handle* h, const m3pc_plan_args* a, const float* states, const float* actions, hipStream_t st);
+
+}
diff --git a/m3pc_amd/csrc/m3pc_passes.hip b/m3pc_amd/csrc/m3pc_passes.hip
--- a/m3pc_amd/csrc/m3pc_passes.hip
+++ b/m3pc_amd/csrc/m3pc_passes.hip
@@ -6,7 +6,7 @@
 int run_block(m3pc_handle* h, const std::string& pfx, float* X, int batch, int L, int dt, hipStream_t st, bool ln1_done,
               int n_sh, const LnP* next_ln, bool* next_ln_done, bool x_dead,
               float* Xnext, int res_nshared, bool qkv_done, const std::string* next_qkv,
-              bool* next_qkv_done, bool x_bf16) {
+              bool* next_qkv_done, bool x_bf16, const void* qkv_sh_pre) {
     const int d = h->d, ff = h->ff;
     const int rows = batch * L;
     const int es = (int)dtype_size(dt);
@@ -41,14 +41,14 @@
         const int n_own = L - n_sh;
         const size_t es2 = dtype_size(dt);
         char* hn_sh = (char*)h->Hn + (size_t)batch * n_own * d * es2;
-        char* qkv_sh = (char*)h->QKV + (size_t)batch * n_own * 3 * d * es2;
+        char* qkv_sh = qkv_sh_pre ? (char*)qkv_sh_pre : (char*)h->QKV + (size_t)batch * n_own * 3 * d * es2;
         {
             GemmP p = gemm_basic(h->Hn, d, Wop(h, pfx + ".self_attn.in_proj_weight", dt), d, batch * n_own, 3 * d, d,
                                  W(h, pfx + ".self_attn.in_proj_bias").f);
             gemm_out(p, dt, h->QKV, 3 * d);
             gemm(h, p, dt, st);
         }
-        {
+        if (!qkv_sh_pre) {
             GemmP p = gemm_basic(hn_sh, d, Wop(h, pfx + ".self_attn.in_proj_weight", dt), d, n_sh, 3 * d, d,
                                  W(h, pfx + ".self_attn.in_proj_bias").f);
             gemm_out(p, dt, qkv_sh, 3 * d);
@@ -260,14 +260,13 @@
 
 int run_encoder(m3pc_handle* h, Plan* pl, const TokIn& in, int batch, int dt, hipStream_t st, bool bf16_out_only,
                 int n_indep, int layer_from, int layer_to, PieceState* ln_state) {
-    int n_sh = 0;
-    static const bool no_prune1 = M3PC_ENV("M3PC_NO_PRUNE1") != nullptr;
-    if (dt == DT_BF16 && batch >= 64 && h->d % 256 == 0 && h->d <= 1024 && n_indep >= 32 && !no_prune1)
-        n_sh = (n_indep / 32) * 32;
+    const int n_sh = first_layer_shared_rows(h->d, dt, batch, n_indep);
+    const void* qkv_sh_pre = n_sh > 0 && in.sh_qkv && in.sh_n == n_sh ? in.sh_qkv : nullptr;
     EmbedP e;
     memset(&e, 0, sizeof(e));
     e.n_indep = n_indep;
     e.n_sh = n_sh;
+    e.sh_skip = qkv_sh_pre ? 1 : 0;
     e.Hb_sh = n_sh ? (bf16_t*)((char*)h->Hn + (size_t)batch * (pl->Le - n_sh) * h->d * 2) : nullptr;
     for (int k = 0; k < 4; ++k) {
         e.tok[k] = in.ptr[k];
@@ -304,7 +303,7 @@
         e.Hb = (bf16_t*)h->Hn;
     else
         e.Hf = (float*)h->Hn;
-    if (layer_from <= 0) launch_embed(e, st);
+    if (layer_from <= 0) launch_embed(e, st, in.sample);
     LnP ln;
     memset(&ln, 0, sizeof(ln));
     ln.X = h->X;
@@ -337,7 +336,8 @@
         const bool q1 = qkv_done;
         qkv_done = false;
         CHK(run_block(h, "encoder.layers." + std::to_string(i), Xs, batch, pl->Le, dt, st, l1, i == 0 ? n_sh : 0, &nxt, &ln_done,
-                      i + 1 == nl && bf16_out_only, Xn, Xn ? n_indep : 0, q1, i + 1 < nl ? &nq : nullptr, &qkv_done, xb16));
+                      i + 1 == nl && bf16_out_only, Xn, Xn ? n_indep : 0, q1, i + 1 < nl ? &nq : nullptr, &qkv_done, xb16,
+                      i == 0 ? qkv_sh_pre : nullptr));
         if (Xn) Xs = Xn;
     }
     if (ln_state) {
@@ -906,55 +906,72 @@
     return rc;
 }
 
-int candidate_pass(m3pc_handle* h, const m3pc_plan_args* a, const float* states, const float* rewards, int n,
-                   const float* sample_actions, float* expect_return, float* pred_rewards, float* pred_boot, int dt,
-                   hipStream_t st, const int* widx, int stage_from, int stage_to, PieceState* ln_state) {
-    const int T = h->T, d = h->d, hh = a->horizon, idx = T - hh;
-    const size_t es = dtype_size(dt);
-    struct ScaleScope {
-        m3pc_handle* h;
-        ~ScaleScope() { h->pass_scale = 1.0; }
-    } scale_scope{h};
-    h->pass_scale = !widx && a->n_total > n ? (double)a->n_total / (double)n : 1.0;
+int precompute_shared_rows(m3pc_handle* h, const m3pc_plan_args* a, const float* states, const float* actions, hipStream_t st) {
+    m3pc_handle::Slot& sl = h->slot[a->slot];
+    sl.sh_idx = -1;
+    const int T = h->T, d = h->d, idx = T - a->horizon;
+    const int dt = pass_dt(a->precision);
+    const int n_sh = h->pre_shared ? first_layer_shared_rows(d, dt, a->n_total, candidate_n_indep(idx)) : 0;
+    if (n_sh <= 0 || !sl.sh_hn) return 0;
     Plan* pl = nullptr;
     CHK(get_mask_plan(h, 1, idx, &pl));
-    const int qi = a->mode == M3PC_MODE_RTG ? 0 : 1;
-    CHK(build_query(h, pl, qi, hh));
-    CHK(build_tables(h, pl, qi, dt, st));
-    Plan::Query& q = pl->query[qi];
-    SharedTables& tb = q.tab[dt];
-    const int Le = pl->Le, nq = q.nq;
-    if ((long long)n * Le > h->R || (long long)n * nq > h->R) return fail(M3PC_ENOMEM, "n_count %d exceeds workspace", n);
-
-    TokIn in;
-    memset(&in, 0, sizeof(in));
-    in.ptr[M3PC_STATES] = states;
-    in.normalize[M3PC_STATES] = h->tok_norm[M3PC_STATES];
-    in.ptr[M3PC_ACTIONS] = h->cand;
-    in.bstride[M3PC_ACTIONS] = (long long)T * h->A;
-    in.normalize[M3PC_ACTIONS] = h->tok_norm[M3PC_ACTIONS];
-    in.ptr[M3PC_REWARDS] = rewards;
-    in.ptr[M3PC_RETURNS] = h->rtok;
-    in.widx = widx;
-    in.wstride[M3PC_STATES] = (long long)T * h->S;
-    in.wstride[M3PC_REWARDS] = T;
-    const int nl_enc = h->dm.n_enc_layer;
-    if (stage_from < nl_enc) CHK(run_encoder(h, pl, in, n, dt, st, dt == DT_BF16, widx ? 0 : (idx + 1) + idx, stage_from, stage_to, ln_state));
-    if (stage_to <= nl_enc) return check_launch("candidate_pass");
-
-    CHK(pruned_decoder(h, pl, q, tb, n, dt, st, TAIL_HEADS, nullptr));
+    if (n_sh > pl->Le || n_sh > 2 * T) return 0;
+    EmbedP e;
+    memset(&e, 0, sizeof(e));
+    const float* src[4] = {states, actions, nullptr, h->rtok};
+    for (int k = 0; k < 4; ++k) {
+        e.tok[k] = src[k];
+        e.normalize[k] = k == M3PC_STATES || k == M3PC_ACTIONS ? h->tok_norm[k] : 0;
+        e.mean[k] = h->tok_mean[k];
+        e.stdv[k] = h->tok_std[k];
+        e.WT[k] = h->WT[k];
+        e.E[k] = h->Eenc[k];
+        e.feat[k] = h->feat[k];
+    }
+    e.tokmap = pl->d_tokmap;
+    e.batch = 1;
+    e.L = pl->Le;
+    e.d = d;
+    e.T = T;
+    e.n_indep = candidate_n_indep(idx);
+    e.n_sh = n_sh;
+    e.sh_only = 1;
+    e.ln_g = W(h, "encoder.layers.0.norm1.weight").f;
+    e.ln_b = W(h, "encoder.layers.0.norm1.bias").f;
+    e.Hb = sl.sh_hn;
+    e.Hb_sh = sl.sh_hn;
+    launch_embed(e, st);
+    const std::string pfx = "encoder.layers.0";
+    GemmP p = gemm_basic(sl.sh_hn, d, Wop(h, pfx + ".self_attn.in_proj_weight", dt), d, n_sh, 3 * d, d,
+                         W(h, pfx + ".self_attn.in_proj_bias").f);
+    gemm_out(p, dt, sl.sh_qkv, 3 * d);
+    const bool splitk = h->allow_splitk;
+    h->allow_splitk = false;
+    gemm(h, p, dt, st);
+    h->allow_splitk = splitk;
+    CHK(check_launch("precompute_shared_rows"));
+    sl.sh_idx = idx;
+    sl.sh_n = n_sh;
+    sl.sh_states = states;
+    sl.sh_actions = actions;
+    return 0;
+}
+
+int score_candidates(m3pc_handle* h, const m3pc_plan_args* a, int n, const float* pred0, const float* pred1, float* qv,
+                     const float* sample_actions, float* expect_return, float* pred_rewards, float* pred_boot, hipStream_t st) {
+    const int hh = a->horizon;
     const float* rw;
     const float* boot;
     float boot_scale;
     if (a->mode == M3PC_MODE_RTG) {
-        rw = h->pred[0];
-        boot = h->pred[1];
+        rw = pred0;
+        boot = pred1;
         boot_scale = 1000.0f;
     } else {
         if (!h->critic_set) return fail(M3PC_ESTATE, "critic weights not set");
         CriticP c;
         memset(&c, 0, sizeof(c));
-        c.states = h->pred[0];
+        c.states = pred0;
         c.actions = sample_actions;
         c.rows = n * hh;
         c.S = h->S;
@@ -972,10 +989,10 @@
             c.W1F[i] = h->cW1F[i];
             c.W2F[i] = h->cW2F[i];
         }
-        c.q = h->qv;
+        c.q = qv;
         launch_critic(c, st);
-        rw = h->pred[1];
-        boot = h->qv;
+        rw = pred1;
+        boot = qv;
         boot_scale = 1.0f;
     }
     ScoreP sc;
@@ -993,6 +1010,56 @@
     sc.scatter_out = h->score_scatter_out;
     launch_score(sc, st);
     if (pred_rewards) HIPCHK(hipMemcpyAsync(pred_rewards, rw, (size_t)n * hh * sizeof(float), hipMemcpyDeviceToDevice, st));
+    return check_launch("score_candidates");
+}
+
+int candidate_pass(m3pc_handle* h, const m3pc_plan_args* a, const float* states, const float* rewards, int n,
+                   const float* sample_actions, float* expect_return, float* pred_rewards, float* pred_boot, int dt,
+                   hipStream_t st, const int* widx, int stage_from, int stage_to, PieceState* ln_state, const PassExtras* ex) {
+    const int T = h->T, hh = a->horizon, idx = T - hh;
+    struct ScaleScope {
+        m3pc_handle* h;
+        ~ScaleScope() { h->pass_scale = 1.0; }
+    } scale_scope{h};
+    h->pass_scale = !widx && a->n_total > n ? (double)a->n_total / (double)n : 1.0;
+    Plan* pl = nullptr;
+    CHK(get_mask_plan(h, 1, idx, &pl));
+    const int qi = a->mode == M3PC_MODE_RTG ? 0 : 1;
+    CHK(build_query(h, pl, qi, hh));
+    CHK(build_tables(h, pl, qi, dt, st));
+    Plan::Query& q = pl->query[qi];
+    SharedTables& tb = q.tab[dt];
+    const int Le = pl->Le, nq = q.nq;
+    if ((long long)n * Le > h->R || (long long)n * nq > h->R) return fail(M3PC_ENOMEM, "n_count %d exceeds workspace", n);
+
+    TokIn in;
+    memset(&in, 0, sizeof(in));
+    in.ptr[M3PC_STATES] = states;
+    in.normalize[M3PC_STATES] = h->tok_norm[M3PC_STATES];
+    in.ptr[M3PC_ACTIONS] = h->cand;
+    in.bstride[M3PC_ACTIONS] = (long long)T * h->A;
+    in.normalize[M3PC_ACTIONS] = h->tok_norm[M3PC_ACTIONS];
+    in.ptr[M3PC_REWARDS] = rewards;
+    in.ptr[M3PC_RETURNS] = h->rtok;
+    in.widx = widx;
+    in.wstride[M3PC_STATES] = (long long)T * h->S;
+    in.wstride[M3PC_REWARDS] = T;
+    if (ex && !widx) {
+        in.sample = ex->sample;
+        in.sh_qkv = ex->sh_qkv;
+        in.sh_n = ex->sh_n;
+    }
+    const int nl_enc = h->dm.n_enc_layer;
+    if (stage_from < nl_enc) CHK(run_encoder(h, pl, in, n, dt, st, dt == DT_BF16, widx ? 0 : candidate_n_indep(idx), stage_from, stage_to, ln_state));
+    if (stage_to <= nl_enc) return check_launch("candidate_pass");
+
+    if (ex && ex->no_score) {
+        for (int g = 0; g < 2; ++g) h->pred[g] = ex->pred[g] + (size_t)ex->c0 * hh * h->feat[q.qkeys[g < q.n_groups ? g : 0]];
+        h->qv = ex->qv + (size_t)ex->c0 * hh;
+        return pruned_decoder(h, pl, q, tb, n, dt, st, TAIL_HEADS, nullptr);
+    }
+    CHK(pruned_decoder(h, pl, q, tb, n, dt, st, TAIL_HEADS, nullptr));
+    CHK(score_candidates(h, a, n, h->pred[0], h->pred[1], h->qv, sample_actions, expect_return, pred_rewards, pred_boot, st));
     return check_launch("candidate_pass");
 }
 
diff --git a/m3pc_amd/planner.py b/m3pc_amd/planner.py
--- a/m3pc_amd/planner.py
+++ b/m3pc_amd/planner.py
@@ -381,7 +381,8 @@
                 chain.wait_event(sl.ev_done)
                 if self._ev_main is not None:
                     chain.wait_event(self._ev_main)
-            hd.policy_pass(mode, states, actions, rewards, h, tk.rtg, slot=sl.i, returns=returns, pruned=self._policy_pruned)
+            hd.policy_pass(mode, states, actions, rewards, h, tk.rtg, slot=sl.i, returns=returns, pruned=self._policy_pruned,
+                           n_total=N, precision=self.precision)
             if eps is None:
                 eps = self._step_eps(tk.index, mode, h, sl.eps_buf if chain is not None else None)
             tk.eps = eps = eps.reshape(N, -1, A)
@@ -436,7 +437,8 @@
         if bound:
             if self._delta_fixed is None and self._cal_left > 0:
                 self._cal_left -= 1
-                hd.policy_pass(mode, states, actions, rewards, h, tk.rtg, slot=sl.i, returns=returns, pruned=self._policy_pruned)
+                hd.policy_pass(mode, states, actions, rewards, h, tk.rtg, slot=sl.i, returns=returns, pruned=self._policy_pruned,
+                               n_total=N, precision=self.precision)
                 low = hd.candidate_pass(mode, states, actions, rewards, eps, h, tk.lmbda, disc, N, precision=self.precision,
                                         slot=sl.i)["expect_return"]
                 d = hd.calibrate_delta(mode, states, actions, rewards, eps, low, h, tk.lmbda, disc, N,
```
